# speechcatcher-asr/speechcatcher

Hardware: AMD Instinct MI355X
Metric: concurrent real-time streams (audio-seconds/s), de_xl dims, 640 ms (10240-sample) chunk steps, beam 10 CTC+attention (higher is better)
Workload: dtype f32

## Files before the change

### include/scasr.h

```cpp
#ifndef SCASR_H
#define SCASR_H

#include <stddef.h>
#include <stdint.h>

#ifdef __cplusplus
extern "C" {
#endif

#define SC_OK 0
#define SC_ERR_ARG (-1)
#define SC_ERR_LAUNCH (-2)
#define SC_ERR_CAPACITY (-3)
#define SC_ERR_INPUT (-4)

#define SC_GEMM_RELU 1
#define SC_GEMM_RESIDUAL 2
#define SC_GEMM_LN_AT_CROWS 8
#define SC_GEMM_NAIVE 4
#define SC_GEMM_SPLIT16 16

#define SC_F_ANY_EOS 1
#define SC_F_BEST_EOS 2
#define SC_F_ALL_EOS 4
// ... 613 lines not shown
  float ctc_weight;
  int32_t use_bbd;
  int32_t max_frames;
  int32_t max_tokens;
  int32_t pcm_capacity;
  int32_t max_chunk_samples;
  int32_t strict_reference;
  int32_t kv_half;
  int32_t kv_pool_rows;
} sc_stream_options;

typedef struct sc_stream_info_t {
  int32_t enc_frames, processed_block, process_idx, n_hyp, hyp_len, pcm_buffered, frontend_started;
  int64_t decode_steps;
} sc_stream_info_t;

typedef struct sc_engine sc_engine;
typedef struct sc_streams sc_streams;

int sc_engine_create(const sc_config *cfg, const sc_named_tensor *tensors, int n_tensors, int device, sc_engine **out);
int sc_engine_load(const char *packed_model_path, int device, sc_engine **out);
int sc_engine_config(const sc_engine *engine, sc_config *out);
void sc_engine_destroy(sc_engine *engine);

int sc_streams_create(sc_engine *engine, const sc_stream_options *options, sc_streams **out);
void sc_streams_destroy(sc_streams *streams);
int sc_push(sc_streams *streams, const int *stream_ids, const float *const *pcm, const int *n_samples,
            const uint8_t *is_final, int n, int *status);
int sc_push_features(sc_streams *streams, const int *stream_ids, const float *const *feats, const int *n_frames,
                     const uint8_t *is_final, int n, int *status);
int sc_submit(sc_streams *streams, const int *stream_ids, const float *const *pcm, const int *n_samples,
              const uint8_t *is_final, int n);
int sc_poll(sc_streams *streams, int min_done, int max_done, int *done_ids , int *status );
int sc_streams_outstanding(const sc_streams *streams);
int sc_streams_set_encoder_batch(sc_streams *streams, int min_streams);
int sc_streams_set_queue_depth(sc_streams *streams, int depth);
const char *sc_stream_last_error(const sc_streams *streams, int stream);
int sc_get_hyps(sc_streams *streams, int stream, int nbest, int max_len, int32_t *ids, int32_t *xpos, int *lens,
                double *scores, double *score_dec, double *score_ctc);
int sc_get_hyps_batch(sc_streams *streams, const int *stream_ids, int n, int nbest, int max_len, int32_t *ids,
                      int32_t *xpos, int *lens, int *n_hyps, double *scores, double *score_dec, double *score_ctc);
int sc_get_hyps_delta(sc_streams *streams, const int *stream_ids, int n, const int *from, const int *final,
                      int max_tail, int32_t *L, int32_t *commit, int32_t *n_hyps, int32_t *ids, int32_t *xpos,
                      double *stability, double *scores, int32_t *status);
int sc_rescore_hyps(sc_streams *streams, const int *stream_ids, int n, int nbest, const sc_lm *lm, double alpha,
                    double beta, int lm_eos, const int *final, int32_t *order, double *fused, double *lm_sum,
                    double *eos_lm, int32_t *status, int *n_hyps);
int sc_lm_rescore_lists(sc_streams *streams, const sc_lm *lm, const int32_t *ids, const int32_t *lens,
                        const double *scores, const int *list_sizes, int n, int nbest, int max_len,
                        const int32_t *state0, double alpha, double beta, int lm_eos, int32_t *order, double *fused,
                        double *lm_sum, double *eos_lm, int32_t *status, int32_t *end_state);
#define SC_ATT_WS_DEFAULT_BYTES ((size_t)256 << 20)
int sc_attention_rescore_beam(sc_streams *streams, const int *stream_ids, int n, int nbest, double w_att, double w_ctc,
                              double beta, int32_t *order, double *fused, double *att, double *ctc_score, int32_t *status,
                              int *n_hyps);
int sc_attention_rescore_lists(sc_streams *streams, const int *stream_ids, int n, const int32_t *ids, const int32_t *lens,
                               const double *scores, const int *list_sizes, int nbest, int max_len, double w_att,
                               double w_ctc, double beta, int32_t *order, double *fused, double *att, int32_t *status);
int sc_streams_set_attention_rescore_ws(sc_streams *streams, size_t max_bytes);
int sc_streams_attention_rescore_ws(const sc_streams *streams, size_t *limit, size_t *allocated);

int sc_align_hyps(sc_streams *streams, const int *stream_ids, int n, int nbest, int max_len, int32_t *start,
                  int32_t *end, float *logp_mean, double *path_score, int *status, int *n_hyps);
int sc_alternates_hyps(sc_streams *streams, const int *stream_ids, int n, int nbest, int max_len, int K, int32_t *start,
                       int32_t *end, float *logp_mean, double *path_score, int *status, int32_t *alt_ids,
                       double *alt_logp, int32_t *own_rank, int32_t *span_status, int *n_hyps);
int sc_align_tokens(sc_streams *streams, int stream, const int32_t *ids, int L, int32_t *start, int32_t *end,
                    float *logp_mean, double *path_score, int *status);
int sc_reset(sc_streams *streams, int stream);
int sc_stream_set_input_rate(sc_streams *streams, int stream, int rate);
int sc_stream_input_rate(const sc_streams *streams, int stream);
int sc_stream_set_input_format(sc_streams *streams, int stream, int format, int channels, int channel, int scale);
int sc_stream_input_format(const sc_streams *streams, int stream, int *format, int *channels, int *channel, int *scale);
int sc_push_raw(sc_streams *streams, const int *stream_ids, const void *const *audio, const int *n_frames,
                const uint8_t *is_final, int n, int *status);
int sc_submit_raw(sc_streams *streams, const int *stream_ids, const void *const *audio, const int *n_frames,
                  const uint8_t *is_final, int n);
int sc_stream_input_level(sc_streams *streams, int stream, sc_input_level_t *out );
int sc_stream_info(const sc_streams *streams, int stream, sc_stream_info_t *out);
#define SC_KV_POOL_DEFAULT_MAX_GIB 24
int sc_streams_kv_rows(const sc_streams *streams);
int sc_streams_stats(const sc_streams *streams, long *enc_calls, long *dec_steps, long *dec_blocks);
int sc_streams_capture_stats(const sc_streams *streams, long *n_captures, double *seconds);
int sc_streams_set_graphs(sc_streams *streams, int on);
int sc_marker(int id, void *stream);
int sc_streams_host_times(sc_streams *streams, double *launch_s, double *wait_s);
int sc_streams_bucket_times(sc_streams *streams, double *seconds, long *iterations);
long sc_streams_take_xattn_rows(sc_streams *streams);
int sc_streams_take_xattn_rows_by_kernel(sc_streams *streams, long *rows);
int sc_streams_take_attn_counters(sc_streams *streams, long *out );
void *sc_streams_hip_stream(sc_streams *streams);
float *sc_streams_pcm(sc_streams *streams, long *capacity);
int sc_streams_write_pcm(sc_streams *streams, int stream, long offset, const float *host, long n);
long sc_streams_read_pcm_buffer(sc_streams *streams, int stream, float *host, long max_n);
int sc_streams_read_enc(sc_streams *streams, int stream, float *host, int max_frames);
int sc_streams_read_ctc(sc_streams *streams, int stream, float *host, int max_rows);
int sc_streams_set_activity(sc_streams *streams, int on, double blank_threshold);
int sc_stream_activity(sc_streams *streams, int stream, sc_activity_t *out );
int sc_streams_read_activity(sc_streams *streams, int stream, double *host, int max_frames);
int sc_streams_set_phrases(sc_streams *streams, const int32_t *labels, const int32_t *lens, const double *min_scores,
                           int n_phrases);
int sc_stream_set_phrase_mask(sc_streams *streams, int stream, uint64_t mask);
int sc_stream_spot(sc_streams *streams, int stream, sc_spot_t *out );
int sc_streams_read_spot_events(sc_streams *streams, int stream, sc_spot_event *host, int max);
int sc_streams_read_spot_state(sc_streams *streams, int stream, double *values, int32_t *starts);
int sc_streams_set_draft(sc_streams *streams, int on);
int sc_stream_draft(sc_streams *streams, int stream, sc_draft_t *out );
int sc_streams_read_draft(sc_streams *streams, int stream, sc_draft_token *host, int max);
int sc_streams_set_ctc_beam(sc_streams *streams, int beam, int candidates);
int sc_stream_ctc_beam(sc_streams *streams, int stream, sc_beam_t *out );
int sc_ctc_beam_hyps(sc_streams *streams, const int *stream_ids, int n, int nbest, int max_len, int32_t *header ,
                     int32_t *ids , int32_t *frames , double *scores );
int sc_streams_set_ctc_beam_lm(sc_streams *streams, const sc_lm *lm, double alpha, double beta);
int sc_stream_ctc_beam_lm(sc_streams *streams, int stream, sc_beam_lm_t *out );
int sc_ctc_beam_hyps_lm(sc_streams *streams, const int *stream_ids, int n, int nbest, double *lm ,
                        double *fused );
int sc_stream_set_grammar(sc_streams *streams, int stream, sc_grammar *grammar );
int sc_stream_ctc_beam_grammar(sc_streams *streams, int stream, sc_beam_gr_t *out );
int sc_ctc_beam_hyps_grammar(sc_streams *streams, const int *stream_ids, int n, int nbest, int32_t *g ,
                             int32_t *accept );
#define SC_DECODER_FULL 0
#define SC_DECODER_NONE 1
int sc_stream_set_decoder(sc_streams *streams, int stream, int mode);
int sc_streams_read_ctc_projected(sc_streams *streams, int stream, float *host , int max_rows);
int sc_stream_decoder(const sc_streams *streams, int stream);

#ifdef __cplusplus
}
#endif
#endif
```

### speechcatcher_amd/_abi.py

```python
import ctypes as C
import os
import subprocess
from pathlib import Path

HERE = Path(__file__).resolve().parent
LIB_PATH = HERE / "libscasr.so"
CSRC = HERE / "csrc"

c_float_p = C.POINTER(C.c_float)
c_int_p = C.POINTER(C.c_int32)
c_double_p = C.POINTER(C.c_double)
vp = C.c_void_p


class EncLayer(C.Structure):
    _fields_ = [(n, vp) for n in ("ln1_g", "ln1_b", "wqkv", "bqkv", "wo", "bo",
                                  "ln2_g", "ln2_b", "w1", "b1", "w2", "b2", "w1_p", "w2_p",
                                  "wqkv_p", "wo_p", "w1_h", "w2_h", "wqkv_h", "wo_h", "w1_s", "w2_s",
                                  "wqkv_s", "wo_s")]


class DecLayer(C.Structure):
    _fields_ = [(n, vp) for n in ("ln1_g", "ln1_b", "wqkv", "bqkv", "wo", "bo",
                                  "ln2_g", "ln2_b", "wq", "bq", "wo2", "bo2",
# ... 258 lines not shown
                                  C.c_int, vp, vp, vp, vp]),
    "sc_rowtile_proj_h": (C.c_int, [vp, C.c_int, C.c_int, C.c_int, vp, vp, C.c_float, vp, vp, C.c_int, vp, vp,
                                    C.c_int, vp, vp, vp, vp]),
    "sc_rowtile_proj_s": (C.c_int, [vp, C.c_int, C.c_int, C.c_int, vp, vp, C.c_float, vp, vp, C.c_int, vp, vp,
                                    C.c_int, vp, vp, vp, vp]),
    "sc_rowtile_proj_supported": (C.c_int, [C.c_int, C.c_int]),
    "sc_workspace_bytes": (C.c_size_t, [vp]),
    "sc_ffn_ln_proj": (C.c_int, [vp, vp, C.c_int, C.c_int, C.c_int, vp, vp, vp, vp, vp, vp, vp, vp, C.c_float, vp,
                                 vp, vp, vp, C.c_int, vp]),
    "sc_graph_capture_begin": (C.c_int, [vp]),
    "sc_graph_capture_end": (C.c_int, [vp, C.POINTER(vp)]),
    "sc_graph_launch": (C.c_int, [vp, vp]),
    "sc_graph_destroy": (C.c_int, [vp]),
    "sc_set_workspace": (C.c_int, [vp, C.c_size_t]),
    "sc_set_stream_workspace": (C.c_int, [vp, vp, C.c_size_t]),
    "sc_prof_collect_kinds": (C.c_int, [C.POINTER(C.c_double), C.POINTER(C.c_double), C.POINTER(C.c_double),
                                        C.POINTER(C.c_longlong), C.c_int]),
    "sc_prof_enable": (C.c_int, [C.c_int]),
    "sc_prof_collect": (C.c_int, [c_double_p, c_double_p, C.POINTER(C.c_longlong)]),
    "sc_prof_collect2": (C.c_int, [c_double_p, c_double_p, c_double_p, C.POINTER(C.c_longlong)]),
    "sc_prof_event_overhead_ms": (C.c_double, [vp]),
    "sc_layernorm": (C.c_int, [vp, vp, C.c_int, vp, vp, C.c_int, C.c_int, C.c_int, vp, vp, C.c_float, vp]),
    "sc_copy_rows": (C.c_int, [vp, vp, vp, vp, C.c_int, C.c_int, vp]),
    "sc_log_softmax_rows": (C.c_int, [vp, vp, C.c_int, C.c_int, vp]),
    "sc_logmel": (C.c_int, [vp, C.c_int, vp, C.c_int, C.c_int, vp, vp, vp, vp, vp, C.c_int, C.c_int,
                            C.c_int, C.c_int, C.c_int, vp, vp]),
    "sc_conv1": (C.c_int, [vp, C.c_int, vp, C.c_int, C.c_int, vp, vp, C.c_int, vp, vp]),
    "sc_block_pack": (C.c_int, [vp, vp, C.c_int, C.c_int, vp, C.c_int, vp, vp]),
    "sc_ctx_handoff": (C.c_int, [vp, C.c_int, vp, C.c_int, vp, C.c_int, C.c_int, vp]),
    "sc_enc_attention": (C.c_int, [vp, vp, C.c_int, C.c_int, C.c_int, C.c_int, C.c_int, vp]),
    "sc_encoder_layers": (C.c_int, [vp, C.c_int, vp, C.c_int, C.c_int, C.c_int, vp, C.c_int, vp, vp,
                                    vp, vp, vp, C.c_int, C.c_int, C.c_int, C.c_float, vp]),
    "sc_glu_dwconv_bn_swish": (C.c_int, [vp, C.c_int, C.c_int, C.c_int, C.c_int, vp, vp, vp, vp, vp, vp,
                                         C.c_float, vp, vp]),
    "sc_relpos_attention": (C.c_int, [vp, vp, vp, vp, vp, C.c_int, C.c_int, C.c_int, C.c_int, vp]),
    "sc_relpos_attention_masked": (C.c_int, [vp, vp, vp, vp, vp, C.c_int, C.c_int, C.c_int, C.c_int, vp, C.c_int, vp]),
    "sc_ctc_extend_state": (C.c_int, [vp, vp]),
    "sc_dec_embed": (C.c_int, [vp, vp]),
    "sc_kv_rows_to_half": (C.c_int, [vp, vp, C.c_int, C.c_int, C.c_int, C.c_int, vp, vp]),
    "sc_dec_self_attn": (C.c_int, [vp, C.c_int, vp]),
    "sc_dec_cross_attn": (C.c_int, [vp, C.c_int, vp]),
    "sc_decoder_layers": (C.c_int, [vp, vp]),
    "sc_logsoftmax_topk": (C.c_int, [vp, vp]),
    "sc_ctc_prefix_scan": (C.c_int, [vp, vp]),
    "sc_fuse_topw": (C.c_int, [vp, vp]),
    "sc_beam_prune": (C.c_int, [vp, vp]),
    "sc_ctc_gather_state": (C.c_int, [vp, vp]),
    "sc_ctc_gather_state_split": (C.c_int, [vp, C.c_int, vp]),
    "sc_decode_step": (C.c_int, [vp, vp]),
    "sc_decode_step_ex": (C.c_int, [vp, C.c_int, vp]),
    "sc_ctc_prefix_scan_split": (C.c_int, [vp, C.c_int, vp]),
    "sc_dec_layer_fused_supported": (C.c_int, [C.c_int, C.c_int, C.c_int, C.c_int]),
    "sc_dec_layer_self": (C.c_int, [vp, C.c_int, vp, vp, vp, C.c_int, vp]),
    "sc_dec_layer_cross": (C.c_int, [vp, C.c_int, vp, vp, vp]),
    "sc_dec_layer_ffn": (C.c_int, [vp, C.c_int, vp, vp, vp, C.c_int, C.POINTER(C.c_int), vp]),
    "sc_dec_output_logits": (C.c_int, [vp, vp, vp, vp, C.c_int, vp]),
    "sc_streams_kv_rows": (C.c_int, [vp]),
    "sc_dec_layer_stream_supported": (C.c_int, [C.c_int, C.c_int, C.c_int, C.c_int]),
    "sc_dec_layer_stream": (C.c_int, [vp, C.c_int, vp, vp, vp, vp, C.c_int, vp]),
    "sc_dec_layer_reduce_ln": (C.c_int, [vp, C.c_int, vp, vp, vp, vp]),
    "sc_dec_layer_ffn_xn": (C.c_int, [vp, C.c_int, vp, vp, C.c_int, C.POINTER(C.c_int), vp]),
    "sc_engine_create": (C.c_int, [C.POINTER(Config), C.POINTER(NamedTensor), C.c_int, C.c_int, C.POINTER(vp)]),
    "sc_engine_load": (C.c_int, [C.c_char_p, C.c_int, C.POINTER(vp)]),
    "sc_engine_config": (C.c_int, [vp, C.POINTER(Config)]),
    "sc_engine_destroy": (None, [vp]),
    "sc_streams_create": (C.c_int, [vp, C.POINTER(StreamOptions), C.POINTER(vp)]),
    "sc_streams_destroy": (None, [vp]),
    "sc_push": (C.c_int, [vp, c_int_p, C.POINTER(vp), c_int_p, C.POINTER(C.c_uint8), C.c_int, c_int_p]),
    "sc_push_features": (C.c_int, [vp, c_int_p, C.POINTER(vp), c_int_p, C.POINTER(C.c_uint8), C.c_int, c_int_p]),
    "sc_get_hyps": (C.c_int, [vp, C.c_int, C.c_int, C.c_int, c_int_p, c_int_p, c_int_p, c_double_p, c_double_p,
                              c_double_p]),
    "sc_get_hyps_batch": (C.c_int, [vp, c_int_p, C.c_int, C.c_int, C.c_int, c_int_p, c_int_p, c_int_p, c_int_p,
                                    c_double_p, c_double_p, c_double_p]),
    "sc_submit": (C.c_int, [vp, c_int_p, C.POINTER(vp), c_int_p, C.POINTER(C.c_uint8), C.c_int]),
    "sc_poll": (C.c_int, [vp, C.c_int, C.c_int, c_int_p, c_int_p]),
    "sc_streams_outstanding": (C.c_int, [vp]),
    "sc_streams_set_encoder_batch": (C.c_int, [vp, C.c_int]),
    "sc_streams_set_queue_depth": (C.c_int, [vp, C.c_int]),
    "sc_stream_last_error": (C.c_char_p, [vp, C.c_int]),
    "sc_reset": (C.c_int, [vp, C.c_int]),
    "sc_stream_info": (C.c_int, [vp, C.c_int, C.POINTER(StreamInfo)]),
    "sc_streams_stats": (C.c_int, [vp, C.POINTER(C.c_long), C.POINTER(C.c_long), C.POINTER(C.c_long)]),
    "sc_streams_capture_stats": (C.c_int, [vp, C.POINTER(C.c_long), c_double_p]),
    "sc_streams_set_graphs": (C.c_int, [vp, C.c_int]),
    "sc_marker": (C.c_int, [C.c_int, vp]),
    "sc_streams_host_times": (C.c_int, [vp, c_double_p, c_double_p]),
    "sc_streams_bucket_times": (C.c_int, [vp, c_double_p, C.POINTER(C.c_long)]),
    "sc_streams_take_xattn_rows": (C.c_long, [vp]),
    "sc_streams_take_xattn_rows_by_kernel": (C.c_int, [vp, vp]),
    "sc_streams_take_attn_counters": (C.c_int, [vp, vp]),
    "sc_streams_hip_stream": (vp, [vp]),
    "sc_streams_pcm": (vp, [vp, C.POINTER(C.c_long)]),
    "sc_streams_write_pcm": (C.c_int, [vp, C.c_int, C.c_long, vp, C.c_long]),
    "sc_streams_read_pcm_buffer": (C.c_long, [vp, C.c_int, vp, C.c_long]),
    "sc_streams_read_enc": (C.c_int, [vp, C.c_int, vp, C.c_int]),
    "sc_ctc_align_ws_bytes": (C.c_size_t, [C.c_int]),
    "sc_ctc_align": (C.c_int, [vp, C.c_int, C.c_int, C.c_int, vp]),
    "sc_align_hyps": (C.c_int, [vp, c_int_p, C.c_int, C.c_int, C.c_int, c_int_p, c_int_p, c_float_p, c_double_p,
                                c_int_p, c_int_p]),
    "sc_align_tokens": (C.c_int, [vp, C.c_int, c_int_p, C.c_int, c_int_p, c_int_p, c_float_p, c_double_p, c_int_p]),
    "sc_streams_read_ctc": (C.c_int, [vp, C.c_int, vp, C.c_int]),
    "sc_ctc_alternates": (C.c_int, [vp, C.c_int, C.c_int, C.c_int, vp]),
    "sc_alternates_hyps": (C.c_int, [vp, c_int_p, C.c_int, C.c_int, C.c_int, C.c_int, c_int_p, c_int_p, c_float_p,
                                     c_double_p, c_int_p, c_int_p, c_double_p, c_int_p, c_int_p, c_int_p]),
    "sc_hyp_commit": (C.c_int, [vp, C.c_int, vp]),
    "sc_get_hyps_delta": (C.c_int, [vp, c_int_p, C.c_int, c_int_p, c_int_p, C.c_int, c_int_p, c_int_p, c_int_p, c_int_p,
                                    c_int_p, c_double_p, c_double_p, c_int_p]),
    "sc_ctc_activity": (C.c_int, [vp, C.c_int, vp]),
    "sc_streams_set_activity": (C.c_int, [vp, C.c_int, C.c_double]),
    "sc_stream_activity": (C.c_int, [vp, C.c_int, C.POINTER(Activity)]),
    "sc_streams_read_activity": (C.c_int, [vp, C.c_int, vp, C.c_int]),
    "sc_ctc_spot": (C.c_int, [vp, C.c_int, vp]),
    "sc_streams_set_phrases": (C.c_int, [vp, vp, vp, vp, C.c_int]),
    "sc_stream_set_phrase_mask": (C.c_int, [vp, C.c_int, C.c_uint64]),
    "sc_stream_spot": (C.c_int, [vp, C.c_int, C.POINTER(Spot)]),
    "sc_streams_read_spot_events": (C.c_int, [vp, C.c_int, vp, C.c_int]),
    "sc_streams_read_spot_state": (C.c_int, [vp, C.c_int, vp, vp]),
    "sc_ctc_draft": (C.c_int, [vp, C.c_int, vp]),
    "sc_streams_set_draft": (C.c_int, [vp, C.c_int]),
    "sc_stream_draft": (C.c_int, [vp, C.c_int, C.POINTER(Draft)]),
    "sc_streams_read_draft": (C.c_int, [vp, C.c_int, vp, C.c_int]),
    "sc_ctc_beam": (C.c_int, [vp, C.c_int, vp]),
    "sc_ctc_beam_pack": (C.c_int, [vp, C.c_int, vp]),
    "sc_ctc_beam_lm": (C.c_int, [vp, C.c_int, vp]),
    "sc_lm_create": (C.c_int, [vp, C.c_size_t, C.POINTER(vp)]),
    "sc_lm_destroy": (None, [vp]),
    "sc_lm_device_view": (C.c_int, [vp, C.POINTER(vp), C.POINTER(LmView)]),
    "sc_streams_set_ctc_beam": (C.c_int, [vp, C.c_int, C.c_int]),
    "sc_stream_ctc_beam": (C.c_int, [vp, C.c_int, C.POINTER(Beam)]),
    "sc_ctc_beam_hyps": (C.c_int, [vp, c_int_p, C.c_int, C.c_int, C.c_int, vp, vp, vp, vp]),
    "sc_streams_set_ctc_beam_lm": (C.c_int, [vp, vp, C.c_double, C.c_double]),
    "sc_stream_ctc_beam_lm": (C.c_int, [vp, C.c_int, C.POINTER(BeamLm)]),
    "sc_ctc_beam_hyps_lm": (C.c_int, [vp, c_int_p, C.c_int, C.c_int, vp, vp]),
    "sc_ctc_beam_grammar": (C.c_int, [vp, C.c_int, vp]),
    "sc_grammar_create": (C.c_int, [vp, C.c_size_t, C.POINTER(vp)]),
    "sc_grammar_destroy": (C.c_int, [vp]),
    "sc_grammar_device_view": (C.c_int, [vp, C.POINTER(vp), C.POINTER(GrammarView)]),
    "sc_grammar_use": (C.c_int, [vp, C.c_int]),
    "sc_grammar_step": (C.c_int, [vp, C.c_int, C.c_int]),
    "sc_grammar_accepts": (C.c_int, [vp, C.c_int]),
    "sc_stream_set_grammar": (C.c_int, [vp, C.c_int, vp]),
    "sc_stream_ctc_beam_grammar": (C.c_int, [vp, C.c_int, C.POINTER(BeamGr)]),
    "sc_ctc_beam_hyps_grammar": (C.c_int, [vp, c_int_p, C.c_int, C.c_int, c_int_p, c_int_p]),
    "sc_lm_rescore": (C.c_int, [vp, C.c_int, vp]),
    "sc_rescore_hyps": (C.c_int, [vp, c_int_p, C.c_int, C.c_int, vp, C.c_double, C.c_double, C.c_int, c_int_p, vp, vp,
                                  vp, vp, vp, c_int_p]),
    "sc_lm_rescore_lists": (C.c_int, [vp, vp, vp, vp, vp, c_int_p, C.c_int, C.c_int, C.c_int, vp, C.c_double,
                                      C.c_double, C.c_int, vp, vp, vp, vp, vp, vp]),
    "sc_seq_attention": (C.c_int, [vp, C.c_int, C.c_int, C.c_int, C.c_int, C.c_int, vp]),
    "sc_dec_rescore_ws_bytes": (C.c_size_t, [vp, C.c_long, C.c_long, C.c_int, C.c_int]),
    "sc_dec_rescore": (C.c_int, [vp, C.c_int, vp, vp, C.c_size_t, vp]),
    "sc_attention_rescore_beam": (C.c_int, [vp, c_int_p, C.c_int, C.c_int, C.c_double, C.c_double, C.c_double, vp, vp, vp, vp,
                                            vp, c_int_p]),
    "sc_attention_rescore_lists": (C.c_int, [vp, c_int_p, C.c_int, vp, vp, vp, c_int_p, C.c_int, C.c_int, C.c_double,
                                             C.c_double, C.c_double, vp, vp, vp, vp]),
    "sc_streams_set_attention_rescore_ws": (C.c_int, [vp, C.c_size_t]),
    "sc_streams_attention_rescore_ws": (C.c_int, [vp, C.POINTER(C.c_size_t), C.POINTER(C.c_size_t)]),
    "sc_stream_set_decoder": (C.c_int, [vp, C.c_int, C.c_int]),
    "sc_stream_decoder": (C.c_int, [vp, C.c_int]),
    "sc_streams_read_ctc_projected": (C.c_int, [vp, C.c_int, vp, C.c_int]),
    "sc_pcm_decode": (C.c_int, [vp, C.c_int, vp]),
    "sc_pcm_bytes_per_frame": (C.c_int, [C.c_int, C.c_int]),
    "sc_stream_set_input_format": (C.c_int, [vp, C.c_int, C.c_int, C.c_int, C.c_int, C.c_int]),
    "sc_stream_input_format": (C.c_int, [vp, C.c_int, c_int_p, c_int_p, c_int_p, c_int_p]),
    "sc_push_raw": (C.c_int, [vp, c_int_p, C.POINTER(vp), c_int_p, C.POINTER(C.c_uint8), C.c_int, c_int_p]),
    "sc_submit_raw": (C.c_int, [vp, c_int_p, C.POINTER(vp), c_int_p, C.POINTER(C.c_uint8), C.c_int]),
# ... 65 lines not shown
```

### speechcatcher_amd/csrc/streams.hip

```cpp
#include <algorithm>
#include <array>
#include <chrono>
#include <cmath>
#include <cstdarg>
#include <cstring>
#include <deque>
#include <map>
#include <memory>
#include <new>
#include <string>
#include <vector>

#include "common.h"
#include "handover.h"
#include "resample.h"

namespace {

#define HIP_TRY(call)                                                              \
  do {                                                                             \
    hipError_t e__ = (call);                                                       \
    if (e__ != hipSuccess) {                                                       \
      sc_set_error("%s: %s failed: %s", __func__, #call, hipGetErrorString(e__));  \
      return SC_ERR_LAUNCH;                                                        \
    }                                                                              \
  } while (0)
#define RC_TRY(call)                 \
  do {                               \
    int rc__ = (call);               \
    if (rc__ != SC_OK) return rc__;  \
  } while (0)

struct Tensor {
  void *ptr = nullptr;
  int64_t numel = 0;
  int dtype = 0;
  bool owned = false;
};

struct StreamFault {
  int stream;
  int code;
  std::string msg;
};

}

struct sc_engine {
  sc_config cfg{};
  int device = 0;
  std::map<std::string, Tensor> t;
  std::vector<sc_enc_layer> enc;
  std::vector<sc_dec_layer> dec;
  std::vector<const float *> wkv, bkv;
  float *wkv_all = nullptr, *bkv_all = nullptr;

  const float *f(const std::string &name, bool required = true) const {
    auto it = t.find(name);
    if (it == t.end()) {
      if (required) sc_set_error("sc_engine: tensor '%s' is missing", name.c_str());
      return nullptr;
    }
    return (const float *)it->second.ptr;
  }
  ~sc_engine() {
    for (auto &kv : t)
      if (kv.second.owned && kv.second.ptr) (void)hipFree(kv.second.ptr);
    if (wkv_all) (void)hipFree(wkv_all);
    if (bkv_all) (void)hipFree(bkv_all);
  }
};

namespace {

struct St {
  bool fe_started = false;
  long pcm_start = 0, pcm_end = 0;
  bool enc_started = false;
  int fpp = 0, nfeat = 0, upp = 0, nsub = 0;
  bool has_sub = false;
  int n_blocks = 0;
  bool has_addin = false, has_ctx = false;
  int short_pos = 0;
  int T_enc = 0, processed_block = 0, process_idx = 0;
  bool prev_valid = false, started = false;
  int cur = 0, L = 1, nhyp = 1;
  bool has_ctc = false;
  int T_ctc = 0, T_kv = 0, output_index = 0;
  int T_proj = 0, T_projkv = 0;
  long n_steps_total = 0;
  int T_hyp = 0;
  int rs_tab = -1, rs_par = 0;
  long rs_in = 0, rs_out = 0;
  int in_fmt = SC_PCM_F32, in_ch = 1, in_sel = 0, in_scale = SC_PCM_SCALE_FULL;
  bool coded() const { return in_fmt != SC_PCM_F32 || in_ch != 1; }
  bool no_dec = false;
};

// ... 62 lines not shown
  HIP_TRY(hipMemset(*p, 0, bytes));
  HIP_TRY(hipStreamSynchronize(nullptr));
  return SC_OK;
}

}

struct EncPlan {
  std::vector<int32_t> conv_jobs, a_rows, lin_dst, feat_src, feat_dst, blk_jobs, sjobs, emit_src, emit_dst, sub_src,
      sub_dst;
  struct Short { int s, ubase, U, pe_pos, dst_T; };
  std::vector<Short> shorts;
  int n_conv = 0, max_t1 = 0;
};

struct EncGroup {
  long gen = 0;
  bool launched = false, features = false;
  bool open = false;
  bool deferred = false;
  int slot = 0;
  int stage_slot = -1;
  std::vector<long long> copy_jobs;
  std::vector<sc_rs_job> rs_jobs;
  size_t stage_floats = 0;
  struct PcmSpan { int s; bool fin; };
  std::vector<sc_pcm_job> pcm_jobs;
  std::vector<PcmSpan> pcm_spans;
  size_t stage_bytes = 0;
  bool stage_filled = false;
  std::vector<int32_t> fe_jobs;
  int n_fe = 0, max_keep = 0;
  EncPlan P;
  std::vector<int32_t> ctc_rows, kv_src, kv_dst;
  struct Span {
    int s = 0, t0 = 0, t1 = 0;
    uint64_t mask = 0;
    const sc_grammar_view *grammar = nullptr;
    handover::Plan opt[N_OPT];
  };
  std::vector<Span> spans;
  bool same_rows = true;
  std::vector<int> streams;
  bool empty() const { return !n_fe && !P.n_conv; }
};

constexpr int N_ARENA = 8;
constexpr int N_STAGE = 4;
constexpr int N_RING = 4;
constexpr int CM_FIXED = 4 + SC_COMMIT_MAX_HYPS + 6;

struct sc_streams {
  sc_engine *eng = nullptr;
  sc_config cfg{};
  int S = 0, W = 0, K = 0, TCAP = 0, LCAP = 0, FCAP = 0, UCAP = 0, max_feat_new = 0, max_t1 = 0, max_t2 = 0,
      max_blocks = 0, max_chunk = 0, max_length = 500;
  long PCAP = 0;
  bool use_bbd = false, strict = true;
  hipStream_t stream = nullptr;
  hipStream_t stream_enc = nullptr, es = nullptr;
  hipEvent_t ev_iter[2] = {nullptr, nullptr};
  int32_t *ring_dev = nullptr;
  int32_t *rm_host[2] = {nullptr, nullptr};
  int rm_idx = 0;
  bool rm_dirty = false;
  int scan_split_min = 1024, scan_split_streams = 0;
  bool scan_long = false;
  int step_split_min() const { return (scan_long && (scan_split_streams <= 0 || n_rows_step <= scan_split_streams * W)) ? scan_split_min : 0; }
  int graph_key() const { return n_rows_step * 2 + (step_split_min() > 0 ? 1 : 0); }
  int enc_start_thr = 0;
  int enc_batch_min = 0;
  int gemm_flags = 0;
  void *ws = nullptr, *ws_enc = nullptr;
  std::vector<void *> owned, owned_host;
  float *pcm = nullptr, *featbuf = nullptr, *subbuf = nullptr, *prev_addin = nullptr, *past_ctx = nullptr, *enc = nullptr,
        *c1 = nullptr, *c2 = nullptr, *xblk = nullptr, *ws_xn = nullptr, *ws_qkv = nullptr, *ws_att = nullptr,
        *ws_ffh = nullptr;
  int32_t *jobs_ctx = nullptr, *ctrlmap = nullptr;
  float *kv_stage = nullptr;
  int kv_stage_rows = 0;
  sc_search sb{};
  int32_t *ctrlmap_host = nullptr, *flags_host = nullptr;
  int32_t *arena_host = nullptr, *arena_dev = nullptr;
  size_t slot_cap = 0, arena_off = 0;
  int cur_slot = 0;
  hipEvent_t ev_group[N_ARENA] = {nullptr};
  long slot_gen[N_ARENA] = {0};
  int32_t *bs_host = nullptr, *bs_dev = nullptr;
  size_t bs_cap = 0;
  int bs_i = 0;
  float *stage_host = nullptr, *stage_dev = nullptr;
  size_t stage_cap = 0;
  hipEvent_t ev_stage[N_STAGE] = {nullptr};
  bool stage_busy[N_STAGE] = {false};
  int stage_next = 0;
  long long *cjobs_host = nullptr, *cjobs_dev = nullptr;
  sc_rs_job *rsjobs_host = nullptr, *rsjobs_dev = nullptr;
  float *rs_hist = nullptr;
  sc_rs_tabs rs_tabs{};
  int rs_rate[SC_RS_MAX_TABS] = {0};
  int n_rs_tabs = 0;
  uint8_t *stageb_host = nullptr, *stageb_dev = nullptr;
  size_t stageb_cap = 0;
  sc_pcm_job *pcmjobs_host = nullptr, *pcmjobs_dev = nullptr;
  sc_input_level_t *lvl_state = nullptr;
  sc_input_level_t *lvl_out_host = nullptr, *lvl_out_dev = nullptr;
  struct LvlSpan { int s; long epoch, ticket; };
  std::vector<LvlSpan> stage_lvl[N_STAGE];
  handover::Track<LevelState> lvl;
  long lvl_ticket = 0;
  int32_t *pack_dev = nullptr, *pack_host = nullptr, *pjobs_host = nullptr, *pjobs_dev = nullptr;
  size_t pack_cap = 0;
  sc_hyp_commit_job *cmjobs_host = nullptr, *cmjobs_dev = nullptr;
  int32_t *cm_dev = nullptr, *cm_host = nullptr;
  size_t cm_cap = 0;
  char *al_dev = nullptr;
  size_t al_cap = 0;
  bool act_on = false;
  double act_thr = 0.8;
  int32_t *act_state = nullptr;
  double *act_track = nullptr;
  sc_ctc_activity_job *act_jobs_host = nullptr, *act_jobs_dev = nullptr;
  int32_t *act_out_host = nullptr, *act_out_dev = nullptr;
  handover::Track<ActState> act;
  bool spot_on = false;
  int spot_P = 0;
  int32_t *spot_labels = nullptr, *spot_lens = nullptr;
  double *spot_floors = nullptr;
  int32_t *spot_counters = nullptr;
  double *spot_values = nullptr;
  int32_t *spot_starts = nullptr;
  sc_spot_event *spot_events = nullptr;
  sc_ctc_spot_job *spot_jobs_host = nullptr, *spot_jobs_dev = nullptr;
  int32_t *spot_out_host = nullptr, *spot_out_dev = nullptr;
  handover::Track<SpotState> spot;
  std::vector<uint64_t> spot_mask;
  bool draft_on = false;
  sc_draft_t *draft_state = nullptr;
  sc_draft_token *draft_tokens = nullptr;
  sc_ctc_draft_job *draft_jobs_host = nullptr, *draft_jobs_dev = nullptr;
  sc_draft_t *draft_out_host = nullptr, *draft_out_dev = nullptr;
  handover::Track<DraftState> draft;
  bool beam_on = false;
  int beam_B = 0, beam_C = 0;
  int beam_nodes_B = 0;
  sc_beam_t *beam_state = nullptr;
  sc_beam_node *beam_nodes = nullptr;
  sc_ctc_beam_job *beam_jobs_host = nullptr, *beam_jobs_dev = nullptr;
  sc_beam_t *beam_out_host = nullptr, *beam_out_dev = nullptr;
  handover::Track<BeamState> beam;
  const sc_lm *beam_lm = nullptr;
  const sc_lm_view *beam_lm_view = nullptr;
  sc_lm_view beam_lm_info{};
  double beam_alpha = 0.0, beam_beta = 0.0;
  sc_beam_lm_t *beam_lm_state = nullptr;
  sc_ctc_beam_lm_job *beam_lm_jobs_host = nullptr, *beam_lm_jobs_dev = nullptr;
  sc_beam_lm_t *beam_lm_out_host = nullptr, *beam_lm_out_dev = nullptr;
  std::vector<sc_grammar *> beam_gr;
  int beam_gr_n = 0;
  sc_beam_gr_t *beam_gr_state = nullptr;
  sc_ctc_beam_gr_job *beam_gr_jobs_host = nullptr, *beam_gr_jobs_dev = nullptr;
  sc_beam_gr_t *beam_gr_out_host = nullptr, *beam_gr_out_dev = nullptr;
  char *bh_dev = nullptr, *bh_host = nullptr;
  size_t bh_cap = 0;
  char *rs_dev = nullptr, *rs_host = nullptr;
  size_t rs_cap = 0;
  char *ar_dev = nullptr, *ar_host = nullptr;
  size_t ar_cap = 0;
  char *ar_ws = nullptr;
  size_t ar_ws_bytes = 0, ar_ws_limit = SC_ATT_WS_DEFAULT_BYTES;
  void *ar_splitk = nullptr;
  size_t beam_ncap() const { return 1 + (size_t)beam_nodes_B * TCAP; }
  std::vector<St> st;
  std::vector<Run> run;
  std::vector<std::deque<Blk>> bq;
  std::vector<Job> job;
  std::vector<std::deque<Job>> ahead;
  std::vector<long> job_seq;
  int queue_depth = 1;
  std::vector<Snap> snap;
  std::vector<long> done_at;
  long done_counter = 0;
  int32_t *snap_yseq = nullptr, *snap_xpos = nullptr;
  double *snap_score = nullptr;
  hipEvent_t ev_snap = nullptr;
  std::vector<std::string> fault_msg;
  std::vector<long> enc_gen;
  std::deque<EncGroup *> groups;
  long gen_next = 1, gen_done = 0, gen_ordered = 0;
  int n_open = 0;
  long iter = 0;
  bool inflight = false;
  std::vector<int> tick_active;
  std::chrono::steady_clock::time_point tick_t0, tick_t1;
  hipStream_t stream_rb = nullptr;
  bool poisoned = false;
  std::vector<int> rowmap_key;
  int row_bucket = 1, n_rows_step = 0;
  bool decode_prepared = false;
  std::map<int, hipGraphExec_t> dec_graphs;
  std::map<std::vector<long>, hipGraphExec_t> enc_graphs;
  long dec_steps = 0, dec_blocks = 0, enc_calls = 0, xattn_rows[3] = {0, 0, 0};
  long sattn_pos[3] = {0, 0, 0};
  unsigned long long *stat_rows = nullptr;
  double t_launch = 0, t_wait = 0;
  double t_bucket[17] = {0};
  long n_bucket[17] = {0};
  bool use_graphs = true;
  long n_enc_captures = 0;
  double t_enc_capture = 0;

  ~sc_streams() {
    for (auto &g : dec_graphs) (void)hipGraphExecDestroy(g.second);
    for (auto &g : enc_graphs) (void)hipGraphExecDestroy(g.second);
    if (stream) (void)sc_set_stream_workspace(stream, nullptr, 0);
    if (stream_enc) {
      (void)sc_set_stream_workspace(stream_enc, nullptr, 0);
      (void)hipStreamDestroy(stream_enc);
    }
    for (int i = 0; i < 2; ++i)
      if (ev_iter[i]) (void)hipEventDestroy(ev_iter[i]);
    for (int i = 0; i < N_ARENA; ++i)
      if (ev_group[i]) (void)hipEventDestroy(ev_group[i]);
    for (int i = 0; i < N_STAGE; ++i)
      if (ev_stage[i]) (void)hipEventDestroy(ev_stage[i]);
    if (ev_snap) (void)hipEventDestroy(ev_snap);
    for (EncGroup *g : groups) delete g;
    for (void *p : owned) (void)hipFree(p);
    for (void *p : owned_host) (void)hipHostFree(p);
    if (stream_rb && ar_splitk) (void)sc_set_stream_workspace(stream_rb, nullptr, 0);
    if (stream_rb) (void)hipStreamDestroy(stream_rb);
    if (stream) (void)hipStreamDestroy(stream);
    if (ar_dev) (void)hipFree(ar_dev);
    if (ar_host) (void)hipHostFree(ar_host);
    if (ar_ws) (void)hipFree(ar_ws);
    if (ar_splitk) (void)hipFree(ar_splitk);
    if (al_dev) (void)hipFree(al_dev);
    if (beam_nodes) (void)hipFree(beam_nodes);
    for (sc_grammar *g : beam_gr)
      if (g) (void)sc_grammar_use(g, -1);
    if (bh_dev) (void)hipFree(bh_dev);
    if (bh_host) (void)hipHostFree(bh_host);
    if (rs_dev) (void)hipFree(rs_dev);
    if (rs_host) (void)hipHostFree(rs_host);
  }

  template <typename T>
  int alloc(T **p, size_t n) {
    RC_TRY(dalloc(p, n));
    owned.push_back(*p);
    return SC_OK;
  }
  template <typename T>
  int halloc(T **p, size_t n) {
    HIP_TRY(hipHostMalloc((void **)p, std::max<size_t>(n, 1) * sizeof(T)));
    owned_host.push_back(*p);
    memset(*p, 0, std::max<size_t>(n, 1) * sizeof(T));
    return SC_OK;
  }
  template <typename T>
  int halloc_mapped(T **host, T **dev, size_t n, const char *who, const char *what) {
    RC_TRY(halloc(host, n));
    void *dv = nullptr;
    if (hipHostGetDevicePointer(&dv, *host, 0) != hipSuccess || !dv) {
      sc_set_error("%s: the pinned %s are not visible to the device", who, what);
      return SC_ERR_LAUNCH;
    }
    *dev = (T *)dv;
    return SC_OK;
  }
  int32_t *ctrl_host() { return ctrlmap_host; }
  int32_t *rowmap_host() { return rm_host[rm_idx]; }

  int itensor(const std::vector<int32_t> &a, const int32_t **out) {
    const size_t n = a.size();
    if (arena_off + n > slot_cap) {
      sc_set_error("job-table arena exhausted (%zu + %zu of %zu entries)", arena_off, n, slot_cap);
      return SC_ERR_ARG;
    }
    const size_t off = (size_t)cur_slot * slot_cap + arena_off;
    arena_off += (n + 63) & ~size_t(63);
    if (n) {
      memcpy(arena_host + off, a.data(), n * sizeof(int32_t));
      HIP_TRY(hipMemcpyAsync(arena_dev + off, arena_host + off, n * sizeof(int32_t), hipMemcpyHostToDevice, es));
    }
    *out = arena_dev + off;
    return SC_OK;
  }
};


namespace {

constexpr int F_ANY_EOS = 1, F_BEST_EOS = 2, F_ALL_EOS = 4, F_REPEAT = 8;

__global__ void init_hyp_kernel(sc_search sb, int s) {
  const size_t o = ((size_t)0 * sb.S + s) * sb.W + 0;
  sb.yseq[o * sb.LCAP] = sb.sos;
  sb.xpos[o * sb.LCAP] = 0;
  sb.anc[((size_t)0 * sb.S + s) * sb.LCAP * sb.W] = 0;
  sb.score[o] = 0.0;
  sb.sc_dec[o] = 0.0;
  sb.sc_ctc[o] = 0.0;
}

__global__ __launch_bounds__(256) void scatter_f32_kernel(const float *__restrict__ src, float *__restrict__ dst,
                                                          const long long *__restrict__ jobs) {
  const long long so = jobs[blockIdx.y * 3], dof = jobs[blockIdx.y * 3 + 1], n = jobs[blockIdx.y * 3 + 2];
  for (long long i = (long long)blockIdx.x * 256 + threadIdx.x; i < n; i += (long long)gridDim.x * 256) dst[dof + i] = src[so + i];
}

void launch_scatter(const float *src, float *dst, const long long *jobs_dev, int nj, long long mx, hipStream_t st) {
  dim3 grid((unsigned)std::min<long long>(64, (std::max<long long>(mx, 1) + 1023) / 1024), nj);
  scatter_f32_kernel<<<grid, 256, 0, st>>>(src, dst, jobs_dev);
}

__global__ __launch_bounds__(128) void pack_hyps_kernel(sc_search sb, const int32_t *__restrict__ jobs, int32_t *__restrict__ out,
                                                        const int32_t *__restrict__ snap_yseq, const int32_t *__restrict__ snap_xpos,
                                                        const double *__restrict__ snap_score) {
  const int32_t *j = jobs + (size_t)blockIdx.x * 4;
  const size_t row = (size_t)j[0];
  const int L = j[1];
  const bool snap = j[3] != 0;
  int32_t *o = out + (size_t)j[2];
  const int32_t *ys = (snap ? snap_yseq : sb.yseq) + row * sb.LCAP, *xp = (snap ? snap_xpos : sb.xpos) + row * sb.LCAP;
  for (int i = threadIdx.x; i < L; i += 128) {
    o[i] = ys[i];
    o[L + i] = xp[i];
  }
  if (threadIdx.x == 0) {
    double *sc = (double *)(o + ((2 * L + 1) & ~1));
    sc[0] = snap ? snap_score[row * 3] : sb.score[row];
    sc[1] = snap ? snap_score[row * 3 + 1] : sb.sc_dec[row];
    sc[2] = snap ? snap_score[row * 3 + 2] : sb.sc_ctc[row];
  }
}

struct SnapArgs { int n; int s[32], cur[32], L[32], nhyp[32]; };
__global__ __launch_bounds__(128) void snapshot_hyps_kernel(sc_search sb, SnapArgs a, int32_t *__restrict__ snap_yseq,
                                                            int32_t *__restrict__ snap_xpos, double *__restrict__ snap_score) {
  const int e = blockIdx.x, h = blockIdx.y;
  if (h >= a.nhyp[e]) return;
  const size_t src = ((size_t)a.cur[e] * sb.S + a.s[e]) * sb.W + h, dst = (size_t)a.s[e] * sb.W + h;
  for (int i = threadIdx.x; i < a.L[e]; i += 128) {
    snap_yseq[dst * sb.LCAP + i] = sb.yseq[src * sb.LCAP + i];
    snap_xpos[dst * sb.LCAP + i] = sb.xpos[src * sb.LCAP + i];
  }
  if (threadIdx.x == 0) {
    snap_score[dst * 3] = sb.score[src];
    snap_score[dst * 3 + 1] = sb.sc_dec[src];
    snap_score[dst * 3 + 2] = sb.sc_ctc[src];
  }
}

void init_hyp(sc_streams *b, int s) {
  init_hyp_kernel<<<1, 1, 0, b->stream>>>(b->sb, s);
}

void reset_stream(sc_streams *b, int s) {
  St old = b->st[s], ns;
  ns.rs_tab = old.rs_tab;
  ns.in_fmt = old.in_fmt; ns.in_ch = old.in_ch; ns.in_sel = old.in_sel; ns.in_scale = old.in_scale;
  ns.no_dec = old.no_dec;
  if (b->strict) {
    ns.short_pos = old.short_pos;
    ns.T_ctc = old.T_ctc;
    ns.T_proj = old.T_ctc;
  }
  b->st[s] = ns;
  b->run[s] = Run();
// ... 142 lines not shown
        st.has_sub = true;
        st.nsub = U;
        continue;
      }
      const int overlap = c.block_size - c.hop_size;
      nb = std::max(0, U - overlap) / c.hop_size;
      const int res = U - c.hop_size * nb;
      const int obase = ((1 - st.upp) * S + s) * b->UCAP;
      for (int i = 0; i < res; ++i) {
        P.sub_src.push_back(ubase + U - res + i);
        P.sub_dst.push_back(obase + i);
      }
      st.upp = 1 - st.upp;
      st.has_sub = true;
      st.nsub = res;
    }
    nb = std::max(nb, 0);
    const int b0 = n_blk_jobs;
    for (int i = 0; i < nb; ++i) {
      const int cur_hop = i * c.hop_size;
      const int clen = std::min(c.block_size, U - cur_hop);
      P.blk_jobs.insert(P.blk_jobs.end(), {ubase + cur_hop, clen, cur_hop + c.hop_size * st.n_blocks, i + st.n_blocks, 0, 0});
      ++n_blk_jobs;
    }
    if (nb > 0) {
      P.sjobs.insert(P.sjobs.end(), {b0, nb, s, (int)st.has_addin, (int)st.has_ctx});
      st.has_addin = st.has_ctx = true;
    }
    const bool first = st.n_blocks == 0;
    const int y_len = fin ? (first ? U : U - offset) : nb * c.hop_size + (first ? offset : 0);
    std::vector<int32_t> src(std::max(y_len, 0), -1);
    if (first && nb > 0)
      for (int i = 0; i < offset && i < y_len; ++i) src[i] = b0 * R + 1 + i;
    for (int i = 0; i < nb; ++i) {
      const int cur_hop = i * c.hop_size + (first ? offset : 0);
      const int clen = (i == nb - 1 && fin) ? std::min(c.block_size - offset, y_len - cur_hop) : c.hop_size;
      for (int j = 0; j < clen; ++j)
        if (cur_hop + j >= 0 && cur_hop + j < y_len) src[cur_hop + j] = (b0 + i) * R + 1 + offset + j;
    }
    if (st.T_enc + y_len > b->TCAP) throw StreamFault{s, SC_ERR_CAPACITY, "encoder-frame capacity exceeded (max_frames)"};
    for (int i = 0; i < y_len; ++i) {
      P.emit_src.push_back(src[i]);
      P.emit_dst.push_back(s * b->TCAP + st.T_enc + i);
    }
    st.T_enc += y_len;
    st.n_blocks += nb;
  }
  for (int s : streams)
    if (finals.at(s)) {
      St &st = b->st[s];
      st.enc_started = false;
      st.nfeat = st.nsub = st.n_blocks = 0;
      st.has_sub = st.has_addin = st.has_ctx = false;
    }
}

int enc_layers_launch(sc_streams *b, int nblk, int R, bool masked, const int32_t *jobs, int ns) {
  const sc_config &c = b->cfg;
  sc_engine *e = b->eng;
  auto launch = [&]() {
    return sc_encoder_layers(e->enc.data(), (int)e->enc.size(), b->xblk, nblk, R, masked ? 1 : 0, jobs, ns, b->past_ctx,
                             b->ws_xn, b->ws_qkv, b->ws_att, b->ws_ffh, c.d_model, c.enc_heads, c.ffn_dim, c.ln_eps,
                             b->es);
  };
  if (!b->use_graphs) return launch();
  std::vector<long> key{nblk, R, (long)masked, (long)(intptr_t)jobs, ns};
  auto it = b->enc_graphs.find(key);
  if (it == b->enc_graphs.end()) {
    if (b->enc_graphs.size() >= 192) return launch();
    const auto tc0 = std::chrono::steady_clock::now();
    RC_TRY(sc_graph_capture_begin(b->es));
    const int rc = launch();
    void *g = nullptr;
    const int rc2 = sc_graph_capture_end(b->es, &g);
    b->n_enc_captures++;
    b->t_enc_capture += std::chrono::duration<double>(std::chrono::steady_clock::now() - tc0).count();
    if (rc != SC_OK) return rc;
    if (rc2 != SC_OK) return rc2;
    it = b->enc_graphs.emplace(key, (hipGraphExec_t)g).first;
  }
  return sc_graph_launch(it->second, b->es);
}

int encode_short(sc_streams *b, const EncPlan::Short &sh) {
  const sc_config &c = b->cfg;
  sc_engine *e = b->eng;
  const int U = sh.U;
  const int32_t *jd, *src, *dst;
  RC_TRY(b->itensor({sh.ubase, U, sh.pe_pos, 0, 1, 0}, &jd));
  RC_TRY(sc_block_pack(b->subbuf, jd, 1, U, e->f("pe"), c.d_model, b->xblk, b->es));
  RC_TRY(sc_encoder_layers(e->enc.data(), (int)e->enc.size(), b->xblk, 1, U, 0, nullptr, 0, b->past_ctx, b->ws_xn,
                           b->ws_qkv, b->ws_att, b->ws_ffh, c.d_model, c.enc_heads, c.ffn_dim, c.ln_eps, b->es));
  std::vector<int32_t> a(U), d(U);
  for (int i = 0; i < U; ++i) { a[i] = i; d[i] = sh.s * b->TCAP + sh.dst_T + i; }
  RC_TRY(b->itensor(a, &src));
  RC_TRY(b->itensor(d, &dst));
  RC_TRY(sc_layernorm(b->xblk, src, c.d_model, b->enc, dst, c.d_model, U, c.d_model, e->f("enc_norm_g"), e->f("enc_norm_b"),
                      c.ln_eps, b->es));
  return SC_OK;
}

int encode_launch(sc_streams *b, EncPlan &P) {
  const sc_config &c = b->cfg;
  sc_engine *e = b->eng;
  const int d = c.d_model, F1 = c.conv_freq1, F2 = c.conv_freq2, R = c.block_size + 2;
  b->enc_calls++;
  const int32_t *cj, *ar, *ld;
  RC_TRY(b->itensor(P.conv_jobs, &cj));
  RC_TRY(sc_conv1(b->featbuf, c.n_mels, cj, P.n_conv, P.max_t1, e->f("conv1_w"), e->f("conv1_b"), d, b->c1, b->es));
  RC_TRY(b->itensor(P.a_rows, &ar));
  RC_TRY(sc_gemm(b->c1, ar, d, e->f("conv2_w"), e->f("conv2_b"), b->c2, nullptr, d, (int)P.a_rows.size(), d, 9 * d,
                 SC_GEMM_RELU | b->gemm_flags, F1, b->es));
  RC_TRY(b->itensor(P.lin_dst, &ld));
  RC_TRY(sc_gemm(b->c2, nullptr, F2 * d, e->f("sub_out_w"), e->f("sub_out_b"), b->subbuf, ld, d, (int)P.lin_dst.size(), d,
                 F2 * d, b->gemm_flags, 0, b->es));
  if (!P.feat_src.empty()) {
    const int32_t *a, *z;
    RC_TRY(b->itensor(P.feat_src, &a));
    RC_TRY(b->itensor(P.feat_dst, &z));
    RC_TRY(sc_copy_rows(b->featbuf, a, b->featbuf, z, (int)P.feat_src.size(), c.n_mels, b->es));
  }
  const int nbk = (int)P.blk_jobs.size() / 6, ns = (int)P.sjobs.size() / 5;
  if (nbk > 0) {
    if (nbk > b->max_blocks) {
      sc_set_error("sc_push: too many encoder blocks in one call");
      return SC_ERR_ARG;
    }
    const int32_t *bj, *ja;
    RC_TRY(b->itensor(P.blk_jobs, &bj));
    RC_TRY(sc_block_pack(b->subbuf, bj, nbk, R, e->f("pe"), d, b->xblk, b->es));
    std::vector<int32_t> j_add(ns * 4), j_ctx(ns * 4);
    for (int i = 0; i < ns; ++i) {
      const int32_t *sj = &P.sjobs[i * 5];
      j_add[i * 4 + 0] = sj[0]; j_add[i * 4 + 1] = sj[1]; j_add[i * 4 + 2] = sj[2]; j_add[i * 4 + 3] = sj[3];
      j_ctx[i * 4 + 0] = sj[0]; j_ctx[i * 4 + 1] = sj[1]; j_ctx[i * 4 + 2] = sj[2] * c.enc_layers; j_ctx[i * 4 + 3] = sj[4];
    }
    RC_TRY(b->itensor(j_add, &ja));
    RC_TRY(sc_ctx_handoff(b->xblk, R, ja, ns, b->prev_addin, 0, d, b->es));
    const int32_t *jc;
    RC_TRY(b->itensor(j_ctx, &jc));
    HIP_TRY(hipMemcpyAsync(b->jobs_ctx, jc, j_ctx.size() * sizeof(int32_t), hipMemcpyDeviceToDevice, b->es));
    RC_TRY(enc_layers_launch(b, nbk, R, true, b->jobs_ctx, ns));
  }
  if (!P.emit_src.empty()) {
    const int32_t *a, *z;
    RC_TRY(b->itensor(P.emit_src, &a));
    RC_TRY(b->itensor(P.emit_dst, &z));
    RC_TRY(sc_layernorm(b->xblk, a, d, b->enc, z, d, (int)P.emit_src.size(), d, e->f("enc_norm_g"), e->f("enc_norm_b"),
                        c.ln_eps, b->es));
  }
  for (auto &sh : P.shorts) RC_TRY(encode_short(b, sh));
  if (!P.sub_src.empty()) {
    const int32_t *a, *z;
    RC_TRY(b->itensor(P.sub_src, &a));
    RC_TRY(b->itensor(P.sub_dst, &z));
    RC_TRY(sc_copy_rows(b->subbuf, a, b->subbuf, z, (int)P.sub_src.size(), d, b->es));
  }
  return SC_OK;
}

void set_rowmap(sc_streams *b, const std::vector<int> &active) {
  const int S = b->S, W = b->W;
  const int na = (int)active.size();
  const int nb = std::min(S, (na + b->row_bucket - 1) / b->row_bucket * b->row_bucket);
  if (active != b->rowmap_key) {
    b->rowmap_key = active;
    b->rm_idx ^= 1;
    b->rm_dirty = true;
    int32_t *rm = b->rowmap_host();
    std::vector<char> isact(S, 0);
    for (int s : active) isact[s] = 1;
    int k = 0;
    for (int pass = 1; pass >= 0; --pass)
      for (int s = 0; s < S; ++s)
        if (isact[s] == pass)
          for (int h = 0; h < W; ++h) rm[k++] = s * W + h;
  }
  b->n_rows_step = nb * W;
}

int decode_step_launch(sc_streams *b) {
  b->sb.n_rows = b->n_rows_step;
  b->sb.flags = b->ring_dev;
  auto step = [&]() { return sc_decode_step_ex(&b->sb, b->step_split_min(), b->stream); };
  if (!b->use_graphs) return step();
  auto it = b->dec_graphs.find(b->graph_key());
  if (it == b->dec_graphs.end()) {
    RC_TRY(step());
    RC_TRY(sc_graph_capture_begin(b->stream));
    const int rc = step();
    void *g = nullptr;
    const int rc2 = sc_graph_capture_end(b->stream, &g);
    if (rc != SC_OK) return rc;
    if (rc2 != SC_OK) return rc2;
    b->dec_graphs[b->graph_key()] = (hipGraphExec_t)g;
    return SC_OK;
  }
  return sc_graph_launch(it->second, b->stream);
}

int prepare_decode(sc_streams *b) {
  memset(b->ctrl_host(), 0, (size_t)b->S * 8 * sizeof(int32_t));
  HIP_TRY(hipMemcpyAsync(b->ctrlmap, b->ctrlmap_host, (size_t)b->S * 8 * sizeof(int32_t), hipMemcpyHostToDevice, b->stream));
  const int keep = b->n_rows_step;
  for (int nb = b->row_bucket; nb < b->S + b->row_bucket; nb += b->row_bucket) {
    b->n_rows_step = std::min(nb, b->S) * b->W;
    if (!b->dec_graphs.count(b->graph_key())) RC_TRY(decode_step_launch(b));
  }
  b->n_rows_step = keep;
  HIP_TRY(hipStreamSynchronize(b->stream));
  return SC_OK;
}

int collect_levels(sc_streams *b, int slot, bool wait) {
  std::vector<sc_streams::LvlSpan> &spans = b->stage_lvl[slot];
  if (spans.empty()) return SC_OK;
  if (wait) HIP_TRY(hipEventSynchronize(b->ev_stage[slot]));
  else {
    const hipError_t q = hipEventQuery(b->ev_stage[slot]);
    if (q == hipErrorNotReady) { (void)hipGetLastError(); return SC_OK; }
    if (q != hipSuccess) {
      sc_set_error("staging slot %d failed: %s", slot, hipGetErrorString(q));
      return SC_ERR_LAUNCH;
    }
  }
  for (size_t i = 0; i < spans.size(); ++i) {
    const sc_streams::LvlSpan &sp = spans[i];
    b->lvl.deliver(sp.s, sp.ticket, sp.epoch, b->lvl_out_host[(size_t)slot * b->S + i], b->job[sp.s], b->ahead[sp.s], &Job::level);
  }
  spans.clear();
  return SC_OK;
}

int retire_groups(sc_streams *b) {
  if (b->lvl_state)
    for (int i = 0; i < N_STAGE; ++i) RC_TRY(collect_levels(b, i, false));
  while (!b->groups.empty()) {
    EncGroup *g = b->groups.front();
    if (!g->launched) break;
    const hipError_t q = hipEventQuery(b->ev_group[g->slot]);
    if (q == hipErrorNotReady) { (void)hipGetLastError(); break; }
    if (q != hipSuccess) {
      sc_set_error("encoder group %ld failed: %s", g->gen, hipGetErrorString(q));
      return SC_ERR_LAUNCH;
    }
    for (size_t i = 0; i < g->spans.size(); ++i) {
      const EncGroup::Span &sp = g->spans[i];
      const int s = sp.s;
      const size_t o = (size_t)g->slot * b->S + i;
      if (sp.opt[OPT_ACT].on) {
        ActState v;
        v.T = sp.t1;
        memcpy(v.v, b->act_out_host + o * 6, sizeof v.v);
        b->act.deliver(s, g->gen, sp.opt[OPT_ACT].epoch, v, b->job[s], b->ahead[s], &Job::act);
      }
      if (sp.opt[OPT_SPOT].on) {
        SpotState v;
        memcpy(v.v, b->spot_out_host + o * 2, sizeof v.v);
        b->spot.deliver(s, g->gen, sp.opt[OPT_SPOT].epoch, v, b->job[s], b->ahead[s], &Job::spot);
      }
      if (sp.opt[OPT_DRAFT].on)
        b->draft.deliver(s, g->gen, sp.opt[OPT_DRAFT].epoch, DraftState{b->draft_out_host[o]}, b->job[s], b->ahead[s], &Job::draft);
      if (sp.opt[OPT_BEAM].on)
        b->beam.deliver(s, g->gen, sp.opt[OPT_BEAM].epoch,
                        b->beam_lm      ? BeamState(b->beam_out_host[o], b->beam_lm_out_host[o])
                        : sp.grammar ? BeamState(b->beam_out_host[o], b->beam_gr_out_host[o])
                                     : BeamState(b->beam_out_host[o]),
                        b->job[s], b->ahead[s], &Job::beam);
    }
    b->gen_done = g->gen;
    b->slot_gen[g->slot] = 0;
    b->groups.pop_front();
    delete g;
  }
  return SC_OK;
}

int launch_pending_groups(sc_streams *b, long upto = -1);
int wait_group(sc_streams *b, long gen) {
  if (gen <= b->gen_done) return SC_OK;
  RC_TRY(launch_pending_groups(b, gen));
  const int slot = (int)(gen % N_ARENA);
  HIP_TRY(hipEventSynchronize(b->ev_group[slot]));
  return retire_groups(b);
}

template <typename J>
void span_job(const sc_streams *b, J &j, const EncGroup::Span &sp, int opt) {
  const int V = b->cfg.vocab_size;
  j.table = b->sb.ctcx + (size_t)sp.s * b->TCAP * V;
  j.stride = V;
  j.V = V; j.blank = b->cfg.blank_id; j.t0 = sp.t0; j.t1 = sp.t1;
  j.restart = sp.opt[opt].restart ? 1 : 0;
}

void span_job(const sc_streams *b, sc_ctc_beam_lm_job &j, const EncGroup::Span &sp, int opt) { span_job(b, j.beam, sp, opt); }

template <typename J, typename Fill>
int launch_spans(sc_streams *b, const EncGroup &g, int opt, const char *name, J *jobs_host, J *jobs_dev,
                 int (*launch)(const J *, int, void *), Fill fill) {
  if (g.spans.empty() || !g.spans[0].opt[opt].on) return SC_OK;
  const int n = (int)g.spans.size();
  if (n > b->S) {
    sc_set_error("%s: %d spans in a group of a batch of %d streams (internal error)", name, n, b->S);
    return SC_ERR_ARG;
  }
  const size_t o = (size_t)g.slot * b->S;
  for (int i = 0; i < n; ++i) {
    span_job(b, jobs_host[o + i], g.spans[i], opt);
    fill(jobs_host[o + i], g.spans[i], o + i);
  }
  HIP_TRY(hipMemcpyAsync(jobs_dev + o, jobs_host + o, (size_t)n * sizeof(J), hipMemcpyHostToDevice, b->es));
  return launch(jobs_dev + o, n, b->es);
}

template <typename Fill>
int launch_beam_grammars(sc_streams *b, const EncGroup &g, Fill beam_fill) {
  if (g.spans.empty() || !g.spans[0].opt[OPT_BEAM].on) return SC_OK;
  const int n = (int)g.spans.size();
  if (n > b->S) {
    sc_set_error("beam: %d spans in a group of a batch of %d streams (internal error)", n, b->S);
    return SC_ERR_ARG;
  }
  const size_t o = (size_t)g.slot * b->S;
  int n_plain = 0, n_gr = 0;
  for (int i = 0; i < n; ++i) {
    const EncGroup::Span &sp = g.spans[i];
    if (!sp.grammar) {
      sc_ctc_beam_job &j = b->beam_jobs_host[o + n_plain++];
      span_job(b, j, sp, OPT_BEAM);
      beam_fill(j, sp, o + i);
    } else {
      sc_ctc_beam_gr_job &j = b->beam_gr_jobs_host[o + n_gr++];
      span_job(b, j.beam, sp, OPT_BEAM);
      beam_fill(j.beam, sp, o + i);
      j.grammar = sp.grammar;
      j.gr_state = b->beam_gr_state + sp.s;
      j.gr_state_after = b->beam_gr_out_dev + o + i;
    }
  }
  if (n_plain) {
    HIP_TRY(hipMemcpyAsync(b->beam_jobs_dev + o, b->beam_jobs_host + o, (size_t)n_plain * sizeof(sc_ctc_beam_job),
                           hipMemcpyHostToDevice, b->es));
    RC_TRY(sc_ctc_beam(b->beam_jobs_dev + o, n_plain, b->es));
  }
  if (n_gr) {
    HIP_TRY(hipMemcpyAsync(b->beam_gr_jobs_dev + o, b->beam_gr_jobs_host + o, (size_t)n_gr * sizeof(sc_ctc_beam_gr_job),
                           hipMemcpyHostToDevice, b->es));
    RC_TRY(sc_ctc_beam_grammar(b->beam_gr_jobs_dev + o, n_gr, b->es));
  }
  return SC_OK;
}

int project_rows(sc_streams *b, EncGroup &g) {
  const sc_config &c = b->cfg;
  sc_engine *e = b->eng;
  const int d = c.d_model, Ld = c.dec_layers, V = c.vocab_size;
  const int32_t *ar = nullptr;
  if (!g.ctc_rows.empty()) {
    RC_TRY(b->itensor(g.ctc_rows, &ar));
    RC_TRY(sc_gemm(b->enc, ar, d, e->f("ctc_w"), e->f("ctc_b"), const_cast<float *>(b->sb.ctcx), ar, V, (int)g.ctc_rows.size(),
                   V, d, b->gemm_flags, 0, b->es));
    RC_TRY(launch_spans(b, g, OPT_ACT, "activity", b->act_jobs_host, b->act_jobs_dev, sc_ctc_activity,
                        [=](sc_ctc_activity_job &j, const EncGroup::Span &sp, size_t at) {
                          j.state = b->act_state + (size_t)sp.s * 6;
                          j.track = b->act_track + (size_t)sp.s * b->TCAP;
                          j.state_after = b->act_out_dev + at * 6;
                          j.thr = b->act_thr;
                          j.reserved = 0;
                        }));
    RC_TRY(launch_spans(b, g, OPT_SPOT, "spotting", b->spot_jobs_host, b->spot_jobs_dev, sc_ctc_spot,
                        [=](sc_ctc_spot_job &j, const EncGroup::Span &sp, size_t at) {
                          j.labels = b->spot_labels; j.lens = b->spot_lens; j.floors = b->spot_floors;
                          j.counters = b->spot_counters + (size_t)sp.s * 2;
                          j.values = b->spot_values + (size_t)sp.s * SC_SPOT_MAX_PHRASES * SC_SPOT_STATES;
                          j.starts = b->spot_starts + (size_t)sp.s * SC_SPOT_MAX_PHRASES * SC_SPOT_STATES;
                          j.events = b->spot_events + (size_t)sp.s * SC_SPOT_MAX_EVENTS;
                          j.state_after = b->spot_out_dev + at * 2;
                          j.mask = sp.mask;
                          j.P = b->spot_P;
                        }));
    RC_TRY(launch_spans(b, g, OPT_DRAFT, "draft", b->draft_jobs_host, b->draft_jobs_dev, sc_ctc_draft,
                        [=](sc_ctc_draft_job &j, const EncGroup::Span &sp, size_t at) {
                          j.state = b->draft_state + sp.s;
                          j.tokens = b->draft_tokens + (size_t)sp.s * b->TCAP;
                          j.state_after = b->draft_out_dev + at;
                          j.capacity = b->TCAP;
                        }));
    const auto beam_fill = [=](sc_ctc_beam_job &j, const EncGroup::Span &sp, size_t at) {
      j.state = b->beam_state + sp.s;
      j.nodes = b->beam_nodes + (size_t)sp.s * b->beam_ncap();
      j.state_after = b->beam_out_dev + at;
      j.capacity = (int32_t)b->beam_ncap();
      j.B = b->beam_B; j.C = b->beam_C;
    };
    bool any_grammar = false;
    for (const EncGroup::Span &sp : g.spans) any_grammar = any_grammar || sp.grammar;
    if (any_grammar)
      RC_TRY(launch_beam_grammars(b, g, beam_fill));
    else if (!b->beam_lm)
      RC_TRY(launch_spans(b, g, OPT_BEAM, "beam", b->beam_jobs_host, b->beam_jobs_dev, sc_ctc_beam, beam_fill));
    else
      RC_TRY(launch_spans(b, g, OPT_BEAM, "beam", b->beam_lm_jobs_host, b->beam_lm_jobs_dev, sc_ctc_beam_lm,
                          [=](sc_ctc_beam_lm_job &j, const EncGroup::Span &sp, size_t at) {
                            beam_fill(j.beam, sp, at);
                            j.lm = b->beam_lm_view;
                            j.lm_state = b->beam_lm_state + sp.s;
                            j.lm_state_after = b->beam_lm_out_dev + at;
                            j.alpha = b->beam_alpha; j.beta = b->beam_beta;
                          }));
  }
  if (!g.kv_dst.empty()) {
    if (!g.same_rows || !ar) RC_TRY(b->itensor(g.kv_src, &ar));
    const int32_t *kvt;
    RC_TRY(b->itensor(g.kv_dst, &kvt));
    const int m = (int)g.kv_dst.size();
    const bool all = e->wkv_all && (2 * d) % 128 == 0;
    if (!b->sb.kv_half) {
      if (all && sc_gemm_colblocks(b->enc, ar, d, e->wkv_all, e->bkv_all, const_cast<float *>(b->sb.ckv), kvt, 2 * d, m, Ld * 2 * d, d,
                                   2 * d, (long)b->TCAP * 2 * d, b->gemm_flags, b->es) == SC_OK)
        return SC_OK;
      for (int li = 0; li < Ld; ++li)
        RC_TRY(sc_gemm(b->enc, ar, d, e->wkv[li], e->bkv[li], const_cast<float *>(b->sb.ckv) + (size_t)li * b->TCAP * 2 * d,
                       kvt, 2 * d, m, 2 * d, d, b->gemm_flags, 0, b->es));
    } else {
      for (int r0 = 0; r0 < m; r0 += b->kv_stage_rows) {
        const int mm = std::min(b->kv_stage_rows, m - r0);
        if (!(all && sc_gemm_colblocks(b->enc, ar + r0, d, e->wkv_all, e->bkv_all, b->kv_stage, nullptr, 2 * d, mm, Ld * 2 * d, d, 2 * d,
                                       (long)mm * 2 * d, b->gemm_flags, b->es) == SC_OK))
          for (int li = 0; li < Ld; ++li)
            RC_TRY(sc_gemm(b->enc, ar + r0, d, e->wkv[li], e->bkv[li], b->kv_stage + (size_t)li * mm * 2 * d, nullptr, 2 * d,
                           mm, 2 * d, d, b->gemm_flags, 0, b->es));
        RC_TRY(sc_kv_rows_to_half(b->kv_stage, kvt + r0, mm, Ld, b->TCAP, 2 * d, const_cast<float *>(b->sb.ckv), b->es));
      }
    }
  }
  return SC_OK;
}

int stage_copy(sc_streams *b, EncGroup &g) {
  if (g.copy_jobs.empty() && g.rs_jobs.empty() && g.pcm_jobs.empty()) return SC_OK;
  hipStream_t es = b->stream_enc ? b->stream_enc : b->stream;
  const int ss = g.stage_slot;
  const size_t so = (size_t)ss * b->stage_cap, jo = (size_t)ss * b->S * 3;
  const int nj = (int)g.copy_jobs.size() / 3;
  if (g.stage_floats && (g.stage_filled || g.pcm_jobs.empty()))
    HIP_TRY(hipMemcpyAsync(b->stage_dev + so, b->stage_host + so, g.stage_floats * sizeof(float), hipMemcpyHostToDevice, es));
  if (!g.pcm_jobs.empty()) {
    const size_t bo = (size_t)ss * b->stageb_cap, po = (size_t)ss * b->S;
    const int np = (int)g.pcm_jobs.size();
    if (g.stage_bytes)
      HIP_TRY(hipMemcpyAsync(b->stageb_dev + bo, b->stageb_host + bo, g.stage_bytes, hipMemcpyHostToDevice, es));
    memcpy(b->pcmjobs_host + po, g.pcm_jobs.data(), np * sizeof(sc_pcm_job));
    HIP_TRY(hipMemcpyAsync(b->pcmjobs_dev + po, b->pcmjobs_host + po, np * sizeof(sc_pcm_job), hipMemcpyHostToDevice, es));
    RC_TRY(sc_pcm_decode(b->pcmjobs_dev + po, np, es));
  }
  if (nj) {
    memcpy(b->cjobs_host + jo, g.copy_jobs.data(), g.copy_jobs.size() * sizeof(long long));
    HIP_TRY(hipMemcpyAsync(b->cjobs_dev + jo, b->cjobs_host + jo, g.copy_jobs.size() * sizeof(long long), hipMemcpyHostToDevice, es));
    long long mx = 1;
    for (int j = 0; j < nj; ++j) mx = std::max(mx, g.copy_jobs[j * 3 + 2]);
    launch_scatter(b->stage_dev + so, g.features ? b->featbuf : b->pcm, b->cjobs_dev + jo, nj, mx, es);
  }
  if (!g.rs_jobs.empty()) {
    const size_t ro = (size_t)ss * b->S;
    const int nr = (int)g.rs_jobs.size();
    memcpy(b->rsjobs_host + ro, g.rs_jobs.data(), nr * sizeof(sc_rs_job));
    HIP_TRY(hipMemcpyAsync(b->rsjobs_dev + ro, b->rsjobs_host + ro, nr * sizeof(sc_rs_job), hipMemcpyHostToDevice, es));
    long long tiles = 1;
    for (const sc_rs_job &j : g.rs_jobs) tiles = std::max(tiles, sc_rs_tiles(b->rs_tabs, j.tab, j.n_out));
    RC_TRY(sc_rs_launch(b->rs_tabs, nullptr, b->rsjobs_dev + ro, nr, tiles, b->stage_dev + so, b->pcm, b->rs_hist, b->S, es));
  }
  HIP_TRY(hipEventRecord(b->ev_stage[ss], es));
  b->stage_busy[ss] = true;
  g.copy_jobs.clear();
  g.rs_jobs.clear();
  g.pcm_jobs.clear();
  g.pcm_spans.clear();
  return SC_OK;
}

void merge_group(sc_streams *b, EncGroup &dst, EncGroup &src) {
  const sc_config &c = b->cfg;
  const int F1 = c.conv_freq1, R = c.block_size + 2;
  EncPlan &D = dst.P, &P = src.P;
  int c1_rows = 0;
  if (D.n_conv) c1_rows = D.conv_jobs[(D.n_conv - 1) * 4 + 2] + D.conv_jobs[(D.n_conv - 1) * 4 + 3];
  const int nblk = (int)D.blk_jobs.size() / 6;
  for (int j = 0; j < P.n_conv; ++j) P.conv_jobs[j * 4 + 2] += c1_rows;
  for (auto &v : P.a_rows) v += c1_rows * F1;
  for (size_t j = 0; j < P.sjobs.size(); j += 5) P.sjobs[j] += nblk;
  for (auto &v : P.emit_src)
    if (v >= 0) v += nblk * R;
  auto cat = [](std::vector<int32_t> &a, const std::vector<int32_t> &x) { a.insert(a.end(), x.begin(), x.end()); };
  cat(D.conv_jobs, P.conv_jobs); cat(D.a_rows, P.a_rows); cat(D.lin_dst, P.lin_dst); cat(D.feat_src, P.feat_src);
  cat(D.feat_dst, P.feat_dst); cat(D.blk_jobs, P.blk_jobs); cat(D.sjobs, P.sjobs); cat(D.emit_src, P.emit_src);
  cat(D.emit_dst, P.emit_dst); cat(D.sub_src, P.sub_src); cat(D.sub_dst, P.sub_dst);
  D.shorts.insert(D.shorts.end(), P.shorts.begin(), P.shorts.end());
  D.n_conv += P.n_conv;
  D.max_t1 = std::max(D.max_t1, P.max_t1);
  cat(dst.fe_jobs, src.fe_jobs);
  dst.n_fe += src.n_fe;
  dst.max_keep = std::max(dst.max_keep, src.max_keep);
  cat(dst.ctc_rows, src.ctc_rows); cat(dst.kv_src, src.kv_src); cat(dst.kv_dst, src.kv_dst);
  dst.spans.insert(dst.spans.end(), src.spans.begin(), src.spans.end());
  dst.same_rows = dst.same_rows && src.same_rows;
  dst.streams.insert(dst.streams.end(), src.streams.begin(), src.streams.end());
}

int launch_group(sc_streams *b, EncGroup *g) {
  if (g->launched) return SC_OK;
  g->launched = true;
  g->open = false;
  const sc_config &c = b->cfg;
  sc_engine *e = b->eng;
  b->es = b->stream_enc ? b->stream_enc : b->stream;
  b->cur_slot = g->slot;
  b->arena_off = 0;
  int rc = SC_OK;
  if (rc == SC_OK && g->n_fe) {
    const int32_t *jobs;
    rc = b->itensor(g->fe_jobs, &jobs);
    if (rc == SC_OK)
      rc = sc_logmel(b->pcm, (int)b->PCAP, jobs, g->n_fe, g->max_keep, e->f("window"), e->f("mel_fb"), e->f("twiddle"),
                     (const double *)e->f("mean64"), (const double *)e->f("std64"), c.mvn_mode, c.n_fft, c.hop_length,
                     c.win_length, c.n_mels, b->featbuf, b->es);
  }
  if (rc == SC_OK && g->P.n_conv) rc = encode_launch(b, g->P);
  if (rc == SC_OK) rc = project_rows(b, *g);
  (void)hipEventRecord(b->ev_group[g->slot], b->es);
  if (b->es == b->stream) b->gen_ordered = std::max(b->gen_ordered, g->gen);
  b->es = b->stream;
  return rc;
}

int launch_pending_groups(sc_streams *b, long upto) {
  for (EncGroup *g : b->groups)
    if (!g->launched && (upto < 0 || g->gen <= upto)) RC_TRY(launch_group(b, g));
  return SC_OK;
}

void finish_block(sc_streams *b, int s) {
  Run &r = b->run[s];
  const bool rw = r.pidx > 1 && r.pvalid;
  const bool r2 = rw && r.took;
  if (r2) {
    r.cur = 1 - r.cur;
    r.L -= 1;
    r.nhyp = r.nhp;
    r.has = r.hasp;
  }
  if (rw) { r.pidx -= 1; r.pvalid = false; }
  St &x = b->st[s];
  x.cur = r.cur; x.L = r.L; x.nhyp = r.nhyp; x.has_ctc = r.has;
  x.T_hyp = r.T;
  x.process_idx = r.pidx; x.prev_valid = r.pvalid;
  x.output_index = r.out;
  x.n_steps_total += r.nsteps;
  if (!r.fin) x.processed_block += 1;
  r.inblk = false;
}

void fault_stream(sc_streams *b, int s, int code, const std::string &msg) {
  const long seq = b->run[s].inblk ? b->run[s].job : b->job[s].seq;
  bool hit = false;
  auto mark = [&](Job &j) {
    if (!j.open) return;
    if (j.seq == seq) { j.fault = code; hit = true; }
    else if (hit && !j.fault) { j.fault = code; j.dropped = true; }
  };
  mark(b->job[s]);
  for (Job &j : b->ahead[s]) mark(j);
  b->fault_msg[s] = msg;
  b->run[s] = Run();
  b->bq[s].clear();
}

inline bool chunk_decoded(const sc_streams *b, int s);

inline bool may_start(const sc_streams *b, int s) {
  const Job &j = b->job[s];
  const long q = b->bq[s].front().job;
  if (!j.open || q <= j.seq) return true;
  return q == j.seq + 1 && b->snap[s].valid && b->snap[s].seq == j.seq;
}

int snapshot_completed(sc_streams *b) {
  if (b->queue_depth <= 1) return SC_OK;
  SnapArgs a;
  a.n = 0;
  bool any = false;
  auto flush = [&]() -> int {
    if (!a.n) return SC_OK;
    snapshot_hyps_kernel<<<dim3(a.n, b->W), 128, 0, b->stream>>>(b->sb, a, b->snap_yseq, b->snap_xpos, b->snap_score);
    SC_CHECK_LAUNCH();
    a.n = 0;
    return SC_OK;
  };
  for (int s = 0; s < b->S; ++s) {
    const Job &j = b->job[s];
    Snap &sn = b->snap[s];
    if (!j.open || j.fault || sn.valid || !chunk_decoded(b, s)) continue;
    const St &x = b->st[s];
    sn.valid = true;
    sn.reported = false;
    sn.seq = j.seq;
    sn.L = x.L;
    sn.T = x.T_hyp;
    sn.nhyp = j.started ? x.nhyp : 0;
    if (sn.nhyp > 0) {
      a.s[a.n] = s; a.cur[a.n] = x.cur; a.L[a.n] = x.L; a.nhyp[a.n] = x.nhyp;
      a.n++;
      any = true;
      if (a.n == 32) RC_TRY(flush());
    }
  }
  RC_TRY(flush());
  if (any) HIP_TRY(hipEventRecord(b->ev_snap, b->stream));
  return SC_OK;
}

int start_blocks(sc_streams *b) {
  const int S = b->S;
  const long gen_ok = std::max(b->gen_done, b->gen_ordered);
  std::vector<int> starts;
  for (int s = 0; s < S; ++s)
    if (!b->run[s].inblk && !b->bq[s].empty() && b->bq[s].front().gen <= gen_ok && may_start(b, s)) starts.push_back(s);
  if (starts.empty()) return SC_OK;
  if (!b->decode_prepared) {
    b->decode_prepared = true;
    RC_TRY(prepare_decode(b));
  }
  b->bs_i = (b->bs_i + 1) % N_RING;
  int32_t *ctrl0 = b->bs_host + (size_t)b->bs_i * b->bs_cap, *lsm = ctrl0 + (size_t)S * 8;
  memset(ctrl0, 0, (size_t)S * 8 * sizeof(int32_t));
  int n_lsm = 0;
  for (int s : starts) {
    const Blk k = b->bq[s].front();
    b->bq[s].pop_front();
    St &x = b->st[s];
    Run &r = b->run[s];
    r = Run();
    r.inblk = r.live = true;
    r.T = k.T; r.fin = k.fin; r.job = k.job;
    r.cur = x.cur; r.L = x.L; r.nhyp = x.nhyp; r.has = x.has_ctc; r.pidx = x.process_idx; r.pvalid = x.prev_valid;
    const int told = x.T_ctc;
    r.Tc = std::max(k.T, told);
    if (k.T > told && told == 0)
      for (int t = 0; t < k.T && n_lsm < (int)(b->bs_cap - (size_t)S * 8); ++t) lsm[n_lsm++] = s * b->TCAP + t;
    int32_t *c = ctrl0 + s * 8;
    c[0] = 1; c[1] = r.cur; c[2] = r.fin; c[3] = r.Tc; c[4] = r.L; c[5] = r.nhyp; c[6] = r.has; c[7] = told;
    x.T_ctc = r.Tc;
    x.T_kv = std::max(k.T, x.T_kv);
    x.output_index = 0;
    r.nhp = r.nhyp; r.hasp = r.has;
    b->dec_blocks++;
  }
  HIP_TRY(hipMemcpyAsync(b->ctrlmap, ctrl0, (size_t)S * 8 * sizeof(int32_t), hipMemcpyHostToDevice, b->stream));
  if (n_lsm) {
    int32_t *ld = b->bs_dev + (size_t)b->bs_i * b->bs_cap;
    HIP_TRY(hipMemcpyAsync(ld, lsm, (size_t)n_lsm * sizeof(int32_t), hipMemcpyHostToDevice, b->stream));
    RC_TRY(sc_log_softmax_rows(const_cast<float *>(b->sb.ctcx), ld, n_lsm, b->cfg.vocab_size, b->stream));
  }
  RC_TRY(sc_ctc_extend_state(&b->sb, b->stream));
  return SC_OK;
}

int tick_collect(sc_streams *b);
int tick_issue(sc_streams *b, bool *progress) {
  const int S = b->S, W = b->W, Ld = b->cfg.dec_layers;
  *progress = false;
  if (b->inflight) RC_TRY(tick_collect(b));
  RC_TRY(retire_groups(b));
  RC_TRY(snapshot_completed(b));
  RC_TRY(start_blocks(b));
  {
    long need = 0;
    for (int s = 0; s < S; ++s)
      if (!b->run[s].inblk && !b->bq[s].empty()) need = std::max(need, b->bq[s].front().gen);
    long upto = -1;
    for (EncGroup *g : b->groups)
      if (!g->launched && g->deferred && g->gen <= need) upto = g->gen;
    if (upto >= 0) RC_TRY(launch_pending_groups(b, upto));
  }
  std::vector<int> &active = b->tick_active;
  active.clear();
  for (int s = 0; s < S; ++s) {
    Run &r = b->run[s];
    if (!r.inblk) continue;
    const bool act = r.live && r.pidx < b->max_length;
    if (act && r.L + 1 > b->LCAP) {
      fault_stream(b, s, SC_ERR_CAPACITY, "max_tokens exceeded");
      *progress = true;
      continue;
    }
    if (!act) {
      finish_block(b, s);
      *progress = true;
      continue;
    }
    active.push_back(s);
  }
  if (active.empty()) {
    if (*progress) return SC_OK;
    long need = 0;
    for (int s = 0; s < S; ++s)
      if (!b->run[s].inblk && !b->bq[s].empty() && (need == 0 || b->bq[s].front().gen < need)) need = b->bq[s].front().gen;
    if (need > std::max(b->gen_done, b->gen_ordered)) {
      RC_TRY(launch_pending_groups(b, need));
      if (b->stream_enc) HIP_TRY(hipStreamWaitEvent(b->stream, b->ev_group[need % N_ARENA], 0));
      b->gen_ordered = std::max(b->gen_ordered, need);
      *progress = true;
    }
    return SC_OK;
  }
  *progress = true;
  b->tick_t0 = std::chrono::steady_clock::now();
  set_rowmap(b, active);
  b->scan_long = false;
  int32_t *ctrl = b->ctrl_host();
  memset(ctrl, 0, (size_t)S * 8 * sizeof(int32_t));
  for (int s : active) {
    const Run &r = b->run[s];
    if (b->scan_split_min > 0 && r.Tc - std::max(r.L - 1, 1) >= b->scan_split_min) b->scan_long = true;
    int32_t *c = ctrl + s * 8;
    c[0] = 1; c[1] = r.cur; c[2] = r.fin; c[3] = r.T; c[4] = r.L; c[5] = r.nhyp; c[6] = r.has; c[7] = r.Tc;
  }
  if ((int)active.size() <= b->enc_start_thr)
    for (EncGroup *g : b->groups)
      if (!g->launched && !g->open) RC_TRY(launch_group(b, g));
  if (b->rm_dirty) {
    memcpy(b->ctrlmap_host + S * 8, b->rm_host[b->rm_idx], (size_t)S * W * sizeof(int32_t));
    HIP_TRY(hipMemcpyAsync(b->ctrlmap, b->ctrlmap_host, (size_t)(S * 8 + S * W) * sizeof(int32_t), hipMemcpyHostToDevice, b->stream));
    b->rm_dirty = false;
  } else {
    HIP_TRY(hipMemcpyAsync(b->ctrlmap, b->ctrlmap_host, (size_t)S * 8 * sizeof(int32_t), hipMemcpyHostToDevice, b->stream));
  }
  RC_TRY(decode_step_launch(b));
  HIP_TRY(hipEventRecord(b->ev_iter[b->iter & 1], b->stream));
  const int form = sc_decode_step_form(&b->sb);
  for (int s : active) {
    b->xattn_rows[form] += (long)b->run[s].T * Ld;
    b->sattn_pos[form] += (long)b->run[s].L * Ld;
  }
  b->tick_t1 = std::chrono::steady_clock::now();
  b->inflight = true;
  return SC_OK;
}

int tick_collect(sc_streams *b) {
  if (!b->inflight) return SC_OK;
  const int S = b->S, W = b->W;
  b->inflight = false;
  const auto tpw = std::chrono::steady_clock::now();
  HIP_TRY(hipEventSynchronize(b->ev_iter[b->iter & 1]));
  const auto tp2 = std::chrono::steady_clock::now();
  b->iter++;
  b->dec_steps++;
  b->t_launch += std::chrono::duration<double>(b->tick_t1 - b->tick_t0).count();
  b->t_wait += std::chrono::duration<double>(tp2 - tpw).count();
  {
    const int bk = std::min(16, (int)((long)b->n_rows_step * 16 / std::max(1, S * W)));
    b->t_bucket[bk] += std::chrono::duration<double>(tp2 - b->tick_t0).count();
    b->n_bucket[bk] += 1;
  }
  for (int s : b->tick_active) {
    Run &r = b->run[s];
    const bool kv_full = b->flags_host[S + s] != 0;
    b->flags_host[S + s] = 0;
    const int f = b->flags_host[s];
    const bool f_any = f & F_ANY_EOS, f_best = f & F_BEST_EOS, f_all = f & F_ALL_EOS, f_rep = f & F_REPEAT;
    r.out += 1;
    r.nsteps += 1;
    const bool stop_eos = f_any && (!r.fin || f_best);
    const bool stop_bbd = b->use_bbd && !stop_eos && f_rep && !r.fin;
    const bool stop_all = !stop_eos && !stop_bbd && f_all && r.fin;
    const bool accept = !(stop_eos || stop_bbd || stop_all);
    const bool take = stop_eos || stop_all || accept;
    if (kv_full && take && !(!accept && r.pidx > 1 && r.pvalid)) {
      fault_stream(b, s, SC_ERR_CAPACITY, "self-attention K|V pool exhausted (kv_pool_rows / max_tokens)");
      continue;
    }
    if (stop_bbd) r.out -= 1;
    if (take) {
      r.nhp = r.nhyp;
      r.hasp = r.has;
      r.cur = 1 - r.cur;
      r.L += 1;
      r.nhyp = std::min(W, r.nhyp * W);
      r.has = true;
    }
    if (stop_eos || stop_all) r.took = true;
    r.live = accept;
    if (accept) {
      r.pvalid = true;
      r.pidx += 1;
    }
    if (!(r.live && r.pidx < b->max_length)) finish_block(b, s);
  }
  return SC_OK;
}

int engine_tick(sc_streams *b, bool *progress) {
  RC_TRY(tick_issue(b, progress));
  return tick_collect(b);
}

inline bool chunk_decoded(const sc_streams *b, int s) {
  const long q = b->job[s].seq;
  return !(b->run[s].inblk && b->run[s].job <= q) && (b->bq[s].empty() || b->bq[s].front().job > q);
}
inline bool chunk_complete(const sc_streams *b, int s) {
  const Job &j = b->job[s];
  if (!j.open) return false;
  if (j.fault != 0) return true;
  if (!chunk_decoded(b, s)) return false;
  return b->queue_depth <= 1 || (b->snap[s].valid && b->snap[s].seq == j.seq);
}

struct Chunk { int s; const void *host; long n; bool fin; int pos; };

inline long st_gen(const sc_streams *b, int s) { return b->enc_gen[s] > b->gen_done ? b->enc_gen[s] : 0; }

void plan_group(sc_streams *b, const std::vector<Chunk> &chunks, bool features, EncGroup &g, std::map<int, int> &feat_new,
                std::map<int, bool> &finals, std::vector<int> &has_out) {
  const sc_config &c = b->cfg;
  float *stage = g.stage_slot >= 0 ? b->stage_host + (size_t)g.stage_slot * b->stage_cap : nullptr;
  auto stage_chunk = [&](const Chunk &ch, const St &st) {
    if (!st.coded()) {
      if (ch.n > 0) memcpy(stage + g.stage_floats, ch.host, (size_t)ch.n * sizeof(float));
      g.stage_filled = g.stage_filled || ch.n > 0;
      return;
    }
    const size_t nb = (size_t)ch.n * (size_t)sc_pcm_bytes_per_frame(st.in_fmt, st.in_ch);
    if (g.stage_bytes + nb > b->stageb_cap)
      throw StreamFault{ch.s, SC_ERR_CAPACITY, "the chunk's raw bytes do not fit the staging slot's byte region (max_chunk_samples x 4 bytes x streams)"};
    const size_t bo = (size_t)g.stage_slot * b->stageb_cap, po = (size_t)g.stage_slot * b->S;
    if (nb) memcpy(b->stageb_host + bo + g.stage_bytes, ch.host, nb);
    sc_pcm_job j{};
    j.src = b->stageb_dev + bo;
    j.offset = (int64_t)g.stage_bytes;
    j.dst = b->stage_dev + (size_t)g.stage_slot * b->stage_cap + g.stage_floats;
    j.level = b->lvl_state + ch.s;
    j.level_after = b->lvl_out_dev + po + g.pcm_jobs.size();
    j.format = st.in_fmt; j.channels = st.in_ch; j.channel = st.in_sel; j.scale = st.in_scale;
    j.n = (int32_t)ch.n;
    j.restart = 0;
    g.pcm_jobs.push_back(j);
    g.pcm_spans.push_back({ch.s, ch.fin});
    g.stage_bytes += (nb + 3) & ~size_t(3);
  };
  for (size_t k = 0; k < chunks.size(); ++k) {
    const Chunk &ch = chunks[k];
    St &st = b->st[ch.s];
    finals[ch.s] = ch.fin;
    if (features) {
      const int nbuf = st.enc_started ? st.nfeat : 0;
      if (ch.n > b->max_feat_new || nbuf + ch.n > b->FCAP)
        throw StreamFault{ch.s, SC_ERR_CAPACITY, "feature frames of one call exceed the batch's capacity (max_chunk_samples)"};
      if (ch.n > 0) {
        const size_t cnt = (size_t)ch.n * c.n_mels;
        memcpy(stage + g.stage_floats, ch.host, cnt * sizeof(float));
        g.copy_jobs.insert(g.copy_jobs.end(), {(long long)g.stage_floats,
                                               (long long)(((size_t)(st.fpp * b->S + ch.s) * b->FCAP + nbuf) * c.n_mels), (long long)cnt});
        g.stage_floats += cnt;
      }
      feat_new[ch.s] = (int)ch.n;
      has_out[k] = 1;
      continue;
    }
    if (st.rs_tab >= 0) {
      const int t = st.rs_tab;
      const long lim = b->max_chunk + 16 * c.hop_length;
      const long out_total = sc_rs_out_count(b->rs_tabs.L[t], b->rs_tabs.M[t], b->rs_tabs.Wc[t], st.rs_in + ch.n, ch.fin);
      const long n_out = out_total - st.rs_out;
      if (ch.n > lim || n_out > lim) throw StreamFault{ch.s, SC_ERR_CAPACITY, "chunk is longer than max_chunk_samples allows"};
      if (st.pcm_end + n_out > b->PCAP) throw StreamFault{ch.s, SC_ERR_CAPACITY, "pcm buffer capacity exceeded"};
      if (st.coded() && !(ch.n > 0 || n_out > 0)) stage_chunk(ch, st);
      if (ch.n > 0 || n_out > 0) {
        stage_chunk(ch, st);
        g.rs_jobs.push_back(sc_rs_job{(long long)g.stage_floats, (long long)ch.n, (long long)ch.s * b->PCAP + st.pcm_end,
                                      (long long)n_out, (long long)st.rs_out, (long long)st.rs_in, t, ch.s, st.rs_par, 0});
        g.stage_floats += (size_t)ch.n;
        st.rs_par ^= 1;
      }
      st.rs_in += ch.n;
      st.rs_out = out_total;
      if (ch.fin) st.rs_in = st.rs_out = 0;
      st.pcm_end += n_out;
    } else {
      if (st.pcm_end + ch.n > b->PCAP) throw StreamFault{ch.s, SC_ERR_CAPACITY, "pcm buffer capacity exceeded"};
      if (st.coded() && !(ch.n > 0 && ch.host)) stage_chunk(ch, st);
      if (ch.n > 0 && ch.host) {
        if (ch.n > b->max_chunk + 16 * c.hop_length)
          throw StreamFault{ch.s, SC_ERR_CAPACITY, "chunk is longer than max_chunk_samples allows"};
        stage_chunk(ch, st);
        g.copy_jobs.insert(g.copy_jobs.end(), {(long long)g.stage_floats, (long long)ch.s * b->PCAP + st.pcm_end, (long long)ch.n});
        g.stage_floats += (size_t)ch.n;
      }
      st.pcm_end += ch.n;
    }
    FePlan p = plan_frontend(c, st, ch.fin);
    if (!p.emit) continue;
    if (p.n > b->max_feat_new) throw StreamFault{ch.s, SC_ERR_CAPACITY, "chunk produces more feature frames than max_chunk_samples allows"};
    const int nbuf = st.enc_started ? st.nfeat : 0;
    const int dst_row0 = (st.fpp * b->S + ch.s) * b->FCAP + nbuf;
    g.fe_jobs.insert(g.fe_jobs.end(), {ch.s, (int)p.seg_start, (int)p.seg_len, (int)p.eff_len, p.lo, p.n, dst_row0, 0});
    ++g.n_fe;
    g.max_keep = std::max(g.max_keep, p.n);
    feat_new[ch.s] = p.n;
    has_out[k] = 1;
  }
  std::vector<int> enc_streams;
  for (auto &kv : feat_new) {
    St &st = b->st[kv.first];
    if (!st.started) st.started = true;
    if (kv.second >= 3) enc_streams.push_back(kv.first);
  }
  if (!enc_streams.empty()) encode_plan(b, enc_streams, feat_new, finals, g.P);
}

int admit(sc_streams *b, std::vector<Chunk> chunks, bool features, bool defer, std::vector<int> *has_out_by_pos) {
  const sc_config &c = b->cfg;
  RC_TRY(retire_groups(b));
  bool host_input = false;
// ... 383 lines not shown
    ptrs.push_back(p);
    tens[i] = sc_named_tensor{names[i].c_str(), p, numel, dt};
  }
  fclose(fp);
  const int rc = sc_engine_create(&cfg, tens.data(), n, device, out);
  if (rc != SC_OK) {
    for (void *p : ptrs) (void)hipFree(p);
    return rc;
  }
  for (auto &kv : (*out)->t) kv.second.owned = true;
  return SC_OK;
  SC_API_END
}

extern "C" void sc_engine_destroy(sc_engine *e) { delete e; }

extern "C" int sc_engine_config(const sc_engine *e, sc_config *out) {
  SC_CHECK_ARG(e && out, "null");
  *out = e->cfg;
  return SC_OK;
}

extern "C" int sc_streams_create(sc_engine *e, const sc_stream_options *o, sc_streams **out) {
  SC_CHECK_ARG(e && o && out, "null");
  SC_API_BEGIN
  const sc_config &c = e->cfg;
  SC_CHECK_ARG(o->n_streams > 0 && o->beam_size > 0 && o->max_frames > 0 && o->max_tokens > 1, "bad options");
  const int pre_beam = 40;
  const int K = std::min(pre_beam, c.vocab_size);
  SC_CHECK_ARG(o->beam_size <= K && o->beam_size <= 16, "beam size must not exceed 16 (and the pre-beam size 40)");
  const int dk = c.d_model / c.dec_heads;
  SC_CHECK_ARG(c.d_model % c.dec_heads == 0 && (dk == 16 || dk == 32 || (dk == 64 && o->beam_size <= 10)),
               "decoder head dim must be 16, 32 or 64 (64: beam <= 10)");
  SC_CHECK_ARG(c.vocab_size > 1 && c.vocab_size <= SC_MAX_VOCAB,
               "vocabulary larger than SC_MAX_VOCAB (8192): the LDS of the full-vocabulary top-k of sc_fuse_topw");
  HIP_TRY(hipSetDevice(e->device));
  sc_streams *b = new sc_streams;
  b->eng = e;
  b->cfg = c;
  const int S = b->S = o->n_streams, W = b->W = o->beam_size;
  b->K = K;
  b->TCAP = o->max_frames;
  b->LCAP = o->max_tokens;
  b->max_chunk = o->max_chunk_samples > 0 ? o->max_chunk_samples : 32768;
  b->PCAP = o->pcm_capacity > 0 ? o->pcm_capacity : (1 << 20);
  b->use_bbd = o->use_bbd != 0;
  b->strict = o->strict_reference != 0;
  const int d = c.d_model, V = c.vocab_size, F = c.ffn_dim;
  b->max_feat_new = 2 + b->max_chunk / c.hop_length + 8;
  b->FCAP = b->max_feat_new + 16;
  b->UCAP = c.block_size + b->FCAP / 4 + 8;
  b->max_t1 = (b->FCAP - 3) / 2 + 1;
  b->max_t2 = (b->max_t1 - 3) / 2 + 1;
  b->max_blocks = S * (b->UCAP / c.hop_size + 1);
  const int R = c.block_size + 2;
  const size_t m_enc = (size_t)b->max_blocks * R, n = (size_t)S * W;
  int rc = SC_OK;
#define A(ptr, count) if (rc == SC_OK) rc = b->alloc(&ptr, (size_t)(count))
  if (hipStreamCreateWithPriority(&b->stream, hipStreamNonBlocking, -1) != hipSuccess) {
    sc_set_error("sc_streams_create: hipStreamCreate failed");
    delete b;
    return SC_ERR_LAUNCH;
  }
  if (hipStreamCreateWithPriority(&b->stream_rb, hipStreamNonBlocking, -1) != hipSuccess) {
    sc_set_error("sc_streams_create: hipStreamCreate failed");
    delete b;
    return SC_ERR_LAUNCH;
  }
  A(b->pcm, (size_t)S * b->PCAP);
  A(b->featbuf, (size_t)2 * S * b->FCAP * c.n_mels);
  A(b->subbuf, (size_t)2 * S * b->UCAP * d);
  A(b->prev_addin, (size_t)S * d);
  A(b->past_ctx, (size_t)S * c.enc_layers * d);
  A(b->enc, (size_t)S * b->TCAP * d);
  A(b->c1, (size_t)S * b->max_t1 * c.conv_freq1 * d);
  A(b->c2, (size_t)S * b->max_t2 * c.conv_freq2 * d);
  A(b->xblk, m_enc * d);
  A(b->ws_xn, m_enc * d);
  A(b->ws_qkv, m_enc * 3 * d);
  A(b->ws_att, m_enc * d);
  A(b->ws_ffh, m_enc * F);
  A(b->jobs_ctx, (size_t)S * 4);
  A(b->ctrlmap, (size_t)S * 8 + n);
  b->slot_cap = (((size_t)S * ((size_t)b->max_t2 * (c.conv_freq2 + 12) + 512) + 8192) + 63) & ~size_t(63);
  A(b->arena_dev, b->slot_cap * N_ARENA);
  b->bs_cap = (size_t)S * 8 + (size_t)S * c.block_size;
  A(b->bs_dev, b->bs_cap * N_RING);
  b->stage_cap = (size_t)S * std::max<size_t>((size_t)b->max_chunk + 16 * c.hop_length, (size_t)b->max_feat_new * c.n_mels);
  A(b->stage_dev, b->stage_cap * N_STAGE);
  b->pack_cap = n * (2 * (size_t)b->LCAP + 8);
  A(b->pack_dev, b->pack_cap);
  A(b->pjobs_dev, n * 4);
  A(b->cjobs_dev, (size_t)N_STAGE * S * 3);
  A(b->rsjobs_dev, (size_t)N_STAGE * S);
  A(b->rs_hist, (size_t)2 * S * SC_RS_HIST);
  sc_search &sb = b->sb;
  sb.S = S; sb.W = W; sb.K = K; sb.V = V; sb.d = d; sb.H = c.dec_heads; sb.F = F; sb.n_layers = c.dec_layers;
  sb.TCAP = b->TCAP; sb.LCAP = b->LCAP; sb.blank = c.blank_id; sb.eos = c.eos_id; sb.sos = c.sos_id;
  sb.w_dec = 1.0f - o->ctc_weight; sb.w_ctc = o->ctc_weight; sb.ln_eps = c.ln_eps;
  float *ctcx = nullptr, *ckv = nullptr;
  A(ctcx, (size_t)S * b->TCAP * V);
  sb.kv_half = o->kv_half != 0;
  const size_t kvdiv = sb.kv_half ? 2 : 1;
  A(ckv, (size_t)S * c.dec_layers * b->TCAP * 2 * d / kvdiv + 4);
  sb.ctcx = ctcx; sb.ckv = ckv;
  if (sb.kv_half) {
    b->kv_stage_rows = std::max(256, S * 24);
    A(b->kv_stage, (size_t)c.dec_layers * b->kv_stage_rows * 2 * d);
  }
  sb.tct = (b->TCAP + 3) / 4 * 4;
  A(sb.ctcxT, (size_t)S * V * sb.tct);
  {
    const long full = (long)b->LCAP * W;
    long rows = o->kv_pool_rows;
    if (rows <= 0) {
      const long floor_rows = (long)b->LCAP + b->LCAP / 2 + 4 * W;
      size_t free_b = 0, total_b = 0;
      rows = floor_rows;
      if (hipMemGetInfo(&free_b, &total_b) == hipSuccess) {
        const size_t per_row = (size_t)S * c.dec_layers * 2 * d * sizeof(float) / kvdiv;
        const size_t budget = std::min<size_t>(free_b / 4, (size_t)SC_KV_POOL_DEFAULT_MAX_GIB << 30);
        rows = std::max<long>(floor_rows, (long)std::min<size_t>((size_t)full, budget / per_row));
      } else {
        (void)hipGetLastError();
      }
    }
    rows = std::max<long>(std::min(rows, full), 2 * W);
    if (rows > 65536) {
      if (o->kv_pool_rows > 0) {
        sc_set_error("sc_streams_create: the self-attention K|V pool is limited to 65536 rows per stream (max_tokens / kv_pool_rows)");
        delete b;
        return SC_ERR_ARG;
      }
      rows = 65536;
    }
    sb.kv_rows = (int32_t)rows;
  }
  A(sb.skv, (size_t)S * c.dec_layers * sb.kv_rows * 2 * d / kvdiv + 4);
  A(sb.yseq, (size_t)2 * n * b->LCAP);
  A(sb.xpos, (size_t)2 * n * b->LCAP);
  A(sb.anc, (size_t)2 * S * b->LCAP * W);
  A(sb.score, 2 * n); A(sb.sc_dec, 2 * n); A(sb.sc_ctc, 2 * n);
  A(sb.ctc_r, (size_t)2 * S * b->TCAP * 2 * W);
  A(sb.ctc_rs, (size_t)2 * S * b->TCAP * W);
  A(sb.ctc_s, 2 * n);
  A(sb.ctc_rnew, (size_t)S * ((b->TCAP + 15) / 16) * 2 * W * K);
  A(sb.dx, n * d); A(sb.dxn, n * d); A(sb.dqkv, n * 3 * d); A(sb.datt, n * d); A(sb.dq, n * d); A(sb.dffh, n * F);
  A(sb.logits, n * V); A(sb.logp, n * V);
  A(sb.pre_ids, n * K); A(sb.psi, n * K); A(sb.psi_eos, n);
  A(sb.cand_score, n * W); A(sb.cand_tok, n * W); A(sb.cand_ctc, n * W);
  A(sb.sel, n * 2);
  A(b->stat_rows, 3);
  sb.stat_rows = b->stat_rows;
  if (sc_dec_layer_fused_supported(d, c.dec_heads, W, F) && V % d == 0 && e->dec[0].wqkv_pp && e->f("out_w_q", false)) {
    A(sb.ph1, n * c.dec_heads * d);
    A(sb.ph2, n * c.dec_heads * d);
    A(sb.ffn_part, (size_t)(F / 128) * n * d);
    sb.max_ffn_part = F / 128;
  }
  if (rc == SC_OK && hipMalloc(&b->ws, (size_t)128 << 20) != hipSuccess) rc = SC_ERR_LAUNCH;
  if (rc == SC_OK) b->owned.push_back(b->ws);
#undef A
  if (rc != SC_OK) {
    sc_set_error("sc_streams_create: device allocation failed");
    delete b;
    return rc;
  }
  sb.ctrl = b->ctrlmap;
  sb.rowmap = b->ctrlmap + S * 8;
  sb.n_rows = S * W;
  sb.embed = e->f("embed"); sb.pe = e->f("pe"); sb.dec_norm_g = e->f("dec_norm_g"); sb.dec_norm_b = e->f("dec_norm_b");
  sb.out_w = e->f("out_w"); sb.out_b = e->f("out_b"); sb.out_w_q = e->f("out_w_q", false);
  sb.out_w_qh = nullptr;
  sb.act_half = 0;
  if (sb.kv_half && e->f("out_w_qh", false) && !e->dec.empty() && e->dec[0].wqkv_pph && e->dec[0].wq_pph && e->dec[0].wo_pph &&
      e->dec[0].wo2_pph && sb.ph1) {
    sb.out_w_qh = e->f("out_w_qh", false);
    sb.act_half = 1 | 2;
    if (const char *ah = sc_hook("SC_ACT_HALF")) sb.act_half = atoi(ah) & 7;
  }
  sb.layers = e->dec.data();
  (void)sc_set_stream_workspace(b->stream, b->ws, (size_t)128 << 20);
  b->es = b->stream;
  {
    b->enc_start_thr = S < 16 ? S : std::max(1, (int)((long)S * 7 / 100));
  }
  {
    const hipError_t er = hipStreamCreateWithPriority(&b->stream_enc, hipStreamNonBlocking, 0);
    if (er == hipSuccess && hipMalloc(&b->ws_enc, (size_t)128 << 20) == hipSuccess) {
      b->owned.push_back(b->ws_enc);
      (void)sc_set_stream_workspace(b->stream_enc, b->ws_enc, (size_t)128 << 20);
    } else {
      (void)hipGetLastError();
      if (b->stream_enc) (void)hipStreamDestroy(b->stream_enc);
      b->stream_enc = nullptr;
    }
  }
  const size_t cm = ((size_t)S * 8 + n) * sizeof(int32_t);
  bool ok = b->halloc(&b->ctrlmap_host, (size_t)S * 8 + n) == SC_OK && b->halloc(&b->flags_host, (size_t)S * 2) == SC_OK &&
            b->halloc(&b->rm_host[0], n) == SC_OK && b->halloc(&b->rm_host[1], n) == SC_OK &&
            b->halloc(&b->arena_host, b->slot_cap * N_ARENA) == SC_OK && b->halloc(&b->bs_host, b->bs_cap * N_RING) == SC_OK &&
            b->halloc(&b->stage_host, b->stage_cap * N_STAGE) == SC_OK && b->halloc(&b->pack_host, b->pack_cap) == SC_OK &&
            b->halloc(&b->pjobs_host, n * 4) == SC_OK && b->halloc(&b->cjobs_host, (size_t)N_STAGE * S * 3) == SC_OK &&
            b->halloc(&b->rsjobs_host, (size_t)N_STAGE * S) == SC_OK;
  for (int i = 0; i < 2 && ok; ++i) ok = hipEventCreateWithFlags(&b->ev_iter[i], hipEventDisableTiming) == hipSuccess;
  for (int i = 0; i < N_ARENA && ok; ++i) ok = hipEventCreateWithFlags(&b->ev_group[i], hipEventDisableTiming) == hipSuccess;
  for (int i = 0; i < N_STAGE && ok; ++i) ok = hipEventCreateWithFlags(&b->ev_stage[i], hipEventDisableTiming) == hipSuccess;
  if (!ok) {
    sc_set_error("sc_streams_create: pinned host allocation failed");
    delete b;
    return SC_ERR_LAUNCH;
  }
  memset(b->flags_host, 0, (size_t)S * 8);
  {
    void *dv = nullptr;
    if (hipHostGetDevicePointer(&dv, b->flags_host, 0) != hipSuccess || !dv) {
      sc_set_error("sc_streams_create: pinned flags are not device-accessible");
      delete b;
      return SC_ERR_LAUNCH;
    }
    b->ring_dev = (int32_t *)dv;
    sb.flags = b->ring_dev;
    sb.kvflags = b->ring_dev + S;
  }
  if (const char *sp = sc_hook("SC_SCAN_SPLIT_MIN")) b->scan_split_min = atoi(sp);
  memset(b->ctrlmap_host, 0, cm);
  for (size_t i = 0; i < n; ++i) b->rm_host[0][i] = b->rm_host[1][i] = (int32_t)i;
  (void)hipMemcpy(b->ctrlmap, b->ctrlmap_host, (size_t)S * 8 * sizeof(int32_t), hipMemcpyHostToDevice);
  (void)hipMemcpy(b->ctrlmap + S * 8, b->rm_host[0], n * sizeof(int32_t), hipMemcpyHostToDevice);
  b->rowmap_key.resize(S);
  for (int s = 0; s < S; ++s) b->rowmap_key[s] = s;
  b->enc_batch_min = std::max(1, S / 2);
  b->gemm_flags = (!b->eng->enc.empty() && b->eng->enc[0].wqkv_s) ? SC_GEMM_SPLIT16 : 0;
  b->row_bucket = std::max(1, S / 32);
  b->n_rows_step = S * W;
  b->st.assign(S, St());
  b->run.assign(S, Run());
  b->bq.assign(S, std::deque<Blk>());
  b->job.assign(S, Job());
  b->ahead.assign(S, std::deque<Job>());
  b->job_seq.assign(S, 0);
  b->snap.assign(S, Snap());
  b->done_at.assign(S, 0);
  b->fault_msg.assign(S, std::string());
  b->enc_gen.assign(S, 0);
  for (int s = 0; s < S; ++s) init_hyp(b, s);
  *out = b;
  return SC_OK;
  SC_API_END
}

extern "C" void sc_streams_destroy(sc_streams *b) {
  if (b) {
    (void)hipStreamSynchronize(b->stream);
    if (b->stream_enc) (void)hipStreamSynchronize(b->stream_enc);
    delete b;
  }
}

extern "C" int sc_reset(sc_streams *b, int stream) {
  SC_CHECK_ARG(b && stream >= 0 && stream < b->S, "stream out of range");
  SC_CHECK_ARG(!b->job[stream].open, "the stream has a chunk outstanding (sc_poll reports it first)");
  reset_stream(b, stream);
  return SC_OK;
}

extern "C" int sc_stream_set_input_rate(sc_streams *b, int stream, int rate) {
  SC_CHECK_ARG(b && stream >= 0 && stream < b->S, "stream out of range");
  SC_API_BEGIN
  const St &cur = b->st[stream];
  SC_CHECK_ARG(!b->job[stream].open && b->ahead[stream].empty(), "the stream has a chunk outstanding (sc_poll reports it first)");
  SC_CHECK_ARG(cur.pcm_end == 0 && !cur.fe_started && !cur.enc_started && !cur.started && cur.rs_in == 0,
               "the stream has buffered audio since its last reset (sc_reset first)");
  int L, M, Wc;
  if (!sc_rs_params(rate, &L, &M, &Wc)) {
    sc_set_error("sc_stream_set_input_rate: unsupported input rate %d (supported: 8000..48000 Hz with 16000 / gcd(rate, 16000) <= 640)", rate);
    return SC_ERR_ARG;
  }
  int t = -1;
  if (rate != 16000) {
    for (int i = 0; i < b->n_rs_tabs; ++i)
      if (b->rs_rate[i] == rate) t = i;
    if (t < 0) {
      SC_CHECK_ARG(b->n_rs_tabs < SC_RS_MAX_TABS, "at most 8 distinct input rates per sc_streams");
      HIP_TRY(hipSetDevice(b->eng->device));
      std::vector<float> host((size_t)L * 2 * Wc);
      RC_TRY(sc_resample_design(rate, nullptr, nullptr, nullptr, host.data()));
      float *dev = nullptr;
      RC_TRY(b->alloc(&dev, host.size()));
      HIP_TRY(hipMemcpy(dev, host.data(), host.size() * sizeof(float), hipMemcpyHostToDevice));
      t = b->n_rs_tabs++;
      b->rs_rate[t] = rate;
      b->rs_tabs.coef[t] = dev;
      b->rs_tabs.L[t] = L; b->rs_tabs.M[t] = M; b->rs_tabs.Wc[t] = Wc;
    }
  }
  b->st[stream].rs_tab = t;
  return SC_OK;
  SC_API_END
}

extern "C" int sc_stream_set_decoder(sc_streams *b, int stream, int mode) {
  SC_CHECK_ARG(b && stream >= 0 && stream < b->S, "stream out of range");
  SC_API_BEGIN
  SC_CHECK_ARG(mode == SC_DECODER_FULL || mode == SC_DECODER_NONE, "mode is neither SC_DECODER_FULL nor SC_DECODER_NONE");
  const St &cur = b->st[stream];
  SC_CHECK_ARG(!b->job[stream].open && b->ahead[stream].empty(), "the stream has a chunk outstanding (sc_poll reports it first)");
  SC_CHECK_ARG(cur.pcm_end == 0 && !cur.fe_started && !cur.enc_started && !cur.started && cur.rs_in == 0,
               "the stream has buffered audio since its last reset (sc_reset first)");
  b->st[stream].no_dec = mode == SC_DECODER_NONE;
  return SC_OK;
  SC_API_END
}

extern "C" int sc_stream_decoder(const sc_streams *b, int stream) {
  if (!b || stream < 0 || stream >= b->S) return SC_ERR_ARG;
  return b->st[stream].no_dec ? SC_DECODER_NONE : SC_DECODER_FULL;
}

extern "C" int sc_stream_input_rate(const sc_streams *b, int stream) {
  SC_CHECK_ARG(b && stream >= 0 && stream < b->S, "stream out of range");
  return b->st[stream].rs_tab < 0 ? 16000 : b->rs_rate[b->st[stream].rs_tab];
}

extern "C" int sc_stream_set_input_format(sc_streams *b, int stream, int format, int channels, int channel, int scale) {
  SC_CHECK_ARG(b && stream >= 0 && stream < b->S, "stream out of range");
  SC_API_BEGIN
  const St &cur = b->st[stream];
  SC_CHECK_ARG(!b->job[stream].open && b->ahead[stream].empty(), "the stream has a chunk outstanding (sc_poll reports it first)");
  SC_CHECK_ARG(cur.pcm_end == 0 && !cur.fe_started && !cur.enc_started && !cur.started && cur.rs_in == 0,
               "the stream has buffered audio since its last reset (sc_reset first)");
  SC_CHECK_ARG(format >= 0 && format < SC_PCM_N_FORMATS, "format out of range (SC_PCM_*)");
  SC_CHECK_ARG(channels >= 1 && channels <= SC_PCM_MAX_CHANNELS, "channels outside 1..8");
  SC_CHECK_ARG(channel >= SC_PCM_MIX && channel < channels, "channel outside [-1, channels)");
  const bool b15 = format == SC_PCM_S16LE || format == SC_PCM_MULAW || format == SC_PCM_ALAW;
  SC_CHECK_ARG(scale == SC_PCM_SCALE_FULL || (scale == SC_PCM_SCALE_SERVER && b15),
               "scale: SC_PCM_SCALE_FULL, or SC_PCM_SCALE_SERVER with S16LE / MULAW / ALAW");
  const bool coded = format != SC_PCM_F32 || channels != 1;
  if (coded && !b->lvl_state) {
    HIP_TRY(hipSetDevice(b->eng->device));
    const size_t S = b->S;
    b->stageb_cap = b->stage_cap * sizeof(float);
    if (!b->stageb_dev) RC_TRY(b->alloc(&b->stageb_dev, b->stageb_cap * N_STAGE));
    if (!b->stageb_host) RC_TRY(b->halloc(&b->stageb_host, b->stageb_cap * N_STAGE));
    if (!b->pcmjobs_dev) RC_TRY(b->alloc(&b->pcmjobs_dev, S * N_STAGE));
    if (!b->pcmjobs_host) RC_TRY(b->halloc(&b->pcmjobs_host, S * N_STAGE));
    if (!b->lvl_out_dev) RC_TRY(b->halloc_mapped(&b->lvl_out_host, &b->lvl_out_dev, S * N_STAGE, __func__, "level slots"));
    b->lvl.init(b->S);
    RC_TRY(b->alloc(&b->lvl_state, S));
  }
  St &st = b->st[stream];
  st.in_fmt = format; st.in_ch = channels; st.in_sel = channel; st.in_scale = scale;
  return SC_OK;
  SC_API_END
}

extern "C" int sc_stream_input_format(const sc_streams *b, int stream, int *format, int *channels, int *channel, int *scale) {
  SC_CHECK_ARG(b && stream >= 0 && stream < b->S, "stream out of range");
  const St &st = b->st[stream];
  if (format) *format = st.in_fmt;
  if (channels) *channels = st.in_ch;
  if (channel) *channel = st.in_sel;
  if (scale) *scale = st.in_scale;
  return SC_OK;
}

extern "C" int sc_stream_input_level(sc_streams *b, int stream, sc_input_level_t *out) {
  SC_CHECK_ARG(b && stream >= 0 && stream < b->S && out, "stream out of range / null");
  SC_API_BEGIN
  *out = sc_input_level_t{0, 0, 0, 0, 0};
  if (!b->lvl_state) return SC_OK;
  const handover::Pending<LevelState> &r = b->lvl.rep[stream];
  if (!r.ready) {
    HIP_TRY(hipSetDevice(b->eng->device));
    for (int i = 0; i < N_STAGE && !r.ready; ++i)
      for (const sc_streams::LvlSpan &sp : b->stage_lvl[i])
        if (sp.s == stream && sp.ticket == r.key) {
          RC_TRY(collect_levels(b, i, true));
          break;
        }
  }
  if (!r.ready) {
    sc_set_error("input level of stream %d did not arrive with its staging step (internal error)", stream);
    return SC_ERR_LAUNCH;
  }
  *out = r.v;
  return SC_OK;
  SC_API_END
}

extern "C" int sc_stage_bench(int rate, int n_jobs, int n_in, int iters, double *ms) {
  SC_CHECK_ARG(n_jobs > 0 && n_jobs <= 4096 && n_in > 0 && n_in <= (1 << 20) && iters > 0 && ms, "bad arguments");
  SC_API_BEGIN
  int L = 1, M = 1, Wc = 0;
  SC_CHECK_ARG(sc_rs_params(rate, &L, &M, &Wc), "unsupported rate");
  const bool copy = rate == 16000;
  const long n_before = 3L * n_in, m0 = copy ? 0 : sc_rs_out_count(L, M, Wc, n_before, false);
  const long n_out = copy ? n_in : sc_rs_out_count(L, M, Wc, n_before + n_in, false) - m0;
  const long row = n_out + 16;
  std::vector<float> x((size_t)n_jobs * n_in), h((size_t)2 * n_jobs * SC_RS_HIST);
  unsigned r = 12345u;
  for (float &v : x) v = ((r = r * 1664525u + 1013904223u) >> 8) * (1.0f / 8388608.0f) - 1.0f;
  for (float &v : h) v = ((r = r * 1664525u + 1013904223u) >> 8) * (1.0f / 8388608.0f) - 1.0f;
  std::vector<long long> cj((size_t)n_jobs * 3);
  std::vector<sc_rs_job> rj(n_jobs);
  for (int j = 0; j < n_jobs; ++j) {
    cj[j * 3] = (long long)j * n_in; cj[j * 3 + 1] = (long long)j * row; cj[j * 3 + 2] = n_in;
    rj[j] = sc_rs_job{(long long)j * n_in, n_in, (long long)j * row, n_out, m0, n_before, 0, j, 0, 0};
  }
  float *src = nullptr, *dst = nullptr, *hist = nullptr, *tab = nullptr;
  long long *cjd = nullptr;
  sc_rs_job *rjd = nullptr;
  hipStream_t st = nullptr;
  hipEvent_t e0 = nullptr, e1 = nullptr;
  std::vector<float> coef((size_t)L * 2 * Wc);
  if (!copy) RC_TRY(sc_resample_design(rate, nullptr, nullptr, nullptr, coef.data()));
  auto cleanup = [&]() {
    for (void *p : {(void *)src, (void *)dst, (void *)hist, (void *)tab, (void *)cjd, (void *)rjd})
      if (p) (void)hipFree(p);
    if (e0) (void)hipEventDestroy(e0);
    if (e1) (void)hipEventDestroy(e1);
    if (st) (void)hipStreamDestroy(st);
  };
  sc_rs_tabs tabs{};
  int rc = SC_OK;
  auto run = [&]() -> int {
    RC_TRY(dalloc(&src, x.size()));
    RC_TRY(dalloc(&dst, (size_t)n_jobs * row));
    RC_TRY(dalloc(&hist, h.size()));
// ... 860 lines not shown
  return SC_OK;
  SC_API_END
}

extern "C" int sc_streams_write_pcm(sc_streams *b, int stream, long offset, const float *host, long n) {
  SC_CHECK_ARG(b && host && stream >= 0 && stream < b->S && offset >= 0 && n >= 0 && offset + n <= b->PCAP, "out of range");
  HIP_TRY(hipMemcpy(b->pcm + (long)stream * b->PCAP + offset, host, (size_t)n * sizeof(float), hipMemcpyHostToDevice));
  return SC_OK;
}
static int settle_encoder(sc_streams *b) {
  RC_TRY(tick_collect(b));
  RC_TRY(launch_pending_groups(b));
  if (b->stream_enc) HIP_TRY(hipStreamSynchronize(b->stream_enc));
  HIP_TRY(hipStreamSynchronize(b->stream));
  return retire_groups(b);
}
extern "C" long sc_streams_read_pcm_buffer(sc_streams *b, int stream, float *host, long max_n) {
  if (!b || stream < 0 || stream >= b->S) return SC_ERR_ARG;
  if (settle_encoder(b) != SC_OK) return SC_ERR_LAUNCH;
  const St &st = b->st[stream];
  const long n = std::min<long>(st.pcm_end - st.pcm_start, max_n);
  if (host && n > 0 &&
      hipMemcpy(host, b->pcm + (long)stream * b->PCAP + st.pcm_start, (size_t)n * sizeof(float), hipMemcpyDeviceToHost) != hipSuccess)
    return SC_ERR_LAUNCH;
  return n;
}
extern "C" int sc_streams_read_enc(sc_streams *b, int stream, float *host, int max_frames) {
  if (!b || stream < 0 || stream >= b->S) return SC_ERR_ARG;
  if (settle_encoder(b) != SC_OK) return SC_ERR_LAUNCH;
  const int T = std::min(b->st[stream].T_enc, max_frames);
  if (host && T > 0 &&
      hipMemcpy(host, b->enc + (size_t)stream * b->TCAP * b->cfg.d_model, (size_t)T * b->cfg.d_model * sizeof(float),
                hipMemcpyDeviceToHost) != hipSuccess)
    return SC_ERR_LAUNCH;
  return T;
}

extern "C" int sc_streams_read_ctc(sc_streams *b, int stream, float *host, int max_rows) {
  SC_CHECK_ARG(b && stream >= 0 && stream < b->S && max_rows >= 0, "bad arguments");
  SC_API_BEGIN
  HIP_TRY(hipSetDevice(b->eng->device));
  int T = 0;
  bool snap = false;
  RC_TRY(hyp_frames(b, stream, &T, &snap));
  T = std::min(T, max_rows);
  const size_t V = (size_t)b->cfg.vocab_size;
  if (host && T > 0) {
    HIP_TRY(hipMemcpyAsync(host, b->sb.ctcx + (size_t)stream * b->TCAP * V, (size_t)T * V * sizeof(float),
                           hipMemcpyDeviceToHost, b->stream_rb));
    HIP_TRY(hipStreamSynchronize(b->stream_rb));
  }
  return T;
  SC_API_END
}

extern "C" int sc_streams_read_ctc_projected(sc_streams *b, int stream, float *host, int max_rows) {
  SC_CHECK_ARG(b && stream >= 0 && stream < b->S && max_rows >= 0, "bad arguments");
  SC_API_BEGIN
  HIP_TRY(hipSetDevice(b->eng->device));
  RC_TRY(launch_pending_groups(b));
  HIP_TRY(hipStreamSynchronize(b->es));
  const int T = std::min(std::min(b->st[stream].T_proj, b->TCAP), max_rows);
  const size_t V = (size_t)b->cfg.vocab_size;
  if (host && T > 0)
    HIP_TRY(hipMemcpy(host, b->sb.ctcx + (size_t)stream * b->TCAP * V, (size_t)T * V * sizeof(float), hipMemcpyDeviceToHost));
  return T;
  SC_API_END
}

extern "C" int sc_streams_set_activity(sc_streams *b, int on, double blank_threshold) {
  SC_CHECK_ARG(b, "null");
  SC_API_BEGIN
  SC_CHECK_ARG(b->n_open == 0, "chunks are outstanding");
  if (!on) {
    b->act_on = false;
    return SC_OK;
  }
  SC_CHECK_ARG(blank_threshold > 0.0 && blank_threshold < 1.0, "blank_threshold must lie in (0, 1)");
  HIP_TRY(hipSetDevice(b->eng->device));
  if (!b->act_state) {
    const size_t S = (size_t)b->S;
    RC_TRY(b->alloc(&b->act_state, S * 6));
    RC_TRY(b->alloc(&b->act_track, S * b->TCAP));
    RC_TRY(b->alloc(&b->act_jobs_dev, S * N_ARENA));
    RC_TRY(b->halloc(&b->act_jobs_host, S * N_ARENA));
    RC_TRY(b->halloc_mapped(&b->act_out_host, &b->act_out_dev, S * N_ARENA * 6, __func__, "state slots"));
    b->act.init(b->S);
  }
  b->act.restart_all();
  b->act_thr = blank_threshold;
  b->act_on = true;
  return SC_OK;
  SC_API_END
}

template <typename V>
static int side_ready(sc_streams *b, const handover::Pending<V> &r, int s, const char *what, const char *whose) {
  if (r.ready) return SC_OK;
  RC_TRY(wait_group(b, r.key));
  if (!r.ready) {
    sc_set_error("%s of stream %d did not arrive with %s encoder group (internal error)", what, s, whose);
    return SC_ERR_LAUNCH;
  }
  return SC_OK;
}
static int activity_ready(sc_streams *b, int s) { return side_ready(b, b->act.rep[s], s, "activity state", "its"); }
static int spot_ready(sc_streams *b, int s) { return side_ready(b, b->spot.rep[s], s, "spotting counters", "their"); }
static int draft_ready(sc_streams *b, int s) { return side_ready(b, b->draft.rep[s], s, "draft state", "its"); }
static int beam_ready(sc_streams *b, int s) { return side_ready(b, b->beam.rep[s], s, "beam state", "its"); }

extern "C" int sc_stream_activity(sc_streams *b, int stream, sc_activity_t *out) {
  SC_CHECK_ARG(b && out && stream >= 0 && stream < b->S, "bad arguments");
  SC_API_BEGIN
  SC_CHECK_ARG(b->act_on, "the activity option is off (sc_streams_set_activity)");
  HIP_TRY(hipSetDevice(b->eng->device));
  RC_TRY(activity_ready(b, stream));
  const int32_t *v = b->act.rep[stream].v.v;
  out->n_frames = v[0]; out->n_speech = v[1]; out->n_bad = v[2];
  out->first_speech = v[3]; out->last_speech = v[4]; out->trail_silence = v[5];
  return SC_OK;
  SC_API_END
}

extern "C" int sc_streams_read_activity(sc_streams *b, int stream, double *host, int max_frames) {
  SC_CHECK_ARG(b && stream >= 0 && stream < b->S && max_frames >= 0, "bad arguments");
  SC_API_BEGIN
  SC_CHECK_ARG(b->act_on, "the activity option is off (sc_streams_set_activity)");
  HIP_TRY(hipSetDevice(b->eng->device));
  RC_TRY(activity_ready(b, stream));
  const int T = std::min(b->act.rep[stream].v.T, max_frames);
  if (host && T > 0) {
    HIP_TRY(hipMemcpyAsync(host, b->act_track + (size_t)stream * b->TCAP, (size_t)T * sizeof(double), hipMemcpyDeviceToHost,
                           b->stream_rb));
    HIP_TRY(hipStreamSynchronize(b->stream_rb));
  }
  return T;
  SC_API_END
}

extern "C" int sc_streams_set_phrases(sc_streams *b, const int32_t *labels, const int32_t *lens, const double *min_scores,
                                      int n_phrases) {
  SC_CHECK_ARG(b, "null");
  SC_API_BEGIN
  SC_CHECK_ARG(b->n_open == 0, "chunks are outstanding");
  SC_CHECK_ARG(n_phrases >= 0 && n_phrases <= SC_SPOT_MAX_PHRASES, "a phrase set holds 0..64 phrases");
  if (n_phrases == 0) {
    b->spot_on = false;
    return SC_OK;
  }
  SC_CHECK_ARG(labels && lens && min_scores, "null phrase set");
  const int V = b->cfg.vocab_size, blank = b->cfg.blank_id;
  std::vector<int32_t> lab((size_t)SC_SPOT_MAX_PHRASES * SC_SPOT_MAX_LEN, 0), len(SC_SPOT_MAX_PHRASES, 0);
  std::vector<double> fl(SC_SPOT_MAX_PHRASES, 0.0);
  for (int p = 0; p < n_phrases; ++p) {
    SC_CHECK_ARG(lens[p] >= 1 && lens[p] <= SC_SPOT_MAX_LEN, "a phrase has 1..32 labels");
    SC_CHECK_ARG(min_scores[p] <= 0.0, "min_score must be <= 0");
    for (int i = 0; i < lens[p]; ++i) {
      const int32_t y = labels[(size_t)p * SC_SPOT_MAX_LEN + i];
      SC_CHECK_ARG(y >= 0 && y < V && y != blank, "a label outside the vocabulary or equal to the blank");
      lab[(size_t)p * SC_SPOT_MAX_LEN + i] = y;
    }
    len[p] = lens[p];
    fl[p] = min_scores[p];
  }
  HIP_TRY(hipSetDevice(b->eng->device));
  if (!b->spot_counters) {
    const size_t S = (size_t)b->S, PS = (size_t)SC_SPOT_MAX_PHRASES * SC_SPOT_STATES;
    RC_TRY(b->alloc(&b->spot_labels, lab.size()));
    RC_TRY(b->alloc(&b->spot_lens, len.size()));
    RC_TRY(b->alloc(&b->spot_floors, fl.size()));
    RC_TRY(b->alloc(&b->spot_counters, S * 2));
    RC_TRY(b->alloc(&b->spot_values, S * PS));
    RC_TRY(b->alloc(&b->spot_starts, S * PS));
    RC_TRY(b->alloc(&b->spot_events, S * SC_SPOT_MAX_EVENTS));
    RC_TRY(b->alloc(&b->spot_jobs_dev, S * N_ARENA));
    RC_TRY(b->halloc(&b->spot_jobs_host, S * N_ARENA));
    RC_TRY(b->halloc_mapped(&b->spot_out_host, &b->spot_out_dev, S * N_ARENA * 2, __func__, "counter slots"));
    b->spot.init(b->S);
  }
  HIP_TRY(hipStreamSynchronize(b->es));
  HIP_TRY(hipMemcpy(b->spot_labels, lab.data(), lab.size() * sizeof(int32_t), hipMemcpyHostToDevice));
  HIP_TRY(hipMemcpy(b->spot_lens, len.data(), len.size() * sizeof(int32_t), hipMemcpyHostToDevice));
  HIP_TRY(hipMemcpy(b->spot_floors, fl.data(), fl.size() * sizeof(double), hipMemcpyHostToDevice));
  b->spot.restart_all();
  b->spot_mask.assign(b->S, ~0ull);
  b->spot_P = n_phrases;
  b->spot_on = true;
  return SC_OK;
  SC_API_END
}

extern "C" int sc_stream_set_phrase_mask(sc_streams *b, int stream, uint64_t mask) {
  SC_CHECK_ARG(b && stream >= 0 && stream < b->S, "bad arguments");
  SC_CHECK_ARG(b->spot_on, "the spotting option is off (sc_streams_set_phrases)");
  b->spot_mask[stream] = mask;
  return SC_OK;
}

extern "C" int sc_stream_spot(sc_streams *b, int stream, sc_spot_t *out) {
  SC_CHECK_ARG(b && out && stream >= 0 && stream < b->S, "bad arguments");
  SC_API_BEGIN
  SC_CHECK_ARG(b->spot_on, "the spotting option is off (sc_streams_set_phrases)");
  HIP_TRY(hipSetDevice(b->eng->device));
  RC_TRY(spot_ready(b, stream));
  out->n_frames = b->spot.rep[stream].v.v[0];
  out->n_events = b->spot.rep[stream].v.v[1];
  return SC_OK;
  SC_API_END
}

extern "C" int sc_streams_read_spot_events(sc_streams *b, int stream, sc_spot_event *host, int max) {
  SC_CHECK_ARG(b && stream >= 0 && stream < b->S && max >= 0, "bad arguments");
  SC_API_BEGIN
  SC_CHECK_ARG(b->spot_on, "the spotting option is off (sc_streams_set_phrases)");
  HIP_TRY(hipSetDevice(b->eng->device));
  RC_TRY(spot_ready(b, stream));
  const int n = std::min(std::min((int)b->spot.rep[stream].v.v[1], SC_SPOT_MAX_EVENTS), max);
  if (host && n > 0) {
    HIP_TRY(hipMemcpyAsync(host, b->spot_events + (size_t)stream * SC_SPOT_MAX_EVENTS, (size_t)n * sizeof(sc_spot_event),
                           hipMemcpyDeviceToHost, b->stream_rb));
    HIP_TRY(hipStreamSynchronize(b->stream_rb));
  }
  return n;
  SC_API_END
}

extern "C" int sc_streams_read_spot_state(sc_streams *b, int stream, double *values, int32_t *starts) {
  SC_CHECK_ARG(b && stream >= 0 && stream < b->S && values && starts, "bad arguments");
  SC_API_BEGIN
  SC_CHECK_ARG(b->spot_on, "the spotting option is off (sc_streams_set_phrases)");
  HIP_TRY(hipSetDevice(b->eng->device));
  RC_TRY(launch_pending_groups(b));
  HIP_TRY(hipStreamSynchronize(b->es));
  const size_t n = (size_t)b->spot_P * SC_SPOT_STATES, o = (size_t)stream * SC_SPOT_MAX_PHRASES * SC_SPOT_STATES;
  if (b->spot.fresh[stream]) {
    for (size_t i = 0; i < n; ++i) { values[i] = -INFINITY; starts[i] = -1; }
    return b->spot_P;
  }
  HIP_TRY(hipMemcpy(values, b->spot_values + o, n * sizeof(double), hipMemcpyDeviceToHost));
  HIP_TRY(hipMemcpy(starts, b->spot_starts + o, n * sizeof(int32_t), hipMemcpyDeviceToHost));
  return b->spot_P;
  SC_API_END
}

extern "C" int sc_streams_set_draft(sc_streams *b, int on) {
  SC_CHECK_ARG(b, "null");
  SC_API_BEGIN
  SC_CHECK_ARG(b->n_open == 0, "chunks are outstanding");
  if (!on) {
    b->draft_on = false;
    return SC_OK;
  }
  HIP_TRY(hipSetDevice(b->eng->device));
  if (!b->draft_state) {
    const size_t S = (size_t)b->S;
    RC_TRY(b->alloc(&b->draft_state, S));
    RC_TRY(b->alloc(&b->draft_tokens, S * b->TCAP));
    RC_TRY(b->alloc(&b->draft_jobs_dev, S * N_ARENA));
    RC_TRY(b->halloc(&b->draft_jobs_host, S * N_ARENA));
    RC_TRY(b->halloc_mapped(&b->draft_out_host, &b->draft_out_dev, S * N_ARENA, __func__, "state slots"));
    b->draft.init(b->S);
  }
  b->draft.restart_all();
  b->draft_on = true;
  return SC_OK;
  SC_API_END
}

extern "C" int sc_stream_draft(sc_streams *b, int stream, sc_draft_t *out) {
  SC_CHECK_ARG(b && out && stream >= 0 && stream < b->S, "bad arguments");
  SC_API_BEGIN
  SC_CHECK_ARG(b->draft_on, "the draft option is off (sc_streams_set_draft)");
  HIP_TRY(hipSetDevice(b->eng->device));
  RC_TRY(draft_ready(b, stream));
  *out = b->draft.rep[stream].v.d;
  return SC_OK;
  SC_API_END
}

extern "C" int sc_streams_read_draft(sc_streams *b, int stream, sc_draft_token *host, int max) {
  SC_CHECK_ARG(b && stream >= 0 && stream < b->S && max >= 0, "bad arguments");
  SC_API_BEGIN
  SC_CHECK_ARG(b->draft_on, "the draft option is off (sc_streams_set_draft)");
  HIP_TRY(hipSetDevice(b->eng->device));
  RC_TRY(draft_ready(b, stream));
  const sc_draft_t &v = b->draft.rep[stream].v.d;
  int n = std::min(std::min((int)v.n_closed, b->TCAP), max);
  if (host && n > 0) {
    HIP_TRY(hipMemcpyAsync(host, b->draft_tokens + (size_t)stream * b->TCAP, (size_t)n * sizeof(sc_draft_token),
                           hipMemcpyDeviceToHost, b->stream_rb));
    HIP_TRY(hipStreamSynchronize(b->stream_rb));
  }
  if (host && v.open_id >= 0 && n < max) {
    sc_draft_token &t = host[n++];
    t.id = v.open_id; t.start = v.open_start; t.end = v.open_end; t.reserved = 0; t.conf = v.open_conf;
  }
  return n;
  SC_API_END
}

extern "C" int sc_streams_set_ctc_beam(sc_streams *b, int beam, int candidates) {
  SC_CHECK_ARG(b, "null");
  SC_API_BEGIN
  SC_CHECK_ARG(b->n_open == 0, "chunks are outstanding");
  if (!beam) {
    b->beam_on = false;
    if (b->beam_gr_n) {
      HIP_TRY(hipSetDevice(b->eng->device));
      RC_TRY(launch_pending_groups(b));
      HIP_TRY(hipStreamSynchronize(b->es));
      for (sc_grammar *&g : b->beam_gr) {
        if (g) (void)sc_grammar_use(g, -1);
        g = nullptr;
      }
      b->beam_gr_n = 0;
    }
    if (b->beam_lm) {
      HIP_TRY(hipSetDevice(b->eng->device));
      HIP_TRY(hipStreamSynchronize(b->es));
      b->beam_lm = nullptr;
      b->beam_lm_view = nullptr;
    }
    return SC_OK;
  }
  SC_CHECK_ARG(beam >= 1 && beam <= SC_BEAM_MAX && candidates >= 1 && candidates <= SC_BEAM_MAX,
               "beam and candidates must lie in [1, SC_BEAM_MAX]");
  SC_CHECK_ARG(1 + (size_t)beam * b->TCAP <= 0x7fffffffu, "the node store exceeds 2^31 records");
  HIP_TRY(hipSetDevice(b->eng->device));
  if (!b->beam_state) {
    const size_t S = (size_t)b->S;
    RC_TRY(b->alloc(&b->beam_state, S));
    RC_TRY(b->alloc(&b->beam_jobs_dev, S * N_ARENA));
    RC_TRY(b->halloc(&b->beam_jobs_host, S * N_ARENA));
    RC_TRY(b->halloc_mapped(&b->beam_out_host, &b->beam_out_dev, S * N_ARENA, __func__, "state slots"));
    b->beam.init(b->S);
  }
  if (beam > b->beam_nodes_B) {
    HIP_TRY(hipStreamSynchronize(b->es));
    if (b->beam_nodes) (void)hipFree(b->beam_nodes);
    b->beam_nodes = nullptr;
    b->beam_nodes_B = 0;
    RC_TRY(dalloc(&b->beam_nodes, (size_t)b->S * (1 + (size_t)beam * b->TCAP)));
    b->beam_nodes_B = beam;
  }
  b->beam.restart_all();
  b->beam_B = beam;
  b->beam_C = candidates;
  b->beam_on = true;
  return SC_OK;
  SC_API_END
}

extern "C" int sc_streams_set_ctc_beam_lm(sc_streams *b, const sc_lm *lm, double alpha, double beta) {
  SC_CHECK_ARG(b, "null");
  SC_API_BEGIN
  SC_CHECK_ARG(b->n_open == 0, "chunks are outstanding");
  HIP_TRY(hipSetDevice(b->eng->device));
  if (!lm) {
    if (!b->beam_lm) return SC_OK;
    HIP_TRY(hipStreamSynchronize(b->es));
    b->beam_lm = nullptr;
    b->beam_lm_view = nullptr;
    b->beam.restart_all();
    return SC_OK;
  }
  SC_CHECK_ARG(b->beam_on, "the beam option is off (sc_streams_set_ctc_beam)");
  SC_CHECK_ARG(b->beam_gr_n == 0, "a stream has a grammar (sc_stream_set_grammar): grammar and model together are not served");
  SC_CHECK_ARG(std::isfinite(alpha) && std::isfinite(beta), "alpha and beta must be finite");
  sc_lm_view info;
  const sc_lm_view *view = nullptr;
  RC_TRY(sc_lm_device_view(lm, &view, &info));
  SC_CHECK_ARG(view && info.V == b->cfg.vocab_size, "the model's vocabulary size is not the batch's");
  if (!b->beam_lm_state) {
    const size_t S = (size_t)b->S;
    RC_TRY(b->alloc(&b->beam_lm_state, S));
    RC_TRY(b->alloc(&b->beam_lm_jobs_dev, S * N_ARENA));
    RC_TRY(b->halloc(&b->beam_lm_jobs_host, S * N_ARENA));
    RC_TRY(b->halloc_mapped(&b->beam_lm_out_host, &b->beam_lm_out_dev, S * N_ARENA, __func__, "state slots"));
  }
  HIP_TRY(hipStreamSynchronize(b->es));
  b->beam.restart_all();
  b->beam_lm = lm;
  b->beam_lm_view = view;
  b->beam_lm_info = info;
  b->beam_alpha = alpha;
  b->beam_beta = beta;
  return SC_OK;
  SC_API_END
}

extern "C" int sc_stream_ctc_beam_lm(sc_streams *b, int stream, sc_beam_lm_t *out) {
  SC_CHECK_ARG(b && out && stream >= 0 && stream < b->S, "bad arguments");
  SC_API_BEGIN
  SC_CHECK_ARG(b->beam_on && b->beam_lm, "no language model is attached (sc_streams_set_ctc_beam_lm)");
  HIP_TRY(hipSetDevice(b->eng->device));
  RC_TRY(beam_ready(b, stream));
  const BeamState &v = b->beam.rep[stream].v;
  *out = v.lm;
  if (v.d.n_frames == 0) out->ctx[0] = b->beam_lm_info.start_state;
  return SC_OK;
  SC_API_END
}

extern "C" int sc_ctc_beam_hyps_lm(sc_streams *b, const int *stream_ids, int n, int nbest, double *lm, double *fused) {
  SC_CHECK_ARG(b && stream_ids && n >= 0 && nbest >= 0 && nbest <= SC_BEAM_MAX, "bad arguments");
  SC_API_BEGIN
  SC_CHECK_ARG(b->beam_on && b->beam_lm, "no language model is attached (sc_streams_set_ctc_beam_lm)");
  SC_CHECK_ARG(n <= b->S, "more streams listed than the batch has");
  HIP_TRY(hipSetDevice(b->eng->device));
  for (int i = 0; i < n; ++i) {
    const int s = stream_ids[i];
    SC_CHECK_ARG(s >= 0 && s < b->S, "stream out of range");
    RC_TRY(beam_ready(b, s));
    const BeamState &v = b->beam.rep[s].v;
    for (int r = 0; r < nbest; ++r) {
      const size_t k = (size_t)i * nbest + r;
      double l = NAN, f = NAN;
      if (r < v.d.n_entries) {
        const sc_beam_entry &e = v.d.e[r];
        const double hi = std::max(e.pb, e.pnb), lo = std::min(e.pb, e.pnb);
        const double total = lo == -INFINITY ? hi : hi + log1p(exp(lo - hi));
        l = v.lm.lm[r];
        const double wa = b->beam_alpha * l, wb = b->beam_beta * (double)e.len;
        f = total + (wa + wb);
      }
      if (lm) lm[k] = l;
      if (fused) fused[k] = f;
    }
  }
  return SC_OK;
  SC_API_END
}

extern "C" int sc_stream_set_grammar(sc_streams *b, int stream, sc_grammar *grammar) {
  SC_CHECK_ARG(b && stream >= 0 && stream < b->S, "stream out of range");
  SC_API_BEGIN
  const St &cur = b->st[stream];
  SC_CHECK_ARG(!b->job[stream].open && b->ahead[stream].empty(), "the stream has a chunk outstanding (sc_poll reports it first)");
  SC_CHECK_ARG(cur.pcm_end == 0 && !cur.fe_started && !cur.enc_started && !cur.started && cur.rs_in == 0,
               "the stream has buffered audio since its last reset (sc_reset first)");
  sc_grammar *old = b->beam_gr_n ? b->beam_gr[stream] : nullptr;
  if (grammar == old) return SC_OK;
  HIP_TRY(hipSetDevice(b->eng->device));
  if (grammar) {
    SC_CHECK_ARG(b->beam_on, "the beam option is off (sc_streams_set_ctc_beam)");
    SC_CHECK_ARG(!b->beam_lm, "a language model is attached (sc_streams_set_ctc_beam_lm): grammar and model together are not served");
    sc_grammar_view info;
    RC_TRY(sc_grammar_device_view(grammar, nullptr, &info));
    SC_CHECK_ARG(info.V == b->cfg.vocab_size && info.blank == b->cfg.blank_id,
                 "the grammar's vocabulary size or blank is not the batch's");
    if (!b->beam_gr_state) {
      const size_t S = (size_t)b->S;
      RC_TRY(b->alloc(&b->beam_gr_state, S));
      RC_TRY(b->alloc(&b->beam_gr_jobs_dev, S * N_ARENA));
      RC_TRY(b->halloc(&b->beam_gr_jobs_host, S * N_ARENA));
      RC_TRY(b->halloc_mapped(&b->beam_gr_out_host, &b->beam_gr_out_dev, S * N_ARENA, __func__, "state slots"));
    }
    if (b->beam_gr.empty()) b->beam_gr.assign((size_t)b->S, nullptr);
  }
  if (old) {
    RC_TRY(launch_pending_groups(b));
    HIP_TRY(hipStreamSynchronize(b->es));
    (void)sc_grammar_use(old, -1);
    b->beam_gr_n--;
  }
  if (grammar) {
    RC_TRY(sc_grammar_use(grammar, 1) > 0 ? SC_OK : SC_ERR_ARG);
    b->beam_gr_n++;
  }
  b->beam_gr[stream] = grammar;
  b->beam.restart(stream);
  return SC_OK;
  SC_API_END
}

extern "C" int sc_stream_ctc_beam_grammar(sc_streams *b, int stream, sc_beam_gr_t *out) {
  SC_CHECK_ARG(b && out && stream >= 0 && stream < b->S, "bad arguments");
  SC_API_BEGIN
  SC_CHECK_ARG(b->beam_on && b->beam_gr_n && b->beam_gr[stream], "the stream has no grammar (sc_stream_set_grammar)");
  HIP_TRY(hipSetDevice(b->eng->device));
  RC_TRY(beam_ready(b, stream));
  const BeamState &v = b->beam.rep[stream].v;
  *out = v.gr;
  if (v.d.n_frames == 0) {
    sc_grammar_view info;
    RC_TRY(sc_grammar_device_view(b->beam_gr[stream], nullptr, &info));
    out->g[0] = info.start_state;
  }
  return SC_OK;
  SC_API_END
}

extern "C" int sc_ctc_beam_hyps_grammar(sc_streams *b, const int *stream_ids, int n, int nbest, int32_t *g, int32_t *accept) {
  SC_CHECK_ARG(b && stream_ids && n >= 0 && nbest >= 0 && nbest <= SC_BEAM_MAX, "bad arguments");
  SC_API_BEGIN
  SC_CHECK_ARG(b->beam_on, "the beam option is off (sc_streams_set_ctc_beam)");
  SC_CHECK_ARG(n <= b->S, "more streams listed than the batch has");
  HIP_TRY(hipSetDevice(b->eng->device));
  for (int i = 0; i < n; ++i) {
    const int s = stream_ids[i];
    SC_CHECK_ARG(s >= 0 && s < b->S, "stream out of range");
    RC_TRY(beam_ready(b, s));
    const BeamState &v = b->beam.rep[s].v;
    const sc_grammar *gr = b->beam_gr_n ? b->beam_gr[s] : nullptr;
    sc_grammar_view info{};
    if (gr) RC_TRY(sc_grammar_device_view(gr, nullptr, &info));
    for (int r = 0; r < nbest; ++r) {
      const size_t k = (size_t)i * nbest + r;
      int32_t st = -1;
      if (gr && r < v.d.n_entries) st = v.d.n_frames == 0 ? info.start_state : v.gr.g[r];
      if (g) g[k] = st;
      if (accept) accept[k] = st < 0 ? -1 : sc_grammar_accepts(gr, st);
    }
  }
  return SC_OK;
  SC_API_END
}

extern "C" int sc_stream_ctc_beam(sc_streams *b, int stream, sc_beam_t *out) {
  SC_CHECK_ARG(b && out && stream >= 0 && stream < b->S, "bad arguments");
  SC_API_BEGIN
  SC_CHECK_ARG(b->beam_on, "the beam option is off (sc_streams_set_ctc_beam)");
  HIP_TRY(hipSetDevice(b->eng->device));
  RC_TRY(beam_ready(b, stream));
  *out = b->beam.rep[stream].v.d;
  return SC_OK;
  SC_API_END
}

extern "C" int sc_ctc_beam_hyps(sc_streams *b, const int *stream_ids, int n, int nbest, int max_len, int32_t *header,
                                int32_t *ids, int32_t *frames, double *scores) {
  SC_CHECK_ARG(b && stream_ids && header && n >= 0 && nbest >= 0 && nbest <= SC_BEAM_MAX && max_len >= 0, "bad arguments");
  SC_API_BEGIN
  SC_CHECK_ARG(b->beam_on, "the beam option is off (sc_streams_set_ctc_beam)");
  SC_CHECK_ARG(n <= b->S, "more streams listed than the batch has");
  HIP_TRY(hipSetDevice(b->eng->device));
  const size_t m = (size_t)n * nbest;
  if (m == 0) return SC_OK;
// ... 305 lines not shown
      ar_copy_out(b->ar_host + o_out + (size_t)job_of[i] * AR_OUT, (size_t)i, nbest, n_hyps[i], order, fused, att, status);
  return SC_OK;
  SC_API_END
}

extern "C" int sc_stream_info(const sc_streams *b, int stream, sc_stream_info_t *out) {
  SC_CHECK_ARG(b && out && stream >= 0 && stream < b->S, "bad arguments");
  const St &st = b->st[stream];
  out->enc_frames = st.T_enc;
  out->processed_block = st.processed_block;
  out->process_idx = st.process_idx;
  out->n_hyp = st.started ? st.nhyp : 0;
  out->hyp_len = st.L;
  out->decode_steps = st.n_steps_total;
  out->pcm_buffered = (int32_t)(st.pcm_end - st.pcm_start);
  out->frontend_started = st.fe_started;
  return SC_OK;
}

extern "C" int sc_streams_set_graphs(sc_streams *b, int on) {
  SC_CHECK_ARG(b, "null");
  b->use_graphs = on != 0;
  return SC_OK;
}
extern "C" int sc_streams_kv_rows(const sc_streams *b) { return b ? b->sb.kv_rows : 0; }

extern "C" long sc_streams_take_xattn_rows(sc_streams *b) {
  if (!b) return 0;
  const long v = b->xattn_rows[0] + b->xattn_rows[1] + b->xattn_rows[2];
  b->xattn_rows[0] = b->xattn_rows[1] = b->xattn_rows[2] = 0;
  return v;
}
extern "C" int sc_streams_take_xattn_rows_by_kernel(sc_streams *b, long *rows) {
  SC_CHECK_ARG(b && rows, "null");
  for (int i = 0; i < 3; ++i) {
    rows[i] = b->xattn_rows[i];
    b->xattn_rows[i] = 0;
  }
  return SC_OK;
}

extern "C" int sc_streams_take_attn_counters(sc_streams *b, long *out) {
  SC_CHECK_ARG(b && out, "null");
  unsigned long long dr[3] = {0, 0, 0};
  HIP_TRY(hipSetDevice(b->eng->device));
  HIP_TRY(hipStreamSynchronize(b->stream));
  HIP_TRY(hipMemcpy(dr, b->stat_rows, sizeof dr, hipMemcpyDeviceToHost));
  HIP_TRY(hipMemset(b->stat_rows, 0, sizeof dr));
  for (int i = 0; i < 3; ++i) {
    out[i] = b->xattn_rows[i];
    out[3 + i] = b->sattn_pos[i];
    out[6 + i] = (long)dr[i];
    b->xattn_rows[i] = b->sattn_pos[i] = 0;
  }
  return SC_OK;
}

extern "C" int sc_streams_bucket_times(sc_streams *b, double *seconds, long *iterations) {
  SC_CHECK_ARG(b && seconds && iterations, "null");
  for (int i = 0; i < 17; ++i) {
    seconds[i] = b->t_bucket[i];
    iterations[i] = b->n_bucket[i];
    b->t_bucket[i] = 0;
    b->n_bucket[i] = 0;
  }
  return SC_OK;
}

extern "C" int sc_streams_host_times(sc_streams *b, double *launch_s, double *wait_s) {
  SC_CHECK_ARG(b && launch_s && wait_s, "null");
  *launch_s = b->t_launch;
  *wait_s = b->t_wait;
  b->t_launch = b->t_wait = 0;
  return SC_OK;
}

extern "C" int sc_streams_capture_stats(const sc_streams *b, long *n_captures, double *seconds) {
  SC_CHECK_ARG(b && n_captures && seconds, "null");
  *n_captures = b->n_enc_captures;
  *seconds = b->t_enc_capture;
  return SC_OK;
}

extern "C" int sc_streams_stats(const sc_streams *b, long *enc_calls, long *dec_steps, long *dec_blocks) {
  SC_CHECK_ARG(b, "null");
  if (enc_calls) *enc_calls = b->enc_calls;
  if (dec_steps) *dec_steps = b->dec_steps;
  if (dec_blocks) *dec_blocks = b->dec_blocks;
  return SC_OK;
}
```

### speechcatcher_amd/native.py

```python
import ctypes as C
from typing import Optional, Sequence, Tuple

import numpy as np
import torch

from . import _abi
from .config import SearchConfig
from .engine import EngineError
from .weights import PackedWeights

_ERR_CAPACITY, _ERR_INPUT = -3, -4


class NativeEngine:

    def __init__(self, weights: Optional[PackedWeights] = None, packed_path: Optional[str] = None, device="cuda:0"):
        self.lib = _abi.load()
        self.device = torch.device(device)
        h = C.c_void_p()
        if packed_path is not None:
            _abi.check(self.lib.sc_engine_load(str(packed_path).encode(), self.device.index or 0, C.byref(h)),
                       "sc_engine_load")
            self.weights = None
        else:
# ... 8 lines not shown
            for i, (n, t) in enumerate(ts):
                arr[i].name, arr[i].data, arr[i].numel = self._names[i], t.data_ptr(), t.numel()
                arr[i].dtype = {torch.float64: 1, torch.float16: 2}.get(t.dtype, 0)
            _abi.check(self.lib.sc_engine_create(C.byref(c), arr, len(ts), self.device.index or 0, C.byref(h)),
                       "sc_engine_create")
        self.handle = h

    def close(self):
        if getattr(self, "handle", None):
            self.lib.sc_engine_destroy(self.handle)
            self.handle = None

    def __del__(self):
        try:
            self.close()
        except Exception:
            pass


class _Info:
    __slots__ = ("_b", "_s")
    _MAP = {"T_enc": "enc_frames", "processed_block": "processed_block", "process_idx": "process_idx",
            "L": "hyp_len", "nhyp": "n_hyp", "n_steps_total": "decode_steps", "fe_started": "frontend_started",
            "pcm_buffered": "pcm_buffered"}

    def __init__(self, b, s):
        self._b, self._s = b, s

    def __getattr__(self, name):
        info = _abi.StreamInfo()
        _abi.check(self._b.lib.sc_stream_info(self._b.handle, self._s, C.byref(info)), "sc_stream_info")
        v = getattr(info, self._MAP[name])
        return bool(v) if name == "fe_started" else int(v)


class _InfoList:
    def __init__(self, b):
        self._b = b

    def __getitem__(self, s):
        return _Info(self._b, s)

    def __iter__(self):
        return (_Info(self._b, s) for s in range(self._b.S))

    def __len__(self):
        return self._b.S


class NativeStreamBatch:

    def __init__(self, weights, n_streams: int, search: SearchConfig = SearchConfig(), max_frames: int = 1600,
                 max_tokens: int = 640, pcm_capacity: int = 1 << 20, max_chunk_samples: int = 32768,
                 strict_reference: bool = True, engine: Optional[NativeEngine] = None, kv_dtype: str = "float32",
                 kv_pool_rows: int = 0):
        if not torch.cuda.is_available():
            raise _abi.ScasrError("NativeStreamBatch needs a ROCm GPU (torch.cuda.is_available() is False)")
        self.engine = engine or NativeEngine(weights, device=weights.device)
        self.lib = self.engine.lib
        self.w, self.cfg, self.search = weights, (weights.cfg if weights is not None else None), search
        self.S, self.W = n_streams, search.beam_size
        self.TCAP, self.LCAP, self.PCAP = max_frames, max_tokens, pcm_capacity
        self.strict_reference = strict_reference
        if search.pre_beam != 40 or search.max_length != 500:
            raise EngineError("the native engine implements the reference's constants: pre-beam 40, max_length 500")
        o = _abi.StreamOptions(n_streams, search.beam_size, search.ctc_weight, int(search.use_bbd), max_frames,
                               max_tokens, pcm_capacity, max_chunk_samples, int(strict_reference),
                               {"float32": 0, "float16": 1}[kv_dtype], int(kv_pool_rows))
        self.kv_dtype = kv_dtype
        h = C.c_void_p()
        try:
            _abi.check(self.lib.sc_streams_create(self.engine.handle, C.byref(o), C.byref(h)), "sc_streams_create")
        except _abi.ScasrError as e:
            raise EngineError(str(e)) from e
        self.handle = h
        self.st = _InfoList(self)
        self._coded = {}

    @property
    def stats(self):
        a, b, c = C.c_long(), C.c_long(), C.c_long()
        self.lib.sc_streams_stats(self.handle, C.byref(a), C.byref(b), C.byref(c))
        return {"enc_calls": a.value, "dec_steps": b.value, "dec_blocks": c.value}

    def _fault(self, s, code):
        msg = (self.lib.sc_stream_last_error(self.handle, int(s)) or b"").decode()
        return (RuntimeError if code == _ERR_INPUT else EngineError)(f"stream {s}: {msg}")

    @staticmethod
    def _marshal(ids, ptrs, counts, finals):
        n = len(ids)
        return ((C.c_int32 * n)(*ids), (C.c_void_p * n)(*ptrs), (C.c_int32 * n)(*counts),
                (C.c_uint8 * n)(*[1 if f else 0 for f in finals]))

    def _call(self, fn, ids, ptrs, counts, finals, keep, isolate_faults):
        n = len(ids)
        a_ids, a_ptr, a_cnt, a_fin = self._marshal(ids, ptrs, counts, finals)
        status = (C.c_int32 * n)()
        try:
            _abi.check(getattr(self.lib, fn)(self.handle, a_ids, a_ptr, a_cnt, a_fin, n, status), fn)
        except _abi.ScasrError as e:
            raise EngineError(str(e)) from e
        del keep
        out = {}
        for i, s in enumerate(ids):
            if status[i] >= 0:
                out[s] = bool(status[i])
                continue
            exc = self._fault(s, status[i])
            if not isolate_faults:
                raise exc
            out[s] = exc
        return out

    def _gather(self, chunks, pcm_resident):
        ids, ptrs, counts, finals, keep = [], [], [], [], []
        for s, samples, fin in chunks:
            ids.append(int(s))
            finals.append(bool(fin))
            if pcm_resident:
                ptrs.append(None)
                counts.append(int(samples))
            elif int(s) in self._coded:
                a, n = self._coded_bytes(int(s), samples)
                keep.append(a)
                ptrs.append(a.ctypes.data if a.size else None)
                counts.append(n)
            else:
                if isinstance(samples, torch.Tensor):
                    samples = samples.detach().cpu().numpy()
                a = np.ascontiguousarray(samples, dtype=np.float32)
                keep.append(a)
                ptrs.append(a.ctypes.data)
                counts.append(int(a.shape[0]))
        return ids, ptrs, counts, finals, keep

    def _coded_bytes(self, s, samples):
        from . import pcm
        fmt, channels, _, _ = self._coded[s]
        if isinstance(samples, torch.Tensor):
            samples = samples.detach().cpu().numpy()
        if isinstance(samples, np.ndarray) and samples.dtype.kind == "f" and not (fmt == pcm.F32 and samples.dtype == np.float32):
            raise EngineError(f"stream {s} has input format {pcm.NAME_OF[fmt]}: it takes the coded bytes, not {samples.dtype} samples")
        a = np.ascontiguousarray(pcm.as_bytes(samples))
        bpf = pcm.bytes_per_frame(fmt, channels)
        if a.size % bpf:
            raise EngineError(f"stream {s}: {a.size} bytes are not a whole number of {bpf}-byte frames")
        return a, a.size // bpf

    def push(self, chunks: Sequence[Tuple[int, Optional[np.ndarray], bool]], pcm_resident: bool = False,
             isolate_faults: bool = False):
        ids, ptrs, counts, finals, keep = self._gather(chunks, pcm_resident)
        fn = "sc_push_raw" if any(s in self._coded for s in ids) else "sc_push"
        return self._call(fn, ids, ptrs, counts, finals, keep, isolate_faults)

    def push_raw(self, chunks, isolate_faults: bool = False):
        ids, ptrs, counts, finals, keep = self._gather(chunks, False)
        return self._call("sc_push_raw", ids, ptrs, counts, finals, keep, isolate_faults)

    def push_block(self, stream_ids: np.ndarray, pcm: np.ndarray, finals: Optional[np.ndarray] = None) -> np.ndarray:
        n, m = pcm.shape
        assert pcm.dtype == np.float32 and pcm.flags.c_contiguous and len(stream_ids) == n
        ids = np.ascontiguousarray(stream_ids, dtype=np.int32)
        ptrs = (pcm.ctypes.data + np.arange(n, dtype=np.uint64) * np.uint64(m * 4)).astype(np.uint64)
        cnt = np.full(n, m, np.int32)
        fin = np.zeros(n, np.uint8) if finals is None else np.ascontiguousarray(finals, dtype=np.uint8)
# ... 666 lines not shown
```

Before: 4071.

## Batch job-table uploads into one coalesced H2D copy per encoder group

Job tables for the encoder and CTC side jobs used to be written into separate host/device buffers, each with its own hipMemcpyAsync. They now go into one shared arena slot, and each upload is deferred until just before the next kernel launch so consecutive tables go up as one contiguous copy. Resample and PCM job headers move into the staging buffer header so they travel with the payload. This aims to cut per-chunk memcpy launches and host overhead. The cost is a larger arena and a more complex staging and launch split, plus new copy-count counters.

```diff
diff --git a/include/scasr.h b/include/scasr.h
--- a/include/scasr.h
+++ b/include/scasr.h
@@ -719,6 +719,7 @@
 int sc_streams_kv_rows(const sc_streams *streams);
 int sc_streams_stats(const sc_streams *streams, long *enc_calls, long *dec_steps, long *dec_blocks);
 int sc_streams_capture_stats(const sc_streams *streams, long *n_captures, double *seconds);
+int sc_streams_copy_stats(const sc_streams *streams, long *group_uploads, long *groups, long *tick_uploads, long *ticks);
 int sc_streams_set_graphs(sc_streams *streams, int on);
 int sc_marker(int id, void *stream);
 int sc_streams_host_times(sc_streams *streams, double *launch_s, double *wait_s);
diff --git a/speechcatcher_amd/_abi.py b/speechcatcher_amd/_abi.py
--- a/speechcatcher_amd/_abi.py
+++ b/speechcatcher_amd/_abi.py
@@ -364,6 +364,8 @@
     "sc_stream_info": (C.c_int, [vp, C.c_int, C.POINTER(StreamInfo)]),
     "sc_streams_stats": (C.c_int, [vp, C.POINTER(C.c_long), C.POINTER(C.c_long), C.POINTER(C.c_long)]),
     "sc_streams_capture_stats": (C.c_int, [vp, C.POINTER(C.c_long), c_double_p]),
+    "sc_streams_copy_stats": (C.c_int, [vp, C.POINTER(C.c_long), C.POINTER(C.c_long), C.POINTER(C.c_long),
+                                        C.POINTER(C.c_long)]),
     "sc_streams_set_graphs": (C.c_int, [vp, C.c_int]),
     "sc_marker": (C.c_int, [C.c_int, vp]),
     "sc_streams_host_times": (C.c_int, [vp, c_double_p, c_double_p]),
diff --git a/speechcatcher_amd/csrc/streams.hip b/speechcatcher_amd/csrc/streams.hip
--- a/speechcatcher_amd/csrc/streams.hip
+++ b/speechcatcher_amd/csrc/streams.hip
@@ -5,6 +5,7 @@
 #include <cstdarg>
 #include <cstring>
 #include <deque>
+#include <functional>
 #include <map>
 #include <memory>
 #include <new>
@@ -14,6 +15,7 @@
 #include "common.h"
 #include "handover.h"
 #include "resample.h"
+#include "table_arena.h"
 
 namespace {
 
@@ -242,8 +244,9 @@
   sc_search sb{};
   int32_t *ctrlmap_host = nullptr, *flags_host = nullptr;
   int32_t *arena_host = nullptr, *arena_dev = nullptr;
-  size_t slot_cap = 0, arena_off = 0;
-  int cur_slot = 0;
+  size_t slot_cap = 0;
+  table_arena::Slot tab;
+  long n_group_uploads = 0, n_groups_launched = 0, n_tick_uploads = 0, n_ticks = 0;
   hipEvent_t ev_group[N_ARENA] = {nullptr};
   long slot_gen[N_ARENA] = {0};
   int32_t *bs_host = nullptr, *bs_dev = nullptr;
@@ -251,18 +254,20 @@
   int bs_i = 0;
   float *stage_host = nullptr, *stage_dev = nullptr;
   size_t stage_cap = 0;
+  size_t stage_hdr = 0, hdr_rs = 0, hdr_pcm = 0;
+  size_t stage_base(int slot) const { return (size_t)slot * (stage_hdr + stage_cap); }
+  size_t stage_pay(int slot) const { return stage_base(slot) + stage_hdr; }
+  template <typename T> T *hdr_host(int slot, size_t byte_off) { return (T *)((char *)(stage_host + stage_base(slot)) + byte_off); }
+  template <typename T> T *hdr_dev(int slot, size_t byte_off) { return (T *)((char *)(stage_dev + stage_base(slot)) + byte_off); }
   hipEvent_t ev_stage[N_STAGE] = {nullptr};
   bool stage_busy[N_STAGE] = {false};
   int stage_next = 0;
-  long long *cjobs_host = nullptr, *cjobs_dev = nullptr;
-  sc_rs_job *rsjobs_host = nullptr, *rsjobs_dev = nullptr;
   float *rs_hist = nullptr;
   sc_rs_tabs rs_tabs{};
   int rs_rate[SC_RS_MAX_TABS] = {0};
   int n_rs_tabs = 0;
   uint8_t *stageb_host = nullptr, *stageb_dev = nullptr;
   size_t stageb_cap = 0;
-  sc_pcm_job *pcmjobs_host = nullptr, *pcmjobs_dev = nullptr;
   sc_input_level_t *lvl_state = nullptr;
   sc_input_level_t *lvl_out_host = nullptr, *lvl_out_dev = nullptr;
   struct LvlSpan { int s; long epoch, ticket; };
@@ -280,7 +285,6 @@
   double act_thr = 0.8;
   int32_t *act_state = nullptr;
   double *act_track = nullptr;
-  sc_ctc_activity_job *act_jobs_host = nullptr, *act_jobs_dev = nullptr;
   int32_t *act_out_host = nullptr, *act_out_dev = nullptr;
   handover::Track<ActState> act;
   bool spot_on = false;
@@ -291,14 +295,12 @@
   double *spot_values = nullptr;
   int32_t *spot_starts = nullptr;
   sc_spot_event *spot_events = nullptr;
-  sc_ctc_spot_job *spot_jobs_host = nullptr, *spot_jobs_dev = nullptr;
   int32_t *spot_out_host = nullptr, *spot_out_dev = nullptr;
   handover::Track<SpotState> spot;
   std::vector<uint64_t> spot_mask;
   bool draft_on = false;
   sc_draft_t *draft_state = nullptr;
   sc_draft_token *draft_tokens = nullptr;
-  sc_ctc_draft_job *draft_jobs_host = nullptr, *draft_jobs_dev = nullptr;
   sc_draft_t *draft_out_host = nullptr, *draft_out_dev = nullptr;
   handover::Track<DraftState> draft;
   bool beam_on = false;
@@ -306,7 +308,6 @@
   int beam_nodes_B = 0;
   sc_beam_t *beam_state = nullptr;
   sc_beam_node *beam_nodes = nullptr;
-  sc_ctc_beam_job *beam_jobs_host = nullptr, *beam_jobs_dev = nullptr;
   sc_beam_t *beam_out_host = nullptr, *beam_out_dev = nullptr;
   handover::Track<BeamState> beam;
   const sc_lm *beam_lm = nullptr;
@@ -314,12 +315,10 @@
   sc_lm_view beam_lm_info{};
   double beam_alpha = 0.0, beam_beta = 0.0;
   sc_beam_lm_t *beam_lm_state = nullptr;
-  sc_ctc_beam_lm_job *beam_lm_jobs_host = nullptr, *beam_lm_jobs_dev = nullptr;
   sc_beam_lm_t *beam_lm_out_host = nullptr, *beam_lm_out_dev = nullptr;
   std::vector<sc_grammar *> beam_gr;
   int beam_gr_n = 0;
   sc_beam_gr_t *beam_gr_state = nullptr;
-  sc_ctc_beam_gr_job *beam_gr_jobs_host = nullptr, *beam_gr_jobs_dev = nullptr;
   sc_beam_gr_t *beam_gr_out_host = nullptr, *beam_gr_out_dev = nullptr;
   char *bh_dev = nullptr, *bh_host = nullptr;
   size_t bh_cap = 0;
@@ -432,20 +431,31 @@
   int32_t *ctrl_host() { return ctrlmap_host; }
   int32_t *rowmap_host() { return rm_host[rm_idx]; }
 
+  int table(size_t n_bytes, void **host, const void **dev) {
+    const size_t off = tab.reserve(n_bytes);
+    if (off == (size_t)-1) {
+      sc_set_error("job-table arena exhausted (%zu + %zu of %zu entries)", tab.off, n_bytes / sizeof(int32_t), slot_cap);
+      return SC_ERR_ARG;
+    }
+    *host = arena_host + off;
+    *dev = arena_dev + off;
+    return SC_OK;
+  }
   int itensor(const std::vector<int32_t> &a, const int32_t **out) {
-    const size_t n = a.size();
-    if (arena_off + n > slot_cap) {
-      sc_set_error("job-table arena exhausted (%zu + %zu of %zu entries)", arena_off, n, slot_cap);
-      return SC_ERR_ARG;
-    }
-    const size_t off = (size_t)cur_slot * slot_cap + arena_off;
-    arena_off += (n + 63) & ~size_t(63);
-    if (n) {
-      memcpy(arena_host + off, a.data(), n * sizeof(int32_t));
-      HIP_TRY(hipMemcpyAsync(arena_dev + off, arena_host + off, n * sizeof(int32_t), hipMemcpyHostToDevice, es));
-    }
-    *out = arena_dev + off;
+    void *h = nullptr;
+    const void *d = nullptr;
+    RC_TRY(table(a.size() * sizeof(int32_t), &h, &d));
+    if (!a.empty()) memcpy(h, a.data(), a.size() * sizeof(int32_t));
+    *out = (const int32_t *)d;
     return SC_OK;
+  }
+  int flush_tables() {
+    if (!tab.dirty()) return SC_OK;
+    return tab.flush([&](size_t first, size_t n) -> int {
+      ++n_group_uploads;
+      HIP_TRY(hipMemcpyAsync(arena_dev + first, arena_host + first, n * sizeof(int32_t), hipMemcpyHostToDevice, es));
+      return SC_OK;
+    });
   }
 };
 
@@ -754,80 +764,109 @@
   return sc_graph_launch(it->second, b->es);
 }
 
-int encode_short(sc_streams *b, const EncPlan::Short &sh) {
+#define ENC_LAUNCH(call)          \
+  do {                            \
+    RC_TRY(b->flush_tables());    \
+    RC_TRY(call);                 \
+  } while (0)
+
+struct ShortTabs { const int32_t *jd = nullptr, *src = nullptr, *dst = nullptr; };
+
+int encode_short_stage(sc_streams *b, const EncPlan::Short &sh, ShortTabs &T) {
+  const int U = sh.U;
+  RC_TRY(b->itensor({sh.ubase, U, sh.pe_pos, 0, 1, 0}, &T.jd));
+  std::vector<int32_t> a(U), d(U);
+  for (int i = 0; i < U; ++i) { a[i] = i; d[i] = sh.s * b->TCAP + sh.dst_T + i; }
+  RC_TRY(b->itensor(a, &T.src));
+  RC_TRY(b->itensor(d, &T.dst));
+  return SC_OK;
+}
+
+int encode_short(sc_streams *b, const EncPlan::Short &sh, const ShortTabs &T) {
   const sc_config &c = b->cfg;
   sc_engine *e = b->eng;
   const int U = sh.U;
-  const int32_t *jd, *src, *dst;
-  RC_TRY(b->itensor({sh.ubase, U, sh.pe_pos, 0, 1, 0}, &jd));
-  RC_TRY(sc_block_pack(b->subbuf, jd, 1, U, e->f("pe"), c.d_model, b->xblk, b->es));
-  RC_TRY(sc_encoder_layers(e->enc.data(), (int)e->enc.size(), b->xblk, 1, U, 0, nullptr, 0, b->past_ctx, b->ws_xn,
-                           b->ws_qkv, b->ws_att, b->ws_ffh, c.d_model, c.enc_heads, c.ffn_dim, c.ln_eps, b->es));
-  std::vector<int32_t> a(U), d(U);
-  for (int i = 0; i < U; ++i) { a[i] = i; d[i] = sh.s * b->TCAP + sh.dst_T + i; }
-  RC_TRY(b->itensor(a, &src));
-  RC_TRY(b->itensor(d, &dst));
-  RC_TRY(sc_layernorm(b->xblk, src, c.d_model, b->enc, dst, c.d_model, U, c.d_model, e->f("enc_norm_g"), e->f("enc_norm_b"),
-                      c.ln_eps, b->es));
-  return SC_OK;
-}
-
-int encode_launch(sc_streams *b, EncPlan &P) {
+  const int32_t *jd = T.jd, *src = T.src, *dst = T.dst;
+  ENC_LAUNCH(sc_block_pack(b->subbuf, jd, 1, U, e->f("pe"), c.d_model, b->xblk, b->es));
+  ENC_LAUNCH(sc_encoder_layers(e->enc.data(), (int)e->enc.size(), b->xblk, 1, U, 0, nullptr, 0, b->past_ctx, b->ws_xn,
+                               b->ws_qkv, b->ws_att, b->ws_ffh, c.d_model, c.enc_heads, c.ffn_dim, c.ln_eps, b->es));
+  ENC_LAUNCH(sc_layernorm(b->xblk, src, c.d_model, b->enc, dst, c.d_model, U, c.d_model, e->f("enc_norm_g"), e->f("enc_norm_b"),
+                          c.ln_eps, b->es));
+  return SC_OK;
+}
+
+struct EncTabs {
+  const int32_t *cj = nullptr, *ar = nullptr, *ld = nullptr, *fa = nullptr, *fz = nullptr, *bj = nullptr, *ja = nullptr,
+                *ea = nullptr, *ez = nullptr, *sa = nullptr, *sz = nullptr;
+  const int32_t *jc_host = nullptr;
+  int nbk = 0, ns = 0;
+  std::vector<ShortTabs> shorts;
+};
+
+int encode_stage(sc_streams *b, EncPlan &P, EncTabs &T) {
   const sc_config &c = b->cfg;
-  sc_engine *e = b->eng;
-  const int d = c.d_model, F1 = c.conv_freq1, F2 = c.conv_freq2, R = c.block_size + 2;
-  b->enc_calls++;
-  const int32_t *cj, *ar, *ld;
-  RC_TRY(b->itensor(P.conv_jobs, &cj));
-  RC_TRY(sc_conv1(b->featbuf, c.n_mels, cj, P.n_conv, P.max_t1, e->f("conv1_w"), e->f("conv1_b"), d, b->c1, b->es));
-  RC_TRY(b->itensor(P.a_rows, &ar));
-  RC_TRY(sc_gemm(b->c1, ar, d, e->f("conv2_w"), e->f("conv2_b"), b->c2, nullptr, d, (int)P.a_rows.size(), d, 9 * d,
-                 SC_GEMM_RELU | b->gemm_flags, F1, b->es));
-  RC_TRY(b->itensor(P.lin_dst, &ld));
-  RC_TRY(sc_gemm(b->c2, nullptr, F2 * d, e->f("sub_out_w"), e->f("sub_out_b"), b->subbuf, ld, d, (int)P.lin_dst.size(), d,
-                 F2 * d, b->gemm_flags, 0, b->es));
+  RC_TRY(b->itensor(P.conv_jobs, &T.cj));
+  RC_TRY(b->itensor(P.a_rows, &T.ar));
+  RC_TRY(b->itensor(P.lin_dst, &T.ld));
   if (!P.feat_src.empty()) {
-    const int32_t *a, *z;
-    RC_TRY(b->itensor(P.feat_src, &a));
-    RC_TRY(b->itensor(P.feat_dst, &z));
-    RC_TRY(sc_copy_rows(b->featbuf, a, b->featbuf, z, (int)P.feat_src.size(), c.n_mels, b->es));
-  }
-  const int nbk = (int)P.blk_jobs.size() / 6, ns = (int)P.sjobs.size() / 5;
-  if (nbk > 0) {
-    if (nbk > b->max_blocks) {
+    RC_TRY(b->itensor(P.feat_src, &T.fa));
+    RC_TRY(b->itensor(P.feat_dst, &T.fz));
+  }
+  T.nbk = (int)P.blk_jobs.size() / 6;
+  T.ns = (int)P.sjobs.size() / 5;
+  if (T.nbk > 0) {
+    if (T.nbk > b->max_blocks) {
       sc_set_error("sc_push: too many encoder blocks in one call");
       return SC_ERR_ARG;
     }
-    const int32_t *bj, *ja;
-    RC_TRY(b->itensor(P.blk_jobs, &bj));
-    RC_TRY(sc_block_pack(b->subbuf, bj, nbk, R, e->f("pe"), d, b->xblk, b->es));
+    RC_TRY(b->itensor(P.blk_jobs, &T.bj));
+    const int ns = T.ns;
     std::vector<int32_t> j_add(ns * 4), j_ctx(ns * 4);
     for (int i = 0; i < ns; ++i) {
       const int32_t *sj = &P.sjobs[i * 5];
       j_add[i * 4 + 0] = sj[0]; j_add[i * 4 + 1] = sj[1]; j_add[i * 4 + 2] = sj[2]; j_add[i * 4 + 3] = sj[3];
       j_ctx[i * 4 + 0] = sj[0]; j_ctx[i * 4 + 1] = sj[1]; j_ctx[i * 4 + 2] = sj[2] * c.enc_layers; j_ctx[i * 4 + 3] = sj[4];
     }
-    RC_TRY(b->itensor(j_add, &ja));
-    RC_TRY(sc_ctx_handoff(b->xblk, R, ja, ns, b->prev_addin, 0, d, b->es));
+    RC_TRY(b->itensor(j_add, &T.ja));
     const int32_t *jc;
     RC_TRY(b->itensor(j_ctx, &jc));
-    HIP_TRY(hipMemcpyAsync(b->jobs_ctx, jc, j_ctx.size() * sizeof(int32_t), hipMemcpyDeviceToDevice, b->es));
-    RC_TRY(enc_layers_launch(b, nbk, R, true, b->jobs_ctx, ns));
+    T.jc_host = b->arena_host + (jc - b->arena_dev);
   }
   if (!P.emit_src.empty()) {
-    const int32_t *a, *z;
-    RC_TRY(b->itensor(P.emit_src, &a));
-    RC_TRY(b->itensor(P.emit_dst, &z));
-    RC_TRY(sc_layernorm(b->xblk, a, d, b->enc, z, d, (int)P.emit_src.size(), d, e->f("enc_norm_g"), e->f("enc_norm_b"),
-                        c.ln_eps, b->es));
-  }
-  for (auto &sh : P.shorts) RC_TRY(encode_short(b, sh));
+    RC_TRY(b->itensor(P.emit_src, &T.ea));
+    RC_TRY(b->itensor(P.emit_dst, &T.ez));
+  }
+  T.shorts.resize(P.shorts.size());
+  for (size_t i = 0; i < P.shorts.size(); ++i) RC_TRY(encode_short_stage(b, P.shorts[i], T.shorts[i]));
   if (!P.sub_src.empty()) {
-    const int32_t *a, *z;
-    RC_TRY(b->itensor(P.sub_src, &a));
-    RC_TRY(b->itensor(P.sub_dst, &z));
-    RC_TRY(sc_copy_rows(b->subbuf, a, b->subbuf, z, (int)P.sub_src.size(), d, b->es));
-  }
+    RC_TRY(b->itensor(P.sub_src, &T.sa));
+    RC_TRY(b->itensor(P.sub_dst, &T.sz));
+  }
+  return SC_OK;
+}
+
+int encode_launch(sc_streams *b, EncPlan &P, const EncTabs &T) {
+  const sc_config &c = b->cfg;
+  sc_engine *e = b->eng;
+  const int d = c.d_model, F1 = c.conv_freq1, F2 = c.conv_freq2, R = c.block_size + 2;
+  b->enc_calls++;
+  ENC_LAUNCH(sc_conv1(b->featbuf, c.n_mels, T.cj, P.n_conv, P.max_t1, e->f("conv1_w"), e->f("conv1_b"), d, b->c1, b->es));
+  ENC_LAUNCH(sc_gemm(b->c1, T.ar, d, e->f("conv2_w"), e->f("conv2_b"), b->c2, nullptr, d, (int)P.a_rows.size(), d, 9 * d,
+                     SC_GEMM_RELU | b->gemm_flags, F1, b->es));
+  ENC_LAUNCH(sc_gemm(b->c2, nullptr, F2 * d, e->f("sub_out_w"), e->f("sub_out_b"), b->subbuf, T.ld, d, (int)P.lin_dst.size(), d,
+                     F2 * d, b->gemm_flags, 0, b->es));
+  if (!P.feat_src.empty())
+    ENC_LAUNCH(sc_copy_rows(b->featbuf, T.fa, b->featbuf, T.fz, (int)P.feat_src.size(), c.n_mels, b->es));
+  if (T.nbk > 0) {
+    ENC_LAUNCH(sc_block_pack(b->subbuf, T.bj, T.nbk, R, e->f("pe"), d, b->xblk, b->es));
+    ENC_LAUNCH(sc_ctx_handoff(b->xblk, R, T.ja, T.ns, b->prev_addin, 0, d, b->es));
+    ENC_LAUNCH(enc_layers_launch(b, T.nbk, R, true, b->jobs_ctx, T.ns));
+  }
+  if (!P.emit_src.empty())
+    ENC_LAUNCH(sc_layernorm(b->xblk, T.ea, d, b->enc, T.ez, d, (int)P.emit_src.size(), d, e->f("enc_norm_g"), e->f("enc_norm_b"),
+                            c.ln_eps, b->es));
+  for (size_t i = 0; i < P.shorts.size(); ++i) RC_TRY(encode_short(b, P.shorts[i], T.shorts[i]));
+  if (!P.sub_src.empty()) ENC_LAUNCH(sc_copy_rows(b->subbuf, T.sa, b->subbuf, T.sz, (int)P.sub_src.size(), d, b->es));
   return SC_OK;
 }
 
@@ -969,25 +1008,34 @@
 void span_job(const sc_streams *b, sc_ctc_beam_lm_job &j, const EncGroup::Span &sp, int opt) { span_job(b, j.beam, sp, opt); }
 
 template <typename J, typename Fill>
-int launch_spans(sc_streams *b, const EncGroup &g, int opt, const char *name, J *jobs_host, J *jobs_dev,
-                 int (*launch)(const J *, int, void *), Fill fill) {
+int stage_spans(sc_streams *b, const EncGroup &g, int opt, const char *name, int (*launch)(const J *, int, void *), Fill fill,
+                std::vector<std::function<int()>> &side) {
   if (g.spans.empty() || !g.spans[0].opt[opt].on) return SC_OK;
   const int n = (int)g.spans.size();
   if (n > b->S) {
     sc_set_error("%s: %d spans in a group of a batch of %d streams (internal error)", name, n, b->S);
     return SC_ERR_ARG;
   }
+  void *h = nullptr;
+  const void *dv = nullptr;
+  RC_TRY(b->table((size_t)n * sizeof(J), &h, &dv));
+  J *jobs_host = (J *)h;
+  const J *jobs_dev = (const J *)dv;
   const size_t o = (size_t)g.slot * b->S;
   for (int i = 0; i < n; ++i) {
-    span_job(b, jobs_host[o + i], g.spans[i], opt);
-    fill(jobs_host[o + i], g.spans[i], o + i);
-  }
-  HIP_TRY(hipMemcpyAsync(jobs_dev + o, jobs_host + o, (size_t)n * sizeof(J), hipMemcpyHostToDevice, b->es));
-  return launch(jobs_dev + o, n, b->es);
+    jobs_host[i] = J{};
+    span_job(b, jobs_host[i], g.spans[i], opt);
+    fill(jobs_host[i], g.spans[i], o + i);
+  }
+  side.push_back([=]() -> int {
+    ENC_LAUNCH(launch(jobs_dev, n, b->es));
+    return SC_OK;
+  });
+  return SC_OK;
 }
 
 template <typename Fill>
-int launch_beam_grammars(sc_streams *b, const EncGroup &g, Fill beam_fill) {
+int stage_beam_grammars(sc_streams *b, const EncGroup &g, Fill beam_fill, std::vector<std::function<int()>> &side) {
   if (g.spans.empty() || !g.spans[0].opt[OPT_BEAM].on) return SC_OK;
   const int n = (int)g.spans.size();
   if (n > b->S) {
@@ -996,14 +1044,24 @@
   }
   const size_t o = (size_t)g.slot * b->S;
   int n_plain = 0, n_gr = 0;
+  for (const EncGroup::Span &sp : g.spans) (sp.grammar ? n_gr : n_plain)++;
+  void *hp = nullptr, *hg = nullptr;
+  const void *dp = nullptr, *dg = nullptr;
+  RC_TRY(b->table((size_t)n_plain * sizeof(sc_ctc_beam_job), &hp, &dp));
+  RC_TRY(b->table((size_t)n_gr * sizeof(sc_ctc_beam_gr_job), &hg, &dg));
+  sc_ctc_beam_job *plain_host = (sc_ctc_beam_job *)hp;
+  sc_ctc_beam_gr_job *gr_host = (sc_ctc_beam_gr_job *)hg;
+  n_plain = n_gr = 0;
   for (int i = 0; i < n; ++i) {
     const EncGroup::Span &sp = g.spans[i];
     if (!sp.grammar) {
-      sc_ctc_beam_job &j = b->beam_jobs_host[o + n_plain++];
+      sc_ctc_beam_job &j = plain_host[n_plain++];
+      j = sc_ctc_beam_job{};
       span_job(b, j, sp, OPT_BEAM);
       beam_fill(j, sp, o + i);
     } else {
-      sc_ctc_beam_gr_job &j = b->beam_gr_jobs_host[o + n_gr++];
+      sc_ctc_beam_gr_job &j = gr_host[n_gr++];
+      j = sc_ctc_beam_gr_job{};
       span_job(b, j.beam, sp, OPT_BEAM);
       beam_fill(j.beam, sp, o + i);
       j.grammar = sp.grammar;
@@ -1011,37 +1069,32 @@
       j.gr_state_after = b->beam_gr_out_dev + o + i;
     }
   }
-  if (n_plain) {
-    HIP_TRY(hipMemcpyAsync(b->beam_jobs_dev + o, b->beam_jobs_host + o, (size_t)n_plain * sizeof(sc_ctc_beam_job),
-                           hipMemcpyHostToDevice, b->es));
-    RC_TRY(sc_ctc_beam(b->beam_jobs_dev + o, n_plain, b->es));
-  }
-  if (n_gr) {
-    HIP_TRY(hipMemcpyAsync(b->beam_gr_jobs_dev + o, b->beam_gr_jobs_host + o, (size_t)n_gr * sizeof(sc_ctc_beam_gr_job),
-                           hipMemcpyHostToDevice, b->es));
-    RC_TRY(sc_ctc_beam_grammar(b->beam_gr_jobs_dev + o, n_gr, b->es));
-  }
-  return SC_OK;
-}
-
-int project_rows(sc_streams *b, EncGroup &g) {
-  const sc_config &c = b->cfg;
-  sc_engine *e = b->eng;
-  const int d = c.d_model, Ld = c.dec_layers, V = c.vocab_size;
-  const int32_t *ar = nullptr;
+  side.push_back([=]() -> int {
+    if (n_plain) ENC_LAUNCH(sc_ctc_beam((const sc_ctc_beam_job *)dp, n_plain, b->es));
+    if (n_gr) ENC_LAUNCH(sc_ctc_beam_grammar((const sc_ctc_beam_gr_job *)dg, n_gr, b->es));
+    return SC_OK;
+  });
+  return SC_OK;
+}
+
+struct ProjTabs {
+  const int32_t *ar_ctc = nullptr, *ar_kv = nullptr, *kvt = nullptr;
+  std::vector<std::function<int()>> side;
+};
+
+int project_tables(sc_streams *b, EncGroup &g, ProjTabs &T) {
+  std::vector<std::function<int()>> &side = T.side;
   if (!g.ctc_rows.empty()) {
-    RC_TRY(b->itensor(g.ctc_rows, &ar));
-    RC_TRY(sc_gemm(b->enc, ar, d, e->f("ctc_w"), e->f("ctc_b"), const_cast<float *>(b->sb.ctcx), ar, V, (int)g.ctc_rows.size(),
-                   V, d, b->gemm_flags, 0, b->es));
-    RC_TRY(launch_spans(b, g, OPT_ACT, "activity", b->act_jobs_host, b->act_jobs_dev, sc_ctc_activity,
+    RC_TRY(b->itensor(g.ctc_rows, &T.ar_ctc));
+    RC_TRY(stage_spans(b, g, OPT_ACT, "activity", sc_ctc_activity,
                         [=](sc_ctc_activity_job &j, const EncGroup::Span &sp, size_t at) {
                           j.state = b->act_state + (size_t)sp.s * 6;
                           j.track = b->act_track + (size_t)sp.s * b->TCAP;
                           j.state_after = b->act_out_dev + at * 6;
                           j.thr = b->act_thr;
                           j.reserved = 0;
-                        }));
-    RC_TRY(launch_spans(b, g, OPT_SPOT, "spotting", b->spot_jobs_host, b->spot_jobs_dev, sc_ctc_spot,
+                        }, side));
+    RC_TRY(stage_spans(b, g, OPT_SPOT, "spotting", sc_ctc_spot,
                         [=](sc_ctc_spot_job &j, const EncGroup::Span &sp, size_t at) {
                           j.labels = b->spot_labels; j.lens = b->spot_lens; j.floors = b->spot_floors;
                           j.counters = b->spot_counters + (size_t)sp.s * 2;
@@ -1051,14 +1104,14 @@
                           j.state_after = b->spot_out_dev + at * 2;
                           j.mask = sp.mask;
                           j.P = b->spot_P;
-                        }));
-    RC_TRY(launch_spans(b, g, OPT_DRAFT, "draft", b->draft_jobs_host, b->draft_jobs_dev, sc_ctc_draft,
+                        }, side));
+    RC_TRY(stage_spans(b, g, OPT_DRAFT, "draft", sc_ctc_draft,
                         [=](sc_ctc_draft_job &j, const EncGroup::Span &sp, size_t at) {
                           j.state = b->draft_state + sp.s;
                           j.tokens = b->draft_tokens + (size_t)sp.s * b->TCAP;
                           j.state_after = b->draft_out_dev + at;
                           j.capacity = b->TCAP;
-                        }));
+                        }, side));
     const auto beam_fill = [=](sc_ctc_beam_job &j, const EncGroup::Span &sp, size_t at) {
       j.state = b->beam_state + sp.s;
       j.nodes = b->beam_nodes + (size_t)sp.s * b->beam_ncap();
@@ -1069,23 +1122,39 @@
     bool any_grammar = false;
     for (const EncGroup::Span &sp : g.spans) any_grammar = any_grammar || sp.grammar;
     if (any_grammar)
-      RC_TRY(launch_beam_grammars(b, g, beam_fill));
+      RC_TRY(stage_beam_grammars(b, g, beam_fill, side));
     else if (!b->beam_lm)
-      RC_TRY(launch_spans(b, g, OPT_BEAM, "beam", b->beam_jobs_host, b->beam_jobs_dev, sc_ctc_beam, beam_fill));
+      RC_TRY(stage_spans(b, g, OPT_BEAM, "beam", sc_ctc_beam, beam_fill, side));
     else
-      RC_TRY(launch_spans(b, g, OPT_BEAM, "beam", b->beam_lm_jobs_host, b->beam_lm_jobs_dev, sc_ctc_beam_lm,
+      RC_TRY(stage_spans(b, g, OPT_BEAM, "beam", sc_ctc_beam_lm,
                           [=](sc_ctc_beam_lm_job &j, const EncGroup::Span &sp, size_t at) {
                             beam_fill(j.beam, sp, at);
                             j.lm = b->beam_lm_view;
                             j.lm_state = b->beam_lm_state + sp.s;
                             j.lm_state_after = b->beam_lm_out_dev + at;
                             j.alpha = b->beam_alpha; j.beta = b->beam_beta;
-                          }));
+                          }, side));
   }
   if (!g.kv_dst.empty()) {
-    if (!g.same_rows || !ar) RC_TRY(b->itensor(g.kv_src, &ar));
-    const int32_t *kvt;
-    RC_TRY(b->itensor(g.kv_dst, &kvt));
+    T.ar_kv = T.ar_ctc;
+    if (!g.same_rows || !T.ar_kv) RC_TRY(b->itensor(g.kv_src, &T.ar_kv));
+    RC_TRY(b->itensor(g.kv_dst, &T.kvt));
+  }
+  return SC_OK;
+}
+
+int project_rows(sc_streams *b, EncGroup &g, const ProjTabs &T) {
+  const sc_config &c = b->cfg;
+  sc_engine *e = b->eng;
+  const int d = c.d_model, Ld = c.dec_layers, V = c.vocab_size;
+  if (!g.ctc_rows.empty()) {
+    ENC_LAUNCH(sc_gemm(b->enc, T.ar_ctc, d, e->f("ctc_w"), e->f("ctc_b"), const_cast<float *>(b->sb.ctcx), T.ar_ctc, V,
+                       (int)g.ctc_rows.size(), V, d, b->gemm_flags, 0, b->es));
+    for (const std::function<int()> &f : T.side) RC_TRY(f());
+  }
+  if (!g.kv_dst.empty()) {
+    RC_TRY(b->flush_tables());
+    const int32_t *ar = T.ar_kv, *kvt = T.kvt;
     const int m = (int)g.kv_dst.size();
     const bool all = e->wkv_all && (2 * d) % 128 == 0;
     if (!b->sb.kv_half) {
@@ -1114,34 +1183,40 @@
   if (g.copy_jobs.empty() && g.rs_jobs.empty() && g.pcm_jobs.empty()) return SC_OK;
   hipStream_t es = b->stream_enc ? b->stream_enc : b->stream;
   const int ss = g.stage_slot;
-  const size_t so = (size_t)ss * b->stage_cap, jo = (size_t)ss * b->S * 3;
-  const int nj = (int)g.copy_jobs.size() / 3;
-  if (g.stage_floats && (g.stage_filled || g.pcm_jobs.empty()))
-    HIP_TRY(hipMemcpyAsync(b->stage_dev + so, b->stage_host + so, g.stage_floats * sizeof(float), hipMemcpyHostToDevice, es));
-  if (!g.pcm_jobs.empty()) {
-    const size_t bo = (size_t)ss * b->stageb_cap, po = (size_t)ss * b->S;
-    const int np = (int)g.pcm_jobs.size();
-    if (g.stage_bytes)
+  const size_t so = b->stage_pay(ss);
+  const int nj = (int)g.copy_jobs.size() / 3, np = (int)g.pcm_jobs.size(), nr = (int)g.rs_jobs.size();
+  if (nj > b->S || np > b->S || nr > b->S) {
+    sc_set_error("stage_copy: %d / %d / %d jobs in an admission of a batch of %d streams (internal error)", nj, np, nr, b->S);
+    return SC_ERR_ARG;
+  }
+  if (nj) memcpy(b->hdr_host<long long>(ss, 0), g.copy_jobs.data(), g.copy_jobs.size() * sizeof(long long));
+  if (nr) memcpy(b->hdr_host<sc_rs_job>(ss, b->hdr_rs), g.rs_jobs.data(), nr * sizeof(sc_rs_job));
+  if (np) memcpy(b->hdr_host<sc_pcm_job>(ss, b->hdr_pcm), g.pcm_jobs.data(), np * sizeof(sc_pcm_job));
+  const bool floats = g.stage_floats && (g.stage_filled || g.pcm_jobs.empty());
+  {
+    const size_t o = b->stage_base(ss);
+    HIP_TRY(hipMemcpyAsync(b->stage_dev + o, b->stage_host + o, (b->stage_hdr + (floats ? g.stage_floats : 0)) * sizeof(float),
+                           hipMemcpyHostToDevice, es));
+    b->n_group_uploads++;
+  }
+  if (np) {
+    const size_t bo = (size_t)ss * b->stageb_cap;
+    if (g.stage_bytes) {
       HIP_TRY(hipMemcpyAsync(b->stageb_dev + bo, b->stageb_host + bo, g.stage_bytes, hipMemcpyHostToDevice, es));
-    memcpy(b->pcmjobs_host + po, g.pcm_jobs.data(), np * sizeof(sc_pcm_job));
-    HIP_TRY(hipMemcpyAsync(b->pcmjobs_dev + po, b->pcmjobs_host + po, np * sizeof(sc_pcm_job), hipMemcpyHostToDevice, es));
-    RC_TRY(sc_pcm_decode(b->pcmjobs_dev + po, np, es));
+      b->n_group_uploads++;
+    }
+    RC_TRY(sc_pcm_decode(b->hdr_dev<sc_pcm_job>(ss, b->hdr_pcm), np, es));
   }
   if (nj) {
-    memcpy(b->cjobs_host + jo, g.copy_jobs.data(), g.copy_jobs.size() * sizeof(long long));
-    HIP_TRY(hipMemcpyAsync(b->cjobs_dev + jo, b->cjobs_host + jo, g.copy_jobs.size() * sizeof(long long), hipMemcpyHostToDevice, es));
     long long mx = 1;
     for (int j = 0; j < nj; ++j) mx = std::max(mx, g.copy_jobs[j * 3 + 2]);
-    launch_scatter(b->stage_dev + so, g.features ? b->featbuf : b->pcm, b->cjobs_dev + jo, nj, mx, es);
-  }
-  if (!g.rs_jobs.empty()) {
-    const size_t ro = (size_t)ss * b->S;
-    const int nr = (int)g.rs_jobs.size();
-    memcpy(b->rsjobs_host + ro, g.rs_jobs.data(), nr * sizeof(sc_rs_job));
-    HIP_TRY(hipMemcpyAsync(b->rsjobs_dev + ro, b->rsjobs_host + ro, nr * sizeof(sc_rs_job), hipMemcpyHostToDevice, es));
+    launch_scatter(b->stage_dev + so, g.features ? b->featbuf : b->pcm, b->hdr_dev<long long>(ss, 0), nj, mx, es);
+  }
+  if (nr) {
     long long tiles = 1;
     for (const sc_rs_job &j : g.rs_jobs) tiles = std::max(tiles, sc_rs_tiles(b->rs_tabs, j.tab, j.n_out));
-    RC_TRY(sc_rs_launch(b->rs_tabs, nullptr, b->rsjobs_dev + ro, nr, tiles, b->stage_dev + so, b->pcm, b->rs_hist, b->S, es));
+    RC_TRY(sc_rs_launch(b->rs_tabs, nullptr, b->hdr_dev<sc_rs_job>(ss, b->hdr_rs), nr, tiles, b->stage_dev + so, b->pcm, b->rs_hist,
+                        b->S, es));
   }
   HIP_TRY(hipEventRecord(b->ev_stage[ss], es));
   b->stage_busy[ss] = true;
@@ -1187,19 +1262,31 @@
   const sc_config &c = b->cfg;
   sc_engine *e = b->eng;
   b->es = b->stream_enc ? b->stream_enc : b->stream;
-  b->cur_slot = g->slot;
-  b->arena_off = 0;
-  int rc = SC_OK;
-  if (rc == SC_OK && g->n_fe) {
-    const int32_t *jobs;
-    rc = b->itensor(g->fe_jobs, &jobs);
-    if (rc == SC_OK)
-      rc = sc_logmel(b->pcm, (int)b->PCAP, jobs, g->n_fe, g->max_keep, e->f("window"), e->f("mel_fb"), e->f("twiddle"),
-                     (const double *)e->f("mean64"), (const double *)e->f("std64"), c.mvn_mode, c.n_fft, c.hop_length,
-                     c.win_length, c.n_mels, b->featbuf, b->es);
-  }
-  if (rc == SC_OK && g->P.n_conv) rc = encode_launch(b, g->P);
-  if (rc == SC_OK) rc = project_rows(b, *g);
+  b->tab.begin(g->slot, b->slot_cap);
+  b->n_groups_launched++;
+  const int32_t *fe = nullptr;
+  EncTabs ET;
+  ProjTabs PT;
+  auto stage = [&]() -> int {
+    if (g->n_fe) RC_TRY(b->itensor(g->fe_jobs, &fe));
+    if (g->P.n_conv) RC_TRY(encode_stage(b, g->P, ET));
+    return project_tables(b, *g, PT);
+  };
+  auto launch = [&]() -> int {
+    RC_TRY(b->flush_tables());
+    if (ET.jc_host) {
+      HIP_TRY(hipMemcpyAsync(b->jobs_ctx, ET.jc_host, (size_t)ET.ns * 4 * sizeof(int32_t), hipMemcpyHostToDevice, b->es));
+      b->n_group_uploads++;
+    }
+    if (g->n_fe)
+      ENC_LAUNCH(sc_logmel(b->pcm, (int)b->PCAP, fe, g->n_fe, g->max_keep, e->f("window"), e->f("mel_fb"), e->f("twiddle"),
+                           (const double *)e->f("mean64"), (const double *)e->f("std64"), c.mvn_mode, c.n_fft, c.hop_length,
+                           c.win_length, c.n_mels, b->featbuf, b->es));
+    if (g->P.n_conv) RC_TRY(encode_launch(b, g->P, ET));
+    return project_rows(b, *g, PT);
+  };
+  int rc = stage();
+  if (rc == SC_OK) rc = launch();
   (void)hipEventRecord(b->ev_group[g->slot], b->es);
   if (b->es == b->stream) b->gen_ordered = std::max(b->gen_ordered, g->gen);
   b->es = b->stream;
@@ -1329,9 +1416,11 @@
     b->dec_blocks++;
   }
   HIP_TRY(hipMemcpyAsync(b->ctrlmap, ctrl0, (size_t)S * 8 * sizeof(int32_t), hipMemcpyHostToDevice, b->stream));
+  b->n_tick_uploads++;
   if (n_lsm) {
     int32_t *ld = b->bs_dev + (size_t)b->bs_i * b->bs_cap;
     HIP_TRY(hipMemcpyAsync(ld, lsm, (size_t)n_lsm * sizeof(int32_t), hipMemcpyHostToDevice, b->stream));
+    b->n_tick_uploads++;
     RC_TRY(sc_log_softmax_rows(const_cast<float *>(b->sb.ctcx), ld, n_lsm, b->cfg.vocab_size, b->stream));
   }
   RC_TRY(sc_ctc_extend_state(&b->sb, b->stream));
@@ -1408,6 +1497,8 @@
   } else {
     HIP_TRY(hipMemcpyAsync(b->ctrlmap, b->ctrlmap_host, (size_t)S * 8 * sizeof(int32_t), hipMemcpyHostToDevice, b->stream));
   }
+  b->n_tick_uploads++;
+  b->n_ticks++;
   RC_TRY(decode_step_launch(b));
   HIP_TRY(hipEventRecord(b->ev_iter[b->iter & 1], b->stream));
   const int form = sc_decode_step_form(&b->sb);
@@ -1497,7 +1588,7 @@
 void plan_group(sc_streams *b, const std::vector<Chunk> &chunks, bool features, EncGroup &g, std::map<int, int> &feat_new,
                 std::map<int, bool> &finals, std::vector<int> &has_out) {
   const sc_config &c = b->cfg;
-  float *stage = g.stage_slot >= 0 ? b->stage_host + (size_t)g.stage_slot * b->stage_cap : nullptr;
+  float *stage = g.stage_slot >= 0 ? b->stage_host + b->stage_pay(g.stage_slot) : nullptr;
   auto stage_chunk = [&](const Chunk &ch, const St &st) {
     if (!st.coded()) {
       if (ch.n > 0) memcpy(stage + g.stage_floats, ch.host, (size_t)ch.n * sizeof(float));
@@ -1512,7 +1603,7 @@
     sc_pcm_job j{};
     j.src = b->stageb_dev + bo;
     j.offset = (int64_t)g.stage_bytes;
-    j.dst = b->stage_dev + (size_t)g.stage_slot * b->stage_cap + g.stage_floats;
+    j.dst = b->stage_dev + b->stage_pay(g.stage_slot) + g.stage_floats;
     j.level = b->lvl_state + ch.s;
     j.level_after = b->lvl_out_dev + po + g.pcm_jobs.size();
     j.format = st.in_fmt; j.channels = st.in_ch; j.channel = st.in_sel; j.scale = st.in_scale;
@@ -2062,17 +2153,21 @@
   A(b->ws_ffh, m_enc * F);
   A(b->jobs_ctx, (size_t)S * 4);
   A(b->ctrlmap, (size_t)S * 8 + n);
-  b->slot_cap = (((size_t)S * ((size_t)b->max_t2 * (c.conv_freq2 + 12) + 512) + 8192) + 63) & ~size_t(63);
+  b->slot_cap = (((size_t)S * ((size_t)b->max_t2 * (c.conv_freq2 + 12) + 512 + 128) + 8192 + 1024) + 63) & ~size_t(63);
   A(b->arena_dev, b->slot_cap * N_ARENA);
   b->bs_cap = (size_t)S * 8 + (size_t)S * c.block_size;
   A(b->bs_dev, b->bs_cap * N_RING);
   b->stage_cap = (size_t)S * std::max<size_t>((size_t)b->max_chunk + 16 * c.hop_length, (size_t)b->max_feat_new * c.n_mels);
-  A(b->stage_dev, b->stage_cap * N_STAGE);
+  {
+    auto up = [](size_t x) { return (x + 255) & ~size_t(255); };
+    b->hdr_rs = up((size_t)S * 3 * sizeof(long long));
+    b->hdr_pcm = b->hdr_rs + up((size_t)S * sizeof(sc_rs_job));
+    b->stage_hdr = (b->hdr_pcm + up((size_t)S * sizeof(sc_pcm_job))) / sizeof(float);
+  }
+  A(b->stage_dev, (b->stage_hdr + b->stage_cap) * N_STAGE);
   b->pack_cap = n * (2 * (size_t)b->LCAP + 8);
   A(b->pack_dev, b->pack_cap);
   A(b->pjobs_dev, n * 4);
-  A(b->cjobs_dev, (size_t)N_STAGE * S * 3);
-  A(b->rsjobs_dev, (size_t)N_STAGE * S);
   A(b->rs_hist, (size_t)2 * S * SC_RS_HIST);
   sc_search &sb = b->sb;
   sb.S = S; sb.W = W; sb.K = K; sb.V = V; sb.d = d; sb.H = c.dec_heads; sb.F = F; sb.n_layers = c.dec_layers;
@@ -2180,9 +2275,8 @@
   bool ok = b->halloc(&b->ctrlmap_host, (size_t)S * 8 + n) == SC_OK && b->halloc(&b->flags_host, (size_t)S * 2) == SC_OK &&
             b->halloc(&b->rm_host[0], n) == SC_OK && b->halloc(&b->rm_host[1], n) == SC_OK &&
             b->halloc(&b->arena_host, b->slot_cap * N_ARENA) == SC_OK && b->halloc(&b->bs_host, b->bs_cap * N_RING) == SC_OK &&
-            b->halloc(&b->stage_host, b->stage_cap * N_STAGE) == SC_OK && b->halloc(&b->pack_host, b->pack_cap) == SC_OK &&
-            b->halloc(&b->pjobs_host, n * 4) == SC_OK && b->halloc(&b->cjobs_host, (size_t)N_STAGE * S * 3) == SC_OK &&
-            b->halloc(&b->rsjobs_host, (size_t)N_STAGE * S) == SC_OK;
+            b->halloc(&b->stage_host, (b->stage_hdr + b->stage_cap) * N_STAGE) == SC_OK && b->halloc(&b->pack_host, b->pack_cap) == SC_OK &&
+            b->halloc(&b->pjobs_host, n * 4) == SC_OK;
   for (int i = 0; i < 2 && ok; ++i) ok = hipEventCreateWithFlags(&b->ev_iter[i], hipEventDisableTiming) == hipSuccess;
   for (int i = 0; i < N_ARENA && ok; ++i) ok = hipEventCreateWithFlags(&b->ev_group[i], hipEventDisableTiming) == hipSuccess;
   for (int i = 0; i < N_STAGE && ok; ++i) ok = hipEventCreateWithFlags(&b->ev_stage[i], hipEventDisableTiming) == hipSuccess;
@@ -2323,8 +2417,6 @@
     b->stageb_cap = b->stage_cap * sizeof(float);
     if (!b->stageb_dev) RC_TRY(b->alloc(&b->stageb_dev, b->stageb_cap * N_STAGE));
     if (!b->stageb_host) RC_TRY(b->halloc(&b->stageb_host, b->stageb_cap * N_STAGE));
-    if (!b->pcmjobs_dev) RC_TRY(b->alloc(&b->pcmjobs_dev, S * N_STAGE));
-    if (!b->pcmjobs_host) RC_TRY(b->halloc(&b->pcmjobs_host, S * N_STAGE));
     if (!b->lvl_out_dev) RC_TRY(b->halloc_mapped(&b->lvl_out_host, &b->lvl_out_dev, S * N_STAGE, __func__, "level slots"));
     b->lvl.init(b->S);
     RC_TRY(b->alloc(&b->lvl_state, S));
@@ -3351,8 +3443,6 @@
     const size_t S = (size_t)b->S;
     RC_TRY(b->alloc(&b->act_state, S * 6));
     RC_TRY(b->alloc(&b->act_track, S * b->TCAP));
-    RC_TRY(b->alloc(&b->act_jobs_dev, S * N_ARENA));
-    RC_TRY(b->halloc(&b->act_jobs_host, S * N_ARENA));
     RC_TRY(b->halloc_mapped(&b->act_out_host, &b->act_out_dev, S * N_ARENA * 6, __func__, "state slots"));
     b->act.init(b->S);
   }
@@ -3442,8 +3532,6 @@
     RC_TRY(b->alloc(&b->spot_values, S * PS));
     RC_TRY(b->alloc(&b->spot_starts, S * PS));
     RC_TRY(b->alloc(&b->spot_events, S * SC_SPOT_MAX_EVENTS));
-    RC_TRY(b->alloc(&b->spot_jobs_dev, S * N_ARENA));
-    RC_TRY(b->halloc(&b->spot_jobs_host, S * N_ARENA));
     RC_TRY(b->halloc_mapped(&b->spot_out_host, &b->spot_out_dev, S * N_ARENA * 2, __func__, "counter slots"));
     b->spot.init(b->S);
   }
@@ -3525,8 +3613,6 @@
     const size_t S = (size_t)b->S;
     RC_TRY(b->alloc(&b->draft_state, S));
     RC_TRY(b->alloc(&b->draft_tokens, S * b->TCAP));
-    RC_TRY(b->alloc(&b->draft_jobs_dev, S * N_ARENA));
-    RC_TRY(b->halloc(&b->draft_jobs_host, S * N_ARENA));
     RC_TRY(b->halloc_mapped(&b->draft_out_host, &b->draft_out_dev, S * N_ARENA, __func__, "state slots"));
     b->draft.init(b->S);
   }
@@ -3599,8 +3685,6 @@
   if (!b->beam_state) {
     const size_t S = (size_t)b->S;
     RC_TRY(b->alloc(&b->beam_state, S));
-    RC_TRY(b->alloc(&b->beam_jobs_dev, S * N_ARENA));
-    RC_TRY(b->halloc(&b->beam_jobs_host, S * N_ARENA));
     RC_TRY(b->halloc_mapped(&b->beam_out_host, &b->beam_out_dev, S * N_ARENA, __func__, "state slots"));
     b->beam.init(b->S);
   }
@@ -3643,8 +3727,6 @@
   if (!b->beam_lm_state) {
     const size_t S = (size_t)b->S;
     RC_TRY(b->alloc(&b->beam_lm_state, S));
-    RC_TRY(b->alloc(&b->beam_lm_jobs_dev, S * N_ARENA));
-    RC_TRY(b->halloc(&b->beam_lm_jobs_host, S * N_ARENA));
     RC_TRY(b->halloc_mapped(&b->beam_lm_out_host, &b->beam_lm_out_dev, S * N_ARENA, __func__, "state slots"));
   }
   HIP_TRY(hipStreamSynchronize(b->es));
@@ -3721,8 +3803,6 @@
     if (!b->beam_gr_state) {
       const size_t S = (size_t)b->S;
       RC_TRY(b->alloc(&b->beam_gr_state, S));
-      RC_TRY(b->alloc(&b->beam_gr_jobs_dev, S * N_ARENA));
-      RC_TRY(b->halloc(&b->beam_gr_jobs_host, S * N_ARENA));
       RC_TRY(b->halloc_mapped(&b->beam_gr_out_host, &b->beam_gr_out_dev, S * N_ARENA, __func__, "state slots"));
     }
     if (b->beam_gr.empty()) b->beam_gr.assign((size_t)b->S, nullptr);
@@ -4194,6 +4274,15 @@
   return SC_OK;
 }
 
+extern "C" int sc_streams_copy_stats(const sc_streams *b, long *group_uploads, long *groups, long *tick_uploads, long *ticks) {
+  SC_CHECK_ARG(b && group_uploads && groups && tick_uploads && ticks, "null");
+  *group_uploads = b->n_group_uploads;
+  *groups = b->n_groups_launched;
+  *tick_uploads = b->n_tick_uploads;
+  *ticks = b->n_ticks;
+  return SC_OK;
+}
+
 extern "C" int sc_streams_stats(const sc_streams *b, long *enc_calls, long *dec_steps, long *dec_blocks) {
   SC_CHECK_ARG(b, "null");
   if (enc_calls) *enc_calls = b->enc_calls;
diff --git a/speechcatcher_amd/csrc/table_arena.h b/speechcatcher_amd/csrc/table_arena.h
--- /dev/null
+++ b/speechcatcher_amd/csrc/table_arena.h
@@ -0,0 +1,42 @@
+#pragma once
+#include <cstddef>
+#include <cstdint>
+#include <cstring>
+
+namespace table_arena {
+
+constexpr size_t ALIGN = 64;
+
+struct Slot {
+  size_t cap = 0;
+  size_t base = 0;
+  size_t off = 0;
+  size_t flushed = 0;
+  long n_copies = 0;
+
+  void begin(int slot, size_t slot_cap) {
+    cap = slot_cap;
+    base = (size_t)slot * slot_cap;
+    off = flushed = 0;
+    n_copies = 0;
+  }
+  bool dirty() const { return off > flushed; }
+  size_t reserve(size_t n_bytes) {
+    const size_t n = (n_bytes + sizeof(int32_t) - 1) / sizeof(int32_t);
+    if (n > cap || off > cap - n) return (size_t)-1;
+    const size_t at = base + off;
+    off += (n + ALIGN - 1) & ~(ALIGN - 1);
+    if (off > cap) off = cap;
+    return at;
+  }
+  template <typename Copy>
+  int flush(Copy copy) {
+    if (!dirty()) return 0;
+    const int rc = copy(base + flushed, off - flushed);
+    flushed = off;
+    ++n_copies;
+    return rc;
+  }
+};
+
+}
diff --git a/speechcatcher_amd/native.py b/speechcatcher_amd/native.py
--- a/speechcatcher_amd/native.py
+++ b/speechcatcher_amd/native.py
@@ -114,6 +114,13 @@
         a, b, c = C.c_long(), C.c_long(), C.c_long()
         self.lib.sc_streams_stats(self.handle, C.byref(a), C.byref(b), C.byref(c))
         return {"enc_calls": a.value, "dec_steps": b.value, "dec_blocks": c.value}
+
+    @property
+    def copy_stats(self):
+        a, b, c, d = C.c_long(), C.c_long(), C.c_long(), C.c_long()
+        _abi.check(self.lib.sc_streams_copy_stats(self.handle, C.byref(a), C.byref(b), C.byref(c), C.byref(d)),
+                   "sc_streams_copy_stats")
+        return {"group_uploads": a.value, "groups": b.value, "tick_uploads": c.value, "ticks": d.value}
 
     def _fault(self, s, code):
         msg = (self.lib.sc_stream_last_error(self.handle, int(s)) or b"").decode()
```

Result: no change. 4097, median of 6 (+0.7%).
